# smolGura/fish-tts

Hardware: AMD Instinct MI355X
Metric: semantic tokens/sec (higher is better)
Workload: dtype bf16; 1 GPU; openaudio-s1-mini shapes (BASELINE configs[1]): batch=1 per GPU, 48-token prompt, 215 frames (10 s), top-p sampling, hipGraph-captured frame step, + DAC codec decode; prompt_len=48, parallelism=replica x1, frame_engine=3

## Files before the change

fish-tts_amd/csrc/engine.hip:

```cpp
#include "engine.h"
#include "ar_kernels.h"
#include "frame_engine.h"
#include "wide_kernels.h"
#include "codec_kernels.h"

#include <math.h>

#include <algorithm>
#include <mutex>
#include <stdio.h>
#include <stdlib.h>
#include <string.h>

using namespace ft;

static std::string g_create_err;
static void eng_release(ft_ctx* ctx);

ft_status ft_fail(ft_ctx* ctx, ft_status code, const std::string& msg) {
    if (ctx) ctx->err = msg; else g_create_err = msg;
    return code;
}

template <typename S, typename D>
// ... 131 lines not shown
    FT_TRY(dmalloc(ctx, &ctx->part_ml, M * c.n_head * ctx->nsplit_max * 2));
    ctx->cache_m_stride = (size_t)c.n_local_heads * ctx->n_slots * c.head_dim;
    ctx->fcache_m_stride = (size_t)c.fast_n_local_heads * c.num_codebooks * c.fast_head_dim;
    ctx->layers.resize(c.n_layer);
    ctx->flayers.resize(c.n_fast_layer);
    for (auto& l : ctx->layers) {
        FT_TRY(dmalloc(ctx, (char**)&l.kc, M * ctx->cache_m_stride * ctx->esz));
        FT_TRY(dmalloc(ctx, (char**)&l.vc, M * ctx->cache_m_stride * ctx->esz));
    }
    for (auto& l : ctx->flayers) {
        FT_TRY(dmalloc(ctx, (char**)&l.kc, M * ctx->fcache_m_stride * ctx->esz));
        FT_TRY(dmalloc(ctx, (char**)&l.vc, M * ctx->fcache_m_stride * ctx->esz));
    }
    const size_t R = c.num_codebooks + 1;
    FT_TRY(dmalloc(ctx, &ctx->d_pos, M));
    FT_TRY(dmalloc(ctx, &ctx->d_tok, M * R));
    FT_TRY(dmalloc(ctx, &ctx->d_tokn, M * R));
    FT_TRY(dmalloc(ctx, &ctx->d_seq, M * R * ctx->cap));
    FT_TRY(dmalloc(ctx, &ctx->d_nf, M));
    FT_TRY(dmalloc(ctx, &ctx->d_done, M));
    FT_TRY(dmalloc(ctx, &ctx->d_prompt, R * (size_t)c.max_seq_len));
    FT_TRY(dmalloc(ctx, &ctx->d_ctl, M));
    ctx->prefill_gemm_mode = getenv("FT_PREFILL_GEMM") ? atoi(getenv("FT_PREFILL_GEMM")) : 2;
    ctx->prefill_v0 = getenv("FT_PREFILL_V0") != nullptr || c.dtype != FT_BF16 || c.dim % 32 || (c.n_head * c.head_dim) % 32 ||
                      c.intermediate_size % 32;
    if (!ctx->prefill_v0) {
        const size_t S = c.max_seq_len;
        FT_TRY(dmalloc(ctx, &ctx->pf_x, S * c.dim));
        FT_TRY(dmalloc(ctx, &ctx->pf_qkv, S * qkvN));
        FT_TRY(dmalloc(ctx, &ctx->pf_y, S * c.n_head * c.head_dim));
        FT_TRY(dmalloc(ctx, &ctx->pf_xn, S * c.dim));
        FT_TRY(dmalloc(ctx, &ctx->pf_ybf, S * c.n_head * c.head_dim));
        FT_TRY(dmalloc(ctx, &ctx->pf_g, S * c.intermediate_size));
        FT_TRY(dmalloc(ctx, &ctx->pf_qbf, S * c.n_head * c.head_dim));
        FT_TRY(dmalloc(ctx, &ctx->pf_seqs, M));
        FT_TRY(dmalloc(ctx, &ctx->pf_rows, S));
    }
    if (c.dtype == FT_F16 || !ctx->prefill_v0) {
        const int HD = c.n_head * c.head_dim, HDf = c.fast_n_head * c.fast_head_dim;
        ctx->wide_ok = !getenv("FT_NO_WIDE") && !c.fast_attention_qkv_bias && !c.fast_attention_o_bias && c.fast_dim == c.dim &&
                       wide_k_ok(c.dim) && wide_k_ok(HD) && wide_k_ok(c.intermediate_size) && wide_k_ok(HDf) && wide_k_ok(c.fast_intermediate_size) &&
                       qkvN % 32 == 0 && fqkvN % 32 == 0 && c.intermediate_size % 16 == 0 && c.fast_intermediate_size % 16 == 0 &&
                       c.dim % 16 == 0 && c.vocab_size % 32 == 0 && ctx->fastV % 16 == 0;
        if (ctx->wide_ok) {
            ctx->xo_pair = (int)((M + 15) / 16 * 16);
            ctx->no_pair = getenv("FT_NO_PAIR") != nullptr;
            ctx->no_attn_wide = getenv("FT_NO_ATTN_WIDE") != nullptr;
            ctx->no_head_stream = getenv("FT_NO_HEAD_STREAM") != nullptr;
            ctx->xo_ldm = 2 * ctx->xo_pair;
            const size_t P = ctx->xo_ldm;
            FT_TRY(dmalloc(ctx, &ctx->xo_x, P * c.dim));
            FT_TRY(dmalloc(ctx, &ctx->xo_xf, P * c.fast_dim));
            FT_TRY(dmalloc(ctx, &ctx->xo_femb, P * c.fast_dim));
            FT_TRY(dmalloc(ctx, &ctx->xo_y, P * (size_t)std::max(HD, HDf)));
            FT_TRY(dmalloc(ctx, &ctx->xo_g, P * (size_t)std::max(c.intermediate_size, c.fast_intermediate_size)));
        }
    }
    const size_t nchunk = ((size_t)c.vocab_size + 1023) / 1024;
    FT_TRY(dmalloc(ctx, &ctx->samp_cut, M));
    FT_TRY(dmalloc(ctx, &ctx->samp_chunk_cnt, M * nchunk));
    FT_TRY(dmalloc(ctx, &ctx->samp_part_score, M * nchunk));
    FT_TRY(dmalloc(ctx, &ctx->samp_part_idx, M * nchunk));
    FT_HIP(ctx, hipHostMalloc((void**)&ctx->h_pin, (3 * M + 8) * sizeof(int), hipHostMallocDefault));
    return FT_OK;
}

extern "C" ft_status ft_create(const ft_ar_config* ar, const ft_codec_config* codec, int32_t device, ft_ctx** out) {
    if (!out || (!ar && !codec)) return ft_fail(nullptr, FT_ERR_ARG, "ft_create: need a config and an out pointer");
    int ndev = 0;
    if (hipGetDeviceCount(&ndev) != hipSuccess || ndev == 0)
        return ft_fail(nullptr, FT_ERR_HIP, "ft_create: no HIP device visible (the MI355X path has no CPU fallback)");
    if (device < 0 || device >= ndev) return ft_fail(nullptr, FT_ERR_ARG, "ft_create: bad device index");
    ft_ctx* ctx = new ft_ctx();
    ctx->device = device;
    ft_status st = FT_OK;
    do {
        if (hipSetDevice(device) != hipSuccess) { st = ft_fail(ctx, FT_ERR_HIP, "hipSetDevice failed"); break; }
        if (hipStreamCreateWithFlags(&ctx->stream, hipStreamNonBlocking) != hipSuccess) {
            st = ft_fail(ctx, FT_ERR_HIP, "hipStreamCreate failed"); break;
        }
        if (ar) {
            ctx->c = *ar;
            ctx->has_ar = true;
            if ((st = ar_validate(ctx)) != FT_OK) break;
            if ((st = ar_alloc(ctx)) != FT_OK) break;
            ar_expected(ctx);
        }
        if (codec) {
            ctx->cc = *codec;
            ctx->has_codec = true;
            if ((st = codec_create(ctx)) != FT_OK) break;
            codec_expected(ctx);
        }
    } while (0);
    if (st != FT_OK) {
        g_create_err = ctx->err;
        ft_destroy(ctx);
        return st;
    }
    *out = ctx;
    return FT_OK;
}

extern "C" void ft_destroy(ft_ctx* ctx) {
    if (!ctx) return;
    hipSetDevice(ctx->device);
    if (ctx->stream) hipStreamSynchronize(ctx->stream);
    for (auto& kv : ctx->graphs) hipGraphExecDestroy(kv.second);
    for (auto& kv : ctx->expected) if (kv.second.p) hipFree(kv.second.p);
    for (auto& l : ctx->layers) { hipFree(l.kc); hipFree(l.vc); if (l.w13) hipFree(l.w13); }
    for (auto& l : ctx->flayers) { hipFree(l.kc); hipFree(l.vc); if (l.w13) hipFree(l.w13); }
    float* bufs[] = {ctx->x, ctx->qkv, ctx->y, ctx->g, ctx->logits, ctx->femb, ctx->xf, ctx->qkvf, ctx->gf,
                     ctx->flog, ctx->part_o, ctx->part_ml, ctx->noise};
    for (float* b : bufs) if (b) hipFree(b);
    if (ctx->hid && ctx->hid != ctx->x) hipFree(ctx->hid);
    int* ibufs[] = {ctx->d_pos, ctx->d_tok, ctx->d_tokn, ctx->d_seq, ctx->d_nf, ctx->d_done, ctx->d_prompt};
    for (int* b : ibufs) if (b) hipFree(b);
    if (ctx->d_ctl) hipFree(ctx->d_ctl);
    if (ctx->wide_qkv0_tab) hipFree(ctx->wide_qkv0_tab);
    { void* pf[] = {ctx->pf_x, ctx->pf_qkv, ctx->pf_y, ctx->pf_xn, ctx->pf_ybf, ctx->pf_g, ctx->xo_x, ctx->xo_xf, ctx->xo_femb, ctx->xo_y, ctx->xo_g, ctx->pf_qbf}; for (void* q : pf) if (q) hipFree(q); }
    for (auto& l : ctx->layers) { if (l.bqkv_f32) hipFree(l.bqkv_f32); if (l.bo_f32) hipFree(l.bo_f32); }
    if (ctx->samp_cut) hipFree(ctx->samp_cut);
    if (ctx->samp_chunk_cnt) hipFree(ctx->samp_chunk_cnt);
    if (ctx->samp_part_score) hipFree(ctx->samp_part_score);
    if (ctx->samp_part_idx) hipFree(ctx->samp_part_idx);
    eng_release(ctx);
    if (ctx->h_pin) hipHostFree(ctx->h_pin);
    for (auto e : ctx->prof_ev) hipEventDestroy(e);
    codec_destroy(ctx);
    if (ctx->stream) hipStreamDestroy(ctx->stream);
    delete ctx;
}

extern "C" const char* ft_last_error(const ft_ctx* ctx) { return ctx ? ctx->err.c_str() : g_create_err.c_str(); }

extern "C" ft_status ft_sync(ft_ctx* ctx) {
    if (!ctx) return FT_ERR_ARG;
    FT_HIP(ctx, hipSetDevice(ctx->device));
    FT_HIP(ctx, hipStreamSynchronize(ctx->stream));
    return FT_OK;
}

extern "C" ft_status ft_load_weight(ft_ctx* ctx, const char* name, const void* src, int32_t src_dtype,
                                    const int64_t* shape, int32_t ndim) {
    if (!ctx || !name || !src || !shape) return ft_fail(ctx, FT_ERR_ARG, "ft_load_weight: null argument");
    if (ctx->finalized) return ft_fail(ctx, FT_ERR_STATE, "ft_load_weight: weights already finalized");
    auto it = ctx->expected.find(name);
    if (it == ctx->expected.end()) return ft_fail(ctx, FT_ERR_ARG, std::string("unknown weight name: ") + name);
    FtTensor& t = it->second;
    if ((int)t.shape.size() != ndim) return ft_fail(ctx, FT_ERR_ARG, std::string("rank mismatch for ") + name);
    for (int i = 0; i < ndim; ++i)
        if (t.shape[i] != shape[i]) {
            char buf[256];
            snprintf(buf, sizeof buf, "shape mismatch for %s: dim %d is %lld, expected %lld", name, i,
                     (long long)shape[i], (long long)t.shape[i]);
            return ft_fail(ctx, FT_ERR_ARG, buf);
        }
    if (src_dtype != FT_F32 && src_dtype != FT_BF16 && src_dtype != FT_F16)
        return ft_fail(ctx, FT_ERR_ARG, "src_dtype must be FT_F32, FT_BF16 or FT_F16");
    FT_HIP(ctx, hipSetDevice(ctx->device));
    const int64_t n = t.numel();
    const size_t ssz = src_dtype == FT_F32 ? 4 : 2, dsz = t.dtype == FT_F32 ? 4 : 2;
    if (!t.p) FT_HIP(ctx, hipMalloc(&t.p, (size_t)n * dsz + 64));
    if (src_dtype == t.dtype) {
        FT_HIP(ctx, hipMemcpy(t.p, src, (size_t)n * dsz, hipMemcpyDefault));
        return FT_OK;
    }
    void* stage = nullptr;
    FT_HIP(ctx, hipMalloc(&stage, (size_t)n * ssz));
    hipError_t e = hipMemcpy(stage, src, (size_t)n * ssz, hipMemcpyDefault);
    if (e == hipSuccess) {
        const int blocks = (int)((n + 255) / 256 < 4096 ? (n + 255) / 256 : 4096);
        auto to = [&](auto* sp) {
            if (t.dtype == FT_F32) convert_kernel<<<blocks, 256, 0, ctx->stream>>>(sp, (float*)t.p, n);
            else if (t.dtype == FT_BF16) convert_kernel<<<blocks, 256, 0, ctx->stream>>>(sp, (bf16_t*)t.p, n);
            else convert_kernel<<<blocks, 256, 0, ctx->stream>>>(sp, (f16_t*)t.p, n);
        };
        if (src_dtype == FT_F32) to((const float*)stage);
        else if (src_dtype == FT_BF16) to((const bf16_t*)stage);
        else to((const f16_t*)stage);
        e = hipStreamSynchronize(ctx->stream);
    }
    hipFree(stage);
    if (e != hipSuccess) return ft_fail(ctx, FT_ERR_HIP, std::string("ft_load_weight copy: ") + hipGetErrorString(e));
    return FT_OK;
}

static void* wp(ft_ctx* ctx, const std::string& n) {
    auto it = ctx->expected.find(n);
    return it == ctx->expected.end() ? nullptr : it->second.p;
}

static ft_status eng_setup(ft_ctx* ctx);
static ft_status wide_qkv0_build(ft_ctx* ctx);

static ft_status ar_finalize(ft_ctx* ctx) {
    const ft_ar_config& c = ctx->c;
    ctx->emb = wp(ctx, "embeddings.weight");
    ctx->cb_emb = wp(ctx, "codebook_embeddings.weight");
    ctx->norm = wp(ctx, "norm.weight");
    ctx->head = c.tie_word_embeddings ? ctx->emb : wp(ctx, "output.weight");
    ctx->fproj_w = wp(ctx, "fast_project_in.weight");
    ctx->fproj_b = wp(ctx, "fast_project_in.bias");
    ctx->fast_emb = wp(ctx, "fast_embeddings.weight");
    ctx->fast_norm = wp(ctx, "fast_norm.weight");
    ctx->fast_out = wp(ctx, "fast_output.weight");
    ctx->rope = (float*)wp(ctx, "rope.slow");
    ctx->frope = (float*)wp(ctx, "rope.fast");
    auto fill = [&](std::vector<FtLayer>& ls, const char* pre, int ffn, int dim) -> ft_status {
        for (size_t i = 0; i < ls.size(); ++i) {
            const std::string p = std::string(pre) + std::to_string(i);
            FtLayer& l = ls[i];
            l.attn_norm = wp(ctx, p + ".attention_norm.weight");
            l.wqkv = wp(ctx, p + ".attention.wqkv.weight");
            l.bqkv = wp(ctx, p + ".attention.wqkv.bias");
            l.qn = wp(ctx, p + ".attention.q_norm.weight");
            l.kn = wp(ctx, p + ".attention.k_norm.weight");
            l.wo = wp(ctx, p + ".attention.wo.weight");
            l.bo = wp(ctx, p + ".attention.wo.bias");
            l.ffn_norm = wp(ctx, p + ".ffn_norm.weight");
            l.w2 = wp(ctx, p + ".feed_forward.w2.weight");
            FtTensor& w1 = ctx->expected[p + ".feed_forward.w1.weight"];
            FtTensor& w3 = ctx->expected[p + ".feed_forward.w3.weight"];
            FT_HIP(ctx, hipMalloc(&l.w13, (size_t)2 * ffn * dim * ctx->esz));
            const int64_t n = (int64_t)ffn * dim;
            const int blocks = (int)((n + 255) / 256 < 4096 ? (n + 255) / 256 : 4096);
            if (ctx->esz == 2)
                interleave_rows_kernel<bf16_t><<<blocks, 256, 0, ctx->stream>>>((bf16_t*)w1.p, (bf16_t*)w3.p, (bf16_t*)l.w13, ffn, dim);
            else
                interleave_rows_kernel<float><<<blocks, 256, 0, ctx->stream>>>((float*)w1.p, (float*)w3.p, (float*)l.w13, ffn, dim);
            FT_HIP(ctx, hipStreamSynchronize(ctx->stream));
            hipFree(w1.p); w1.p = nullptr;
            hipFree(w3.p); w3.p = nullptr;
        }
        return FT_OK;
    };
    FT_TRY(fill(ctx->layers, "layers.", c.intermediate_size, c.dim));
    if (!ctx->prefill_v0 || ctx->wide_ok) {
        const int qkvN = (c.n_head + 2 * c.n_local_heads) * c.head_dim;
        auto to_f32 = [&](const void* b, float* o, int n) {
            if (c.dtype == FT_F16) convert_kernel<f16_t, float><<<(n + 255) / 256, 256, 0, ctx->stream>>>((const f16_t*)b, o, n);
            else convert_kernel<bf16_t, float><<<(n + 255) / 256, 256, 0, ctx->stream>>>((const bf16_t*)b, o, n);
        };
        for (auto& l : ctx->layers) {
            if (l.bqkv) {
                FT_HIP(ctx, hipMalloc((void**)&l.bqkv_f32, qkvN * sizeof(float)));
                to_f32(l.bqkv, l.bqkv_f32, qkvN);
            }
            if (l.bo) {
                FT_HIP(ctx, hipMalloc((void**)&l.bo_f32, c.dim * sizeof(float)));
                to_f32(l.bo, l.bo_f32, c.dim);
            }
        }
        FT_HIP(ctx, hipStreamSynchronize(ctx->stream));
    }
    FT_TRY(fill(ctx->flayers, "fast_layers.", c.fast_intermediate_size, c.fast_dim));
    FT_TRY(eng_setup(ctx));
    FT_TRY(wide_qkv0_build(ctx));
    return FT_OK;
}

constexpr int ENG_MAX_STRIKES = 2;
static std::mutex g_eng_mu;
static std::map<int, ft_ctx*> g_eng_owner;

static void eng_release(ft_ctx* ctx) {
    void* eb[] = {ctx->eng_layers, ctx->eng_flayers, ctx->eng_gx ,
                  ctx->eng_gpart, ctx->eng_fast_g, ctx->eng_ctl, ctx->eng_qkv0_tab};
    for (void* q : eb) if (q) hipFree(q);
    ctx->eng_layers = ctx->eng_flayers = nullptr;
    ctx->eng_gx = ctx->eng_gqkv = ctx->eng_gy = ctx->eng_gxb = ctx->eng_gg = ctx->eng_fast_g = ctx->eng_ctl = nullptr;
    ctx->eng_gpart = nullptr;
    ctx->eng_qkv0_tab = nullptr;
    ctx->eng_on = ctx->eng_fast_on = false;
    if (ctx->eng_owner) {
        std::lock_guard<std::mutex> lk(g_eng_mu);
        auto it = g_eng_owner.find(ctx->device);
        if (it != g_eng_owner.end() && it->second == ctx) g_eng_owner.erase(it);
        ctx->eng_owner = false;
    }
}

static bool eng_fits_cu(const void* fn, size_t lds, size_t lds_cap, const char* name, std::string& why) {
    hipFuncAttributes fa{};
    const hipError_t fe = hipFuncGetAttributes(&fa, fn);
    if (fe != hipSuccess) { (void)hipGetLastError(); why = std::string("hipFuncGetAttributes: ") + hipGetErrorString(fe); return false; }
    const int regs = std::max(fa.numRegs, 1), per_simd = 512 / (((regs + 7) / 8) * 8);
    const bool fits = per_simd * 4 >= ENG_THREADS / 64 && lds + fa.sharedSizeBytes <= lds_cap && fa.maxThreadsPerBlock >= ENG_THREADS;
    if (getenv("FT_LOG")) {
        int occ = -1;
        const hipError_t oe = hipOccupancyMaxActiveBlocksPerMultiprocessor(&occ, fn, ENG_THREADS, lds);
        if (oe != hipSuccess) (void)hipGetLastError();
        fprintf(stderr, "fish_tts_amd: %s engine kernel: %d registers (%d waves per SIMD), %zu B of LDS of %zu: %s (the occupancy query says %d)\n",
                name, fa.numRegs, per_simd, lds + fa.sharedSizeBytes, lds_cap, fits ? "fits a CU" : "does not fit a CU", occ);
    }
    if (!fits) why = std::string("a ") + name + " workgroup does not fit one CU (registers / LDS)";
    return fits;
}

typedef void (*eng_slow_fn_t)(SlowEngP);
typedef void (*eng_fast_fn_t)(FastEngP);
typedef void (*eng_qkv0_fn_t)(const bf16_t*, const bf16_t*, const bf16_t*, const bf16_t*, bf16_t*, int, int, int, float);
struct EngSlowEntry { int D, H, HKV, HDIM, F, SQ, SF, SO; eng_slow_fn_t xl, plain; };
struct EngFastEntry { int D, H, HKV, HDIM, F, V, SQ, SF, SO; eng_fast_fn_t loop; eng_qkv0_fn_t qkv0; };
template <typename S, bool WITH_XL>
static EngSlowEntry eng_slow_entry() {
    eng_slow_fn_t xl = nullptr;
    if constexpr (WITH_XL) xl = slow_engine_kernel<S, true>;
    return EngSlowEntry{S::D, S::H, S::HKV, S::HDIM, S::F, S::SQ, S::SF, S::SO, xl, slow_engine_kernel<S, false>};
}
template <typename S>
static EngFastEntry eng_fast_entry() {
    return EngFastEntry{S::D, S::H, S::HKV, S::HDIM, S::F, S::V, S::SQ, S::SF, S::SO, fast_engine_kernel<S, 10>, eng_qkv0_table_kernel<S>};
}
static const EngSlowEntry* eng_slow_shapes(int* n) {
    static const EngSlowEntry tab[] = {eng_slow_entry<EngSlowS1, true>(), eng_slow_entry<EngSlowShape<1024, 16, 8, 128, 4096>, true>(),
                                       eng_slow_entry<EngSlowShape<1024, 16, 4, 128, 3072>, false>()};
    *n = (int)(sizeof tab / sizeof tab[0]);
    return tab;
}
static const EngFastEntry* eng_fast_shapes(int* n) {
    static const EngFastEntry tab[] = {eng_fast_entry<EngFastS1>(), eng_fast_entry<EngFastShape<1024, 16, 8, 64, 4096, 1024>>()};
    *n = (int)(sizeof tab / sizeof tab[0]);
    return tab;
}

static bool eng_setup_try(ft_ctx* ctx, std::string& why) {
    const ft_ar_config& c = ctx->c;
    auto hip_ok = [&](hipError_t e, const char* what) {
        if (e == hipSuccess) return true;
        why = std::string(what) + ": " + hipGetErrorString(e);
        (void)hipGetLastError();
        return false;
    };
    if (getenv("FT_NO_ENGINE")) { why = "FT_NO_ENGINE is set"; return false; }
    if (c.dtype != FT_BF16) { why = "precision is not bf16"; return false; }
    hipDeviceProp_t prop;
    if (!hip_ok(hipGetDeviceProperties(&prop, ctx->device), "hipGetDeviceProperties")) return false;
    const int nb = prop.multiProcessorCount;
    const int HD = c.n_head * c.head_dim;
    const int qkvN = (c.n_head + 2 * c.n_local_heads) * c.head_dim;
    auto per = [&](int units) { return (units + nb - 1) / nb; };
    const EngSlowEntry* se = nullptr;
    {
        int n = 0;
        const EngSlowEntry* tab = eng_slow_shapes(&n);
        for (int i = 0; i < n && !se; ++i)
            if (c.dim == tab[i].D && c.n_head == tab[i].H && c.n_local_heads == tab[i].HKV && c.head_dim == tab[i].HDIM && c.intermediate_size == tab[i].F)
                se = &tab[i];
    }
    const bool shape_ok = se && c.fast_dim == c.dim && c.n_layer >= 1 && c.n_layer < ENG_EPOCH_STEP &&
                          per(qkvN) <= se->SQ * ENG_CW && per(c.dim) <= se->SO * ENG_CW && per(c.intermediate_size) <= se->SF * ENG_CW &&
                          qkvN % (4 * nb) == 0 && c.dim % (4 * nb) == 0 && c.intermediate_size % (4 * nb) == 0 && per(qkvN) <= ENG_LINE &&
                          per(c.intermediate_size) <= ENG_LINE && c.n_local_heads * ctx->nsplit_max <= nb && c.head_dim % (4 * ctx->nsplit_max) == 0 && nb == ENG_NB;
    if (!shape_ok) {
        char buf[320];
        snprintf(buf, sizeof buf, "widths outside the engine's instantiations (dim %d, heads %d / %d x %d, ffn %d, fast_dim %d on %d CUs; "
                 "built for dim 1024, 16 heads x 128 with 8 kv heads and ffn 3072 or 4096, or 4 kv heads and ffn 3072, on 256 CUs)", c.dim, c.n_head,
                 c.n_local_heads, c.head_dim, c.intermediate_size, c.fast_dim, nb);
        why = buf;
        return false;
    }
    {
        std::lock_guard<std::mutex> lk(g_eng_mu);
        auto it = g_eng_owner.find(ctx->device);
        if (it != g_eng_owner.end() && it->second != ctx) {
            why = "another context of this process already runs the frame engine on this device (its workgroups need every CU)";
            return false;
        }
        g_eng_owner[ctx->device] = ctx;
        ctx->eng_owner = true;
    }
    ctx->eng_nb = nb;
    std::vector<EngLayer> h(c.n_layer);
    for (int i = 0; i < c.n_layer; ++i) {
        const FtLayer& l = ctx->layers[i];
        h[i] = EngLayer{(const bf16_t*)l.wqkv, (const bf16_t*)l.bqkv, (const bf16_t*)l.attn_norm, (const bf16_t*)l.qn,
                        (const bf16_t*)l.kn, (const bf16_t*)l.wo, (const bf16_t*)l.bo, (const bf16_t*)l.ffn_norm,
                        (const bf16_t*)l.w13, (const bf16_t*)l.w2, (bf16_t*)l.kc, (bf16_t*)l.vc};
    }
    if (!hip_ok(hipMalloc((void**)&ctx->eng_layers, h.size() * sizeof(EngLayer)), "hipMalloc(engine layer table)")) return false;
    if (!hip_ok(hipMemcpy(ctx->eng_layers, h.data(), h.size() * sizeof(EngLayer), hipMemcpyHostToDevice), "hipMemcpy(engine layer table)")) return false;
    auto zalloc = [&](void** q, size_t bytes, const char* what) {
        return hip_ok(hipMalloc(q, bytes), what) && hip_ok(hipMemset(*q, 0, bytes), what);
    };
    const size_t L = c.n_layer;
    const size_t VB = (size_t)nb * ENG_LINE * 4;
    const size_t pool_words = ((L + 1) * VB + 3 * L * VB + L * HD * 4) / 4;
    ctx->eng_relay = getenv("FT_NO_RELAY") == nullptr;
    ctx->eng_pool_bytes = pool_words * 4 * (ctx->eng_relay ? 9 : 1);
    if (!zalloc((void**)&ctx->eng_gx, ctx->eng_pool_bytes, "hipMalloc(engine hand-off pool)")) return false;
    ctx->eng_pool_words = pool_words;
    ctx->eng_gxb = ctx->eng_gx + (L + 1) * (VB / 4);
    ctx->eng_gg = ctx->eng_gxb + L * (VB / 4);
    ctx->eng_gy = ctx->eng_gg + L * (VB / 4);
    ctx->eng_gqkv = ctx->eng_gy + L * HD;
    ctx->eng_gpart_bytes = L * c.n_head * ctx->nsplit_max * (size_t)(c.head_dim + 2) * 8;
    if (!zalloc((void**)&ctx->eng_gpart, ctx->eng_gpart_bytes, "hipMalloc(engine split partials)")) return false;
    if (!zalloc((void**)&ctx->eng_ctl, ENG_CTL_WORDS * 4, "hipMalloc(engine control words)")) return false;
    const int G = c.n_head / c.n_local_heads, hd = c.head_dim, NSLOT = 4 * (64 / (hd >> 3));
    size_t fl = (size_t)c.dim * 2 + HD + c.intermediate_size + (size_t)(G + 2) * hd + (size_t)G * hd + 2 * hd +
                (size_t)NSLOT * G * 2 + (size_t)NSLOT * G * hd + 64 * 6 + ENG_MAX_OUT + 8;
    ctx->eng_lds_slow = std::max(fl * sizeof(float), (size_t)82 * 1024);
    const size_t lds_cap = prop.maxSharedMemoryPerMultiProcessor;
    if (ctx->eng_lds_slow > lds_cap) { why = "the slow stack's LDS need exceeds the CU's"; return false; }
    ctx->eng_xl = ctx->xl_shape && nb == 256 && ctx->nsplit_max == 32 && c.n_local_heads * 32 == nb;
    ctx->eng_xl = ctx->eng_xl && se->xl != nullptr;
    ctx->eng_slow_fn = (const void*)(ctx->eng_xl ? se->xl : se->plain);
    const void* slow_fn = ctx->eng_slow_fn;
    if (!hip_ok(hipFuncSetAttribute(slow_fn, hipFuncAttributeMaxDynamicSharedMemorySize, (int)ctx->eng_lds_slow),
                "hipFuncSetAttribute(slow_engine_kernel)")) return false;
    if (!eng_fits_cu(slow_fn, ctx->eng_lds_slow, lds_cap, "slow-stack", why)) return false;
    ctx->eng_on = true;
    why = ctx->eng_xl ? "slow stack on the frame engine (one kv head per XCD)" : "slow stack on the frame engine";

    const int HDf = c.fast_n_head * c.fast_head_dim;
    const int fqkvN = (c.fast_n_head + 2 * c.fast_n_local_heads) * c.fast_head_dim;
    const EngFastEntry* fe = nullptr;
    {
        int n = 0;
        const EngFastEntry* tab = eng_fast_shapes(&n);
        for (int i = 0; i < n && !fe; ++i)
            if (c.fast_dim == tab[i].D && c.fast_n_head == tab[i].H && c.fast_n_local_heads == tab[i].HKV && c.fast_head_dim == tab[i].HDIM &&
                c.fast_intermediate_size == tab[i].F && ctx->fastV == tab[i].V)
                fe = &tab[i];
    }
    const bool fast_ok = !getenv("FT_NO_FAST_ENGINE") && fe && HDf == c.fast_dim && c.n_fast_layer >= 1 &&
                         c.num_codebooks >= 2 && c.num_codebooks <= 10 && fqkvN % (4 * nb) == 0 && ctx->fastV % (4 * nb) == 0 &&
                         per(fqkvN) <= fe->SQ * ENG_CW && per(c.fast_dim) <= fe->SO * ENG_CW && per(c.fast_intermediate_size) <= fe->SF * ENG_CW &&
                         per(ctx->fastV) <= fe->SO * ENG_CW && per(fqkvN) <= ENG_LINE && per(c.fast_intermediate_size) <= ENG_LINE && ctx->fastV <= 1024 &&
                         c.codebook_size <= 65536;
    if (!fast_ok) { why += "; fast loop on launches (FT_NO_FAST_ENGINE, or fast widths outside the instantiations: 1024 / 16 + 8 heads x 64 / ffn 3072 or 4096 / 1024 codes used, <= 10 codebooks)"; return true; }
    ctx->eng_fast_fn = (const void*)fe->loop;
    auto fast_off = [&](const std::string& w2) { why += "; fast loop on launches (" + w2 + ")"; return true; };
    std::vector<EngLayer> hf(c.n_fast_layer);
    for (int i = 0; i < c.n_fast_layer; ++i) {
        const FtLayer& l = ctx->flayers[i];
        hf[i] = EngLayer{(const bf16_t*)l.wqkv, (const bf16_t*)l.bqkv, (const bf16_t*)l.attn_norm, (const bf16_t*)l.qn,
                         (const bf16_t*)l.kn, (const bf16_t*)l.wo, (const bf16_t*)l.bo, (const bf16_t*)l.ffn_norm,
                         (const bf16_t*)l.w13, (const bf16_t*)l.w2, nullptr, nullptr};
    }
    std::string w2;
    auto hip_ok2 = [&](hipError_t e, const char* what) {
        if (e == hipSuccess) return true;
        w2 = std::string(what) + ": " + hipGetErrorString(e);
        (void)hipGetLastError();
        return false;
    };
    if (!hip_ok2(hipMalloc((void**)&ctx->eng_flayers, hf.size() * sizeof(EngLayer)), "hipMalloc(fast layer table)")) return fast_off(w2);
    if (!hip_ok2(hipMemcpy(ctx->eng_flayers, hf.data(), hf.size() * sizeof(EngLayer), hipMemcpyHostToDevice), "hipMemcpy(fast layer table)")) return fast_off(w2);
    const size_t nLf = c.n_fast_layer;
    ctx->eng_fast_words = (2 * ((nLf + 1) + 3 * nLf + 1)) * (VB / 4) + (size_t)c.num_codebooks * ENG_LINE;
    ctx->eng_fast_bytes = ctx->eng_fast_words * 4 * (ctx->eng_relay ? 9 : 1);
    if (!hip_ok2(hipMalloc((void**)&ctx->eng_fast_g, ctx->eng_fast_bytes), "hipMalloc(fast hand-off pool)") ||
        !hip_ok2(hipMemset(ctx->eng_fast_g, 0, ctx->eng_fast_bytes), "hipMemset(fast hand-off pool)")) return fast_off(w2);
    const int kvw = c.fast_n_local_heads * c.fast_head_dim;
    ctx->eng_pair = getenv("FT_NO_PAIR") == nullptr &&
                    eng_fast_lds_bytes(c.fast_dim, fqkvN, HDf, c.fast_intermediate_size, ctx->fastV, (int)nLf, c.num_codebooks, kvw, true) <= lds_cap;
    ctx->eng_lds_fast = eng_fast_lds_bytes(c.fast_dim, fqkvN, HDf, c.fast_intermediate_size, ctx->fastV, (int)nLf, c.num_codebooks, kvw, ctx->eng_pair);
    if (ctx->eng_lds_fast > lds_cap) return fast_off("the codebook loop's LDS need exceeds the CU's");
    ctx->eng_lds_fast = std::max(ctx->eng_lds_fast, (size_t)82 * 1024);
    if (!hip_ok2(hipFuncSetAttribute(ctx->eng_fast_fn, hipFuncAttributeMaxDynamicSharedMemorySize,
                                     (int)ctx->eng_lds_fast), "hipFuncSetAttribute(fast_engine_kernel)")) return fast_off(w2);
    if (!eng_fits_cu(ctx->eng_fast_fn, ctx->eng_lds_fast, lds_cap, "codebook-loop", w2)) return fast_off(w2);
    if (getenv("FT_NO_QKV0") == nullptr && c.num_codebooks > 2) {
        const size_t tb = (size_t)ctx->fastV * fqkvN * sizeof(bf16_t);
        if (!hip_ok2(hipMalloc((void**)&ctx->eng_qkv0_tab, tb), "hipMalloc(layer-0 q k v table)")) return fast_off(w2);
        const FtLayer& l0 = ctx->flayers[0];
        const size_t lds = ((size_t)c.fast_dim + ENG_MAX_OUT) * sizeof(float);
        fe->qkv0<<<dim3(fqkvN / (fe->SQ * ENG_CW), 16), ENG_CW * 64, lds, ctx->stream>>>(
            (const bf16_t*)l0.wqkv, (const bf16_t*)l0.bqkv, (const bf16_t*)l0.attn_norm, (const bf16_t*)ctx->fast_emb,
            (bf16_t*)ctx->eng_qkv0_tab, c.fast_dim, fqkvN, ctx->fastV, c.norm_eps);
        if (!hip_ok2(hipGetLastError(), "eng_qkv0_table_kernel") || !hip_ok2(hipStreamSynchronize(ctx->stream), "eng_qkv0_table_kernel")) {
            hipFree(ctx->eng_qkv0_tab); ctx->eng_qkv0_tab = nullptr;
            return fast_off(w2);
        }
    }
    ctx->eng_fast_on = true;
    why = ctx->eng_xl ? "slow stack (one kv head per XCD) and codebook loop on the frame engine" : "slow stack and codebook loop on the frame engine";
    return true;
}

static ft_status eng_setup(ft_ctx* ctx) {
    ctx->eng_on = ctx->eng_fast_on = false;
    std::string why;
    if (!eng_setup_try(ctx, why)) {
        eng_release(ctx);
        ctx->eng_why = "launch path: " + why;
    } else {
        char buf[64];
        snprintf(buf, sizeof buf, " (%d workgroups)", ctx->eng_nb);
        ctx->eng_why = why + buf;
    }
    if (getenv("FT_LOG")) fprintf(stderr, "fish_tts_amd: batch-1 decode frames: %s\n", ctx->eng_why.c_str());
    return FT_OK;
}

extern "C" ft_status ft_finalize_weights(ft_ctx* ctx) {
    if (!ctx) return FT_ERR_ARG;
    if (ctx->finalized) return FT_OK;
    FT_HIP(ctx, hipSetDevice(ctx->device));
    for (auto& kv : ctx->expected)
        if (!kv.second.p) return ft_fail(ctx, FT_ERR_MISSING_WEIGHT, "missing weight: " + kv.first);
    if (ctx->has_ar) FT_TRY(ar_finalize(ctx));
    if (ctx->has_codec) FT_TRY(codec_finalize(ctx));
    ctx->finalized = true;
    return FT_OK;
}

struct Launch {
    ft_ctx* ctx;
    hipStream_t s;
    int m0, M;
    int pos_off;
    hipError_t err = hipSuccess;
    bool gemv_only = false;
    bool tail_only = false;
    void chk() { hipError_t e = hipGetLastError(); if (e != hipSuccess && err == hipSuccess) err = e; }
};

struct PfX {
    const void* gain = nullptr;
    const float* ss_in = nullptr;
    int nblk = 0;
    float* ss_out = nullptr;
};
enum { PF_ID_NONE = -1, PF_ID_SKINNY1 = 0, PF_ID_SKINNY2 = 1, PF_ID_SKINNY4 = 2, PF_ID_LIN128 = 3, PF_ID_LIN64 = 4, PF_ID_TAP64_128 = 5,
       PF_ID_TAP64_64 = 6, PF_ID_TAP_128 = 7, PF_ID_TAP_64 = 8 };
static int pf_gemm(Launch& L, const bf16_t* X, long ldx, int S, const void* W, const float* bias, int N, int K,
                   int act, const float* resid, float* out_f32, bf16_t* out_bf, long ldo, int round_out,
                   const PfX& fx = PfX());
static bool wide_batch(const Launch& L) {
    return L.ctx->wide_ok && L.M >= L.ctx->wide_min && L.M <= 64 && !L.gemv_only && !L.ctx->prof;
}

static bool wide_pair(const Launch& L) {
    const ft_ctx* ctx = L.ctx;
    return wide_batch(L) && !ctx->no_pair && ctx->c.num_codebooks >= 2 && ctx->c.n_fast_layer > 0 && ctx->xo_pair + L.M <= 64;
}

enum { WIDE_ID_S11 = 0, WIDE_ID_S12 = 1, WIDE_ID_S22 = 2, WIDE_ID_G12 = 3, WIDE_ID_G22 = 4, WIDE_ID_R11 = 5, WIDE_ID_HEAD = 6 };
template <typename WT>
static int wide_gemm(Launch& L, const bf16_t* X, const void* W, const float* bias, int N, int K, const void* gain, int epi,
                      float* out_f32, long ldo, bf16_t* out_xo, const bf16_t* resid_xo, int rows = 0, bool vocab_head = false) {
    const int M = rows > 0 ? rows : L.M;
    WidePT<WT> p{};
    p.X = (const WT*)X; p.ldm = L.ctx->xo_ldm; p.W = (const WT*)W; p.ldw = K; p.gain = (const WT*)gain; p.eps = L.ctx->c.norm_eps;
    p.bias = bias; p.M = M; p.N = N; p.K = K; p.out_f32 = out_f32; p.ldo = ldo; p.out_xo = (WT*)out_xo; p.ldm_o = L.ctx->xo_ldm;
    p.resid_xo = (const WT*)resid_xo;
    bool ok;
    int id;
    if (epi == WEPI_RESID) { id = WIDE_ID_R11; ok = wide_gemm_launch<1, 1, false, WEPI_RESID>(p, L.s); }
    else if (epi == WEPI_SWIGLU) {
        id = M > 16 ? WIDE_ID_G22 : WIDE_ID_G12;
        ok = M > 16 ? wide_gemm_launch<2, 2, true, WEPI_SWIGLU>(p, L.s) : wide_gemm_launch<1, 2, true, WEPI_SWIGLU>(p, L.s);
    }
    else if (vocab_head && M <= 32 && K == 1024 && N % 16 == 0 && N >= 4096 && !L.ctx->no_head_stream) {
        static DevOnce once;
        once.run([] { hipFuncSetAttribute((const void*)wide_head_kernel<1024, WT>, hipFuncAttributeMaxDynamicSharedMemorySize, (int)wide_head_lds<1024>()); });
        wide_head_kernel<1024, WT><<<256, 512, wide_head_lds<1024>(), L.s>>>(p);
        id = WIDE_ID_HEAD;
        ok = true;
    }
    else if (N >= 32768) {
        id = M > 16 ? WIDE_ID_S22 : WIDE_ID_S12;
        ok = M > 16 ? wide_gemm_launch<2, 2, true, WEPI_STORE>(p, L.s) : wide_gemm_launch<1, 2, true, WEPI_STORE>(p, L.s);
    }
    else if (N >= 4096 && M > 16) { id = WIDE_ID_S12; ok = wide_gemm_launch<1, 2, true, WEPI_STORE>(p, L.s); }
    else { id = WIDE_ID_S11; ok = wide_gemm_launch<1, 1, true, WEPI_STORE>(p, L.s); }
    if (!ok && L.err == hipSuccess) L.err = hipErrorInvalidValue;
    L.chk();
    return id;
}

template <typename WT>
static __global__ __launch_bounds__(256) void xo_from_rows_kernel(const float* x, int ldx, int D, bf16_t* xo, int ldm) {
    const int m = blockIdx.y;
    for (int d = blockIdx.x * 256 + threadIdx.x; d < D; d += gridDim.x * 256) xo[xo_index(m, d, ldm)] = h16_bits<WT>(x[(size_t)m * ldx + d]);
}

static __global__ __launch_bounds__(256) void xo_from_h16_rows_kernel(const bf16_t* x, int D, bf16_t* xo, int ldm, int rows) {
    const int m = blockIdx.y;
    if (m >= rows) return;
    for (int d = blockIdx.x * 256 + threadIdx.x; d < D; d += gridDim.x * 256) xo[xo_index(m, d, ldm)] = x[(size_t)m * D + d];
}
template <typename WT>
static __global__ void f32_to_h16_kernel(const float* x, bf16_t* o, long n) {
    for (long i = (long)blockIdx.x * blockDim.x + threadIdx.x; i < n; i += (long)gridDim.x * blockDim.x) o[i] = h16_bits<WT>(x[i]);
}

template <typename WT>
static ft_status wide_qkv0_build_t(ft_ctx* ctx) {
    const ft_ar_config& c = ctx->c;
    if (!ctx->wide_ok || getenv("FT_NO_QKV0") || c.num_codebooks <= 2 || c.n_fast_layer < 1) return FT_OK;
    const int Df = c.fast_dim, qkvN = (c.fast_n_head + 2 * c.fast_n_local_heads) * c.fast_head_dim, V = ctx->fastV;
    const FtLayer& l0 = ctx->flayers[0];
    if (l0.bqkv) return FT_OK;
    constexpr int CH = 64;
    bf16_t* xo = nullptr; float* out = nullptr;
    if (hipMalloc((void**)&xo, (size_t)Df * CH * sizeof(bf16_t)) != hipSuccess || hipMalloc((void**)&out, (size_t)CH * qkvN * sizeof(float)) != hipSuccess ||
        hipMalloc((void**)&ctx->wide_qkv0_tab, (size_t)V * qkvN * sizeof(bf16_t)) != hipSuccess) {
        (void)hipGetLastError();
        if (xo) hipFree(xo);
        if (out) hipFree(out);
        if (ctx->wide_qkv0_tab) { hipFree(ctx->wide_qkv0_tab); ctx->wide_qkv0_tab = nullptr; }
        return FT_OK;
    }
    bool ok = true;
    for (int c0 = 0; c0 < V && ok; c0 += CH) {
        const int rows = std::min(CH, V - c0);
        xo_from_h16_rows_kernel<<<dim3((Df + 255) / 256, rows), 256, 0, ctx->stream>>>((const bf16_t*)ctx->fast_emb + (size_t)c0 * Df, Df, xo, CH, rows);
        WidePT<WT> p{};
        p.X = (const WT*)xo; p.ldm = CH; p.W = (const WT*)l0.wqkv; p.ldw = Df; p.gain = (const WT*)l0.attn_norm; p.eps = c.norm_eps;
        p.M = rows; p.N = qkvN; p.K = Df; p.out_f32 = out; p.ldo = qkvN;
        ok = wide_gemm_launch<1, 1, true, WEPI_STORE>(p, ctx->stream);
        f32_to_h16_kernel<WT><<<256, 256, 0, ctx->stream>>>(out, ctx->wide_qkv0_tab + (size_t)c0 * qkvN, (long)rows * qkvN);
    }
    ok = ok && hipStreamSynchronize(ctx->stream) == hipSuccess && hipGetLastError() == hipSuccess;
    hipFree(xo); hipFree(out);
    if (!ok) { hipFree(ctx->wide_qkv0_tab); ctx->wide_qkv0_tab = nullptr; (void)hipGetLastError(); }
    return FT_OK;
}
static ft_status wide_qkv0_build(ft_ctx* ctx) {
    if (ctx->c.dtype == FT_BF16) return wide_qkv0_build_t<bf16_t>(ctx);
    if (ctx->c.dtype == FT_F16) return wide_qkv0_build_t<f16_t>(ctx);
    return FT_OK;
}

static bool eng_slow_ok(const Launch& L) {
    const ft_ctx* ctx = L.ctx;
    return ctx->eng_on && !ctx->eng_suspended && L.M == 1 && !L.gemv_only && !ctx->prof && ctx->c.n_local_heads * ctx->nsplit <= ctx->eng_nb &&
           ctx->c.head_dim % (4 * ctx->nsplit) == 0;
}

static bool eng_fast_ok(const Launch& L) {
    const ft_ctx* ctx = L.ctx;
    return ctx->eng_fast_on && !ctx->eng_suspended && L.M == 1 && !L.gemv_only && !ctx->prof;
}

static void enqueue_fast_engine(Launch& L) {
    ft_ctx* ctx = L.ctx;
    const ft_ar_config& c = ctx->c;
    const int m0 = L.m0, R = c.num_codebooks + 1, nb = ctx->eng_nb;
    const size_t nLf = c.n_fast_layer, VW = (size_t)nb * ENG_LINE;
    FastEngP p{};
    p.layers = ctx->eng_flayers; p.n_layer = c.n_fast_layer; p.ncb = c.num_codebooks;
    p.D = c.fast_dim; p.H = c.fast_n_head; p.Hkv = c.fast_n_local_heads; p.hd = c.fast_head_dim; p.F = c.fast_intermediate_size;
    p.qkvN = (c.fast_n_head + 2 * c.fast_n_local_heads) * c.fast_head_dim; p.V = ctx->fastV;
    p.eps = c.norm_eps; p.scale = (float)(1.0 / sqrt((double)c.fast_head_dim));
    p.rope = ctx->frope; p.fast_norm = (const bf16_t*)ctx->fast_norm; p.fast_out = (const bf16_t*)ctx->fast_out;
    p.fast_emb = (const bf16_t*)ctx->fast_emb;
    p.qkv0_tab = (const bf16_t*)ctx->eng_qkv0_tab;
    p.hid = ctx->hid + (size_t)m0 * c.fast_dim; p.femb = ctx->femb + (size_t)m0 * c.fast_dim;
    unsigned* g = ctx->eng_fast_g;
    p.gx = g; g += 2 * (nLf + 1) * VW;
    p.gqkv = g; g += 2 * nLf * VW;
    p.gxb = g; g += 2 * nLf * VW;
    p.gg = g; g += 2 * nLf * VW;
    p.glog = g; g += 2 * VW;
    p.gcode = g;
    p.ctl = ctx->eng_ctl;
    p.rep_delta0 = ctx->eng_relay ? (long)ctx->eng_fast_words : 0; p.rep_stride = ctx->eng_relay ? (long)ctx->eng_fast_words : 0;
    SampP s{};
    s.logits = nullptr; s.ldl = ctx->fastV; s.V = ctx->fastV;
    s.ctl = ctx->d_ctl + m0; s.tokn = ctx->d_tokn + (size_t)m0 * R; s.seq = ctx->d_seq + (size_t)m0 * R * ctx->cap;
    s.cap = ctx->cap; s.nf = ctx->d_nf + m0; s.cb = 1; s.ncb = c.num_codebooks; s.sem_begin = c.semantic_begin_id;
    s.im_end = c.im_end_id; s.cbsize = c.codebook_size; s.fast_emb = ctx->fast_emb;
    s.femb = ctx->femb + (size_t)m0 * c.fast_dim; s.Df = c.fast_dim; s.noise = ctx->noise;
    s.noise_row_len = ctx->noise_row_len; s.noise_rows = ctx->noise_rows; s.noise_off = 0; s.last = 0;
    s.tok = ctx->d_tok + (size_t)m0 * R; s.pos = ctx->d_pos + m0; s.done = ctx->d_done + m0;
    p.samp = s;
    p.noise_cb_stride = ctx->fastV; p.noise_off1 = c.vocab_size;
    p.pair = ctx->eng_pair ? 1 : 0;
    ((eng_fast_fn_t)ctx->eng_fast_fn)<<<nb, ENG_THREADS, ctx->eng_lds_fast, L.s>>>(p);
    L.chk();
}

static void enqueue_slow_engine(Launch& L, const int* toks, long tok_row_stride, long tok_m_stride, int col) {
    ft_ctx* ctx = L.ctx;
    const ft_ar_config& c = ctx->c;
    const int m0 = L.m0;
    SlowEngP p{};
    p.layers = ctx->eng_layers; p.n_layer = c.n_layer;
    p.D = c.dim; p.H = c.n_head; p.Hkv = c.n_local_heads; p.hd = c.head_dim; p.F = c.intermediate_size;
    p.qkvN = (c.n_head + 2 * c.n_local_heads) * c.head_dim;
    p.eps = c.norm_eps; p.scale = 1.0f / sqrtf((float)c.head_dim);
    p.emb = (const bf16_t*)ctx->emb; p.cb_emb = (const bf16_t*)ctx->cb_emb;
    p.toks = toks + (size_t)m0 * tok_m_stride + col; p.tok_row_stride = tok_row_stride;
    p.ncb = c.num_codebooks; p.cbsize = c.codebook_size; p.vocab = c.vocab_size; p.sem_begin = c.semantic_begin_id;
    p.sem_end = c.semantic_end_id; p.scale_cb = c.scale_codebook_embeddings; p.inv_div = (float)sqrt((double)(c.num_codebooks + 1));
    p.rope = ctx->rope; p.pos = ctx->d_pos + m0; p.pos_off = L.pos_off; p.n_slots = ctx->n_slots; p.nsplit = ctx->nsplit;
    p.cache_off = (size_t)m0 * ctx->cache_m_stride;
    p.gx = ctx->eng_gx; p.gqkv = ctx->eng_gqkv; p.gpart = ctx->eng_gpart; p.gy = ctx->eng_gy; p.gxb = ctx->eng_gxb; p.gg = ctx->eng_gg;
    p.ctl = ctx->eng_ctl; p.x_out = ctx->x + (size_t)m0 * c.dim; p.nt = 1;
    p.rep_delta0 = ctx->eng_relay ? (long)ctx->eng_pool_words : 0; p.rep_stride = ctx->eng_relay ? (long)ctx->eng_pool_words : 0;
    ((eng_slow_fn_t)ctx->eng_slow_fn)<<<ctx->eng_nb, ENG_THREADS, ctx->eng_lds_slow, L.s>>>(p);
    L.chk();
}


template <typename WT, int ROUND, int R>
static void gemv_nt(Launch& L, const GemvP& p, int nt) {
    const dim3 grid((p.N + 4 * R - 1) / (4 * R), L.M), block(256);
#define FT_NT(n) case n: gemv_kernel<WT, n, R, ROUND><<<grid, block, 0, L.s>>>(p); break;
    switch (nt) { FT_NT(1) FT_NT(2) FT_NT(3) FT_NT(4) FT_NT(6) FT_NT(8) FT_NT(12) default: L.err = hipErrorInvalidValue; }
#undef FT_NT
}

static int pick_nt(int K, int vec) {
    const int need = (K + 64 * vec - 1) / (64 * vec);
    const int opts[] = {1, 2, 3, 4, 6, 8, 12};
    for (int o : opts) if (o >= need) return o;
    return -1;
}

template <typename WT, int ROUND, int R, int MB>
static void gemv_mb_nt(Launch& L, const GemvP& p, int nt) {
    const dim3 grid((p.N + 4 * R - 1) / (4 * R), (L.M + MB - 1) / MB), block(256);
#define FT_NT(n) case n: gemv_mb_kernel<WT, n, R, MB, ROUND><<<grid, block, 0, L.s>>>(p, L.M); break;
    switch (nt) { FT_NT(1) FT_NT(2) FT_NT(4) FT_NT(6) default: L.err = hipErrorInvalidValue; }
#undef FT_NT
}

struct GemvId { int MB, R, NT; };
template <typename WT, int ROUND>
static GemvId gemv(Launch& L, GemvP p, int R) {
    const int nt = pick_nt(p.K, Vec<WT>::N);
    if (nt < 0) { L.err = hipErrorInvalidValue; return GemvId{-1, -1, -1}; }
    GemvId id{0, 0, nt};
    ft_ctx* ctx = L.ctx;
    hipEvent_t e0 = nullptr, e1 = nullptr;
    if (ctx->prof && !ctx->prof_count_only) {
        hipEventCreate(&e0); hipEventCreate(&e1);
        hipEventRecord(e0, L.s);
    }
    if (p.epi == EPI_SWIGLU && R < 2) R = 2;
    const bool mb_ok = sizeof(WT) == 2 && L.M >= 2 && (nt == 1 || nt == 2 || nt == 4 || nt == 6);
    if (mb_ok) {
        if constexpr (sizeof(WT) == 2) {
            const bool four = L.M >= 3 && nt <= 2 && R <= 2;
            if (R >= 4) { id.R = 4; if (nt <= 2) { id.MB = 2; gemv_mb_nt<WT, ROUND, 4, 2>(L, p, nt); } else gemv_nt<WT, ROUND, 4>(L, p, nt); }
            else if (R == 2) { id.R = 2; id.MB = four ? 4 : 2; if (four) gemv_mb_nt<WT, ROUND, 2, 4>(L, p, nt); else gemv_mb_nt<WT, ROUND, 2, 2>(L, p, nt); }
            else { id.R = 1; id.MB = four ? 4 : 2; if (four) gemv_mb_nt<WT, ROUND, 1, 4>(L, p, nt); else gemv_mb_nt<WT, ROUND, 1, 2>(L, p, nt); }
        }
    } else if (R == 1) { id.R = 1; gemv_nt<WT, ROUND, 1>(L, p, nt); }
    else if (R == 2) { id.R = 2; gemv_nt<WT, ROUND, 2>(L, p, nt); }
    else if (R >= 8 && nt <= 2 && p.epi != EPI_SWIGLU) { id.R = 8; gemv_nt<WT, ROUND, 8>(L, p, nt); }
    else { id.R = 4; gemv_nt<WT, ROUND, 4>(L, p, nt); }
    if (ctx->prof) {
        if (!ctx->prof_count_only) {
            hipEventRecord(e1, L.s);
            ctx->prof_ev.push_back(e0); ctx->prof_ev.push_back(e1);
        }
        ctx->prof_bytes += (int64_t)p.N * p.K * sizeof(WT);
        ctx->prof_launches += 1;
    }
    L.chk();
    return id;
}

static int rows_per_wave(int N, int M) {
    const long waves1 = (long)N * M;
    if (waves1 >= 65536) return 4;
    if (waves1 >= 2048) return 2;
    return 1;
}

template <typename WT, int ROUND>
static void attn_decode(Launch& L, const AttnP& p) {
    ft_ctx* ctx = L.ctx;
    const int G = p.H / p.Hkv;
    const int nslot = 2048 / p.hd;
    const size_t lds = ((size_t)G * p.hd + 2 * p.hd + (size_t)nslot * G * 2 + (size_t)nslot * G * p.hd) * sizeof(float);
    const dim3 grid(p.Hkv, p.nsplit, L.M), block(256);
    switch (G) {
        case 1: attn_decode_kernel<WT, 1, ROUND><<<grid, block, lds, L.s>>>(p); break;
        case 2: attn_decode_kernel<WT, 2, ROUND><<<grid, block, lds, L.s>>>(p); break;
        case 4: attn_decode_kernel<WT, 4, ROUND><<<grid, block, lds, L.s>>>(p); break;
        case 8: {
            static DevOnce once;
            once.run([&] { hipFuncSetAttribute((const void*)attn_decode_kernel<WT, 8, ROUND>,
                                               hipFuncAttributeMaxDynamicSharedMemorySize, (int)lds); });
// ... 1987 lines not shown
```

fish-tts_amd/csrc/frame_engine.h:

```cpp
#pragma once
#include "ar_kernels.h"

namespace ft {

constexpr int ENG_NB = 256;
constexpr int ENG_WAVES = 8;
constexpr int ENG_THREADS = ENG_WAVES * 64;
constexpr int ENG_CW = 4;
constexpr int ENG_GW = 4;

template <int D_, int H_, int HKV_, int HDIM_, int F_>
struct EngSlowShape {
    static constexpr int D = D_, H = H_, HKV = HKV_, HDIM = HDIM_, F = F_;
    static constexpr int HD = H * HDIM, QKVN = (H + 2 * HKV) * HDIM, G = H / HKV;
    static constexpr int NTD = D / 512, NTA = HD / 512, NTF = F / 512;
    static constexpr int SQ = (QKVN / ENG_NB + ENG_CW - 1) / ENG_CW, SF = (F / ENG_NB + ENG_CW - 1) / ENG_CW, SO = (D / ENG_NB + ENG_CW - 1) / ENG_CW;
    static constexpr bool PK3 = F % 384 == 0 && (F / ENG_NB) % 3 == 0;
    static_assert(D % 512 == 0 && HD % 512 == 0 && F % 512 == 0, "weight rows are read as whole 16-byte pieces by 64 lanes");
    static_assert(QKVN % (4 * ENG_NB) == 0 && D % (4 * ENG_NB) == 0 && F % (4 * ENG_NB) == 0, "whole 16-byte granule groups per workgroup");
    static_assert(H % HKV == 0 && HDIM % 8 == 0 && HDIM <= 128, "grouped-query attention, 16-byte K/V pieces");
};
template <int D_, int H_, int HKV_, int HDIM_, int F_, int V_>
struct EngFastShape {
    static constexpr int D = D_, H = H_, HKV = HKV_, HDIM = HDIM_, F = F_, V = V_;
    static constexpr int HD = H * HDIM, QKVN = (H + 2 * HKV) * HDIM, KVW = HKV * HDIM;
    static constexpr int NTD = D / 512, NTA = HD / 512, NTF = F / 512;
    static constexpr int SQ = (QKVN / ENG_NB + ENG_CW - 1) / ENG_CW, SF = (F / ENG_NB + ENG_CW - 1) / ENG_CW, SO = (D / ENG_NB + ENG_CW - 1) / ENG_CW;
    static constexpr bool PK3 = F % 384 == 0 && (F / ENG_NB) % 3 == 0;
    static_assert(D % 512 == 0 && HD % 512 == 0 && F % 512 == 0 && V == 1024 && HD == D, "fast widths");
    static_assert(QKVN % (4 * ENG_NB) == 0 && D % (4 * ENG_NB) == 0 && F % (4 * ENG_NB) == 0 && V % (4 * ENG_NB) == 0, "whole granule groups per workgroup");
};
typedef EngSlowShape<1024, 16, 8, 128, 3072> EngSlowS1;
typedef EngFastShape<1024, 16, 8, 64, 3072, 1024> EngFastS1;
constexpr int ENG_EPOCH_STEP = 64;
constexpr unsigned long long ENG_TIMEOUT_TICKS = 20000000ull;

typedef __attribute__((address_space(1))) unsigned eng_gu32;
typedef __attribute__((address_space(1))) unsigned long long eng_gu64;
#define ENG_RLX __ATOMIC_RELAXED, __HIP_MEMORY_SCOPE_AGENT

enum { ENG_CTL_EPOCH = 0, ENG_CTL_ABORT = 1, ENG_CTL_EXIT = 2, ENG_CTL_WHERE = 3, ENG_CTL_ARRIVED = 4, ENG_CTL_FAULT = 5, ENG_CTL_FAULT_SKIP = 6,
       ENG_CTL_XCD = 16, ENG_CTL_WORDS = 32 };
constexpr unsigned ENG_FAULT_FAST = 0x10000u;
__device__ __forceinline__ bool eng_fault_here(unsigned* ctl, unsigned base, int b) {
    const unsigned f = __hip_atomic_load((__attribute__((address_space(1))) unsigned*)(ctl + ENG_CTL_FAULT), __ATOMIC_RELAXED, __HIP_MEMORY_SCOPE_AGENT);
    if (f != base + 1u + (unsigned)b) return false;
    const unsigned skip = __hip_atomic_load((__attribute__((address_space(1))) unsigned*)(ctl + ENG_CTL_FAULT_SKIP), __ATOMIC_RELAXED, __HIP_MEMORY_SCOPE_AGENT);
    if (skip > 0u) {
        __hip_atomic_store((__attribute__((address_space(1))) unsigned*)(ctl + ENG_CTL_FAULT_SKIP), skip - 1u, __ATOMIC_RELAXED, __HIP_MEMORY_SCOPE_AGENT);
        return false;
    }
    __hip_atomic_store((__attribute__((address_space(1))) unsigned*)(ctl + ENG_CTL_FAULT), 0u, __ATOMIC_RELAXED, __HIP_MEMORY_SCOPE_AGENT);
    return true;
}

struct EngLayer {
    const bf16_t *wqkv, *bqkv, *attn_norm, *qn, *kn, *wo, *bo, *ffn_norm, *w13, *w2;
    bf16_t *kc, *vc;
};

__device__ __forceinline__ void eng_barrier() {
    __builtin_amdgcn_fence(__ATOMIC_RELEASE, "workgroup", "local");
    __builtin_amdgcn_s_barrier();
    __builtin_amdgcn_fence(__ATOMIC_ACQUIRE, "workgroup", "local");
}

typedef const __attribute__((address_space(1))) U4* eng_gU4;
template <bool NT> __device__ __forceinline__ U4 eng_ldg16(const void* p) {
    if constexpr (NT) return __builtin_nontemporal_load((eng_gU4)p);
    else return *(eng_gU4)p;
}
__device__ __forceinline__ float eng_ldg_bf16(const bf16_t* p, size_t i) {
    return bf16_bits_to_f32(((const __attribute__((address_space(1))) bf16_t*)p)[i]);
}
typedef const __attribute__((address_space(4))) unsigned long long* eng_c64;
__device__ __forceinline__ EngLayer eng_layer(const EngLayer* table, int i) {
    static_assert(sizeof(EngLayer) == 12 * sizeof(unsigned long long), "EngLayer is twelve pointers");
    eng_c64 q = (eng_c64)(unsigned long long)(table + i);
    EngLayer l;
    l.wqkv = (const bf16_t*)q[0]; l.bqkv = (const bf16_t*)q[1]; l.attn_norm = (const bf16_t*)q[2]; l.qn = (const bf16_t*)q[3];
    l.kn = (const bf16_t*)q[4]; l.wo = (const bf16_t*)q[5]; l.bo = (const bf16_t*)q[6]; l.ffn_norm = (const bf16_t*)q[7];
    l.w13 = (const bf16_t*)q[8]; l.w2 = (const bf16_t*)q[9]; l.kc = (bf16_t*)q[10]; l.vc = (bf16_t*)q[11];
    return l;
}

__device__ __forceinline__ unsigned eng_tag16(unsigned e) { return (e & 0x7fffu) | 0x8000u; }
__device__ __forceinline__ unsigned eng_tag32(unsigned e) { return e | 0x80000000u; }
__device__ __forceinline__ unsigned long long eng_rt() { return __builtin_amdgcn_s_memrealtime(); }

__device__ __forceinline__ void eng_put(unsigned* g, int i, float v, unsigned tag16) {
    __hip_atomic_store((eng_gu32*)(g + i), (tag16 << 16) | (__float_as_uint(v) >> 16), ENG_RLX);
}
__device__ __forceinline__ void eng_put_raw(unsigned* g, int i, unsigned v16, unsigned tag16) {
    __hip_atomic_store((eng_gu32*)(g + i), (tag16 << 16) | (v16 & 0xffffu), ENG_RLX);
}
__device__ __forceinline__ void eng_put4(unsigned* g, float v0, float v1, float v2, float v3, unsigned tag16) {
    U4 w;
    w.x = (tag16 << 16) | (__float_as_uint(v0) >> 16); w.y = (tag16 << 16) | (__float_as_uint(v1) >> 16);
    w.z = (tag16 << 16) | (__float_as_uint(v2) >> 16); w.w = (tag16 << 16) | (__float_as_uint(v3) >> 16);
    asm volatile("global_store_dwordx4 %0, %1, off sc1" :: "v"(g), "v"(w) : "memory");
}
__device__ __forceinline__ void eng_put64(unsigned long long* g, size_t i, float v, unsigned tag32) {
    __hip_atomic_store((eng_gu64*)(g + i), ((unsigned long long)tag32 << 32) | __float_as_uint(v), ENG_RLX);
}

template <int FL = 0>
__device__ __forceinline__ void eng_ld3_sc1(const void* p0, const void* p1, const void* p2, U4& a, U4& b, U4& c) {
    asm volatile("global_load_dwordx4 %0, %3, off sc1\n\tglobal_load_dwordx4 %1, %4, off sc1\n\t"
                 "global_load_dwordx4 %2, %5, off sc1\n\ts_waitcnt vmcnt(0)"
                 : "=&v"(a), "=&v"(b), "=&v"(c) : "v"(p0), "v"(p1), "v"(p2) : "memory");
}
template <int FL = 0>
__device__ __forceinline__ void eng_ld1_sc1(const void* p0, U4& a) {
    asm volatile("global_load_dwordx4 %0, %1, off sc1\n\ts_waitcnt vmcnt(0)" : "=&v"(a) : "v"(p0) : "memory");
}

__device__ __forceinline__ bool eng_tags_ok(const U4& v, unsigned tag) {
    return (v.x >> 16) == tag && (v.y >> 16) == tag && (v.z >> 16) == tag && (v.w >> 16) == tag;
}
__device__ __forceinline__ void eng_unpack_to_lds(float* dst, const U4& v) {
    float4 f;
    f.x = __uint_as_float(v.x << 16); f.y = __uint_as_float(v.y << 16);
    f.z = __uint_as_float(v.z << 16); f.w = __uint_as_float(v.w << 16);
    *reinterpret_cast<float4*>(dst) = f;
}

struct EngSpin {
    unsigned* ctl;
    int* dead;
    unsigned spins = 0;
    unsigned long long t0 = 0;
    int where;
    __device__ __forceinline__ bool give_up(int lane) {
        if ((++spins & 255u) != 0u) return false;
        const unsigned long long t = eng_rt();
        if (t0 == 0) t0 = t;
        if (t - t0 > ENG_TIMEOUT_TICKS || __hip_atomic_load((eng_gu32*)(ctl + ENG_CTL_ABORT), ENG_RLX)) {
            if (lane == 0) {
                if (!__hip_atomic_load((eng_gu32*)(ctl + ENG_CTL_ABORT), ENG_RLX))
                    __hip_atomic_store((eng_gu32*)(ctl + ENG_CTL_WHERE), (unsigned)where, ENG_RLX);
                __hip_atomic_store((eng_gu32*)(ctl + ENG_CTL_ABORT), 1u, ENG_RLX);
                *dead = 1;
            }
            return true;
        }
        return false;
    }
};

constexpr int ENG_LINE = 32;
__device__ __forceinline__ size_t eng_pub(int b, int u_lo) { (void)b; return (size_t)u_lo; }
struct EngLayout {
    int per;
    __device__ __forceinline__ int off(int u) const { return u; }
};
struct EngIdent { __device__ __forceinline__ int operator()(int i) const { return i; } };

template <typename DMap = EngIdent, int FL = 0>
__device__ __forceinline__ void eng_gather(const unsigned* g, EngLayout lay, int u0, int n, unsigned tag, float* dst, int gw, int ngw,
                                           int lane, unsigned* ctl, int* dead, int where, DMap dmap = DMap(),
                                           unsigned long long* dbg = nullptr) {
    const int npiece = (n + 255) >> 8;
    EngSpin sp{ctl, dead, 0, 0, where};
    unsigned long long n_full = 0, t_first = 0;
    for (int p0 = gw; p0 < npiece; p0 += 3 * ngw) {
        const int c0 = p0;
        const int c1 = p0 + ngw < npiece ? p0 + ngw : c0;
        const int c2 = p0 + 2 * ngw < npiece ? p0 + 2 * ngw : c0;
        const int i0 = c0 * 256 + lane * 4 < n ? c0 * 256 + lane * 4 : c0 * 256;
        const int i1 = c1 * 256 + lane * 4 < n ? c1 * 256 + lane * 4 : c1 * 256;
        const int i2 = c2 * 256 + lane * 4 < n ? c2 * 256 + lane * 4 : c2 * 256;
        const int o0 = lay.off(u0 + i0), o1 = lay.off(u0 + i1), o2 = lay.off(u0 + i2);
        U4 a, b, c;
        for (;;) {
            if (c1 == c0) { eng_ld1_sc1<FL>(g + o0, a); b = a; c = a; }
            else eng_ld3_sc1<FL>(g + o0, g + o1, g + o2, a, b, c);
            const bool oa = eng_tags_ok(a, tag), ob = eng_tags_ok(b, tag), oc = eng_tags_ok(c, tag);
            if (dbg && n_full == 0) t_first = eng_rt();
            ++n_full;
            if (__all(oa && ob && oc)) break;
            if (sp.give_up(lane)) return;
        }
        if (c0 * 256 + lane * 4 < n) eng_unpack_to_lds(dst + dmap(i0), a);
        if (c1 != c0 && c1 * 256 + lane * 4 < n) eng_unpack_to_lds(dst + dmap(i1), b);
        if (c2 != c0 && c2 * 256 + lane * 4 < n) eng_unpack_to_lds(dst + dmap(i2), c);
    }
    if (dbg && lane == 0) { dbg[0] = t_first; dbg[1] = n_full; dbg[2] = 0; }
}

struct EngRelay {
    int on;
    int rank, nr;
    long delta;
};

__device__ __forceinline__ void eng_register(unsigned* ctl, int nb, int* r, int* dead) {
    const int xcd = (int)(__builtin_amdgcn_s_getreg(20 | (0 << 6) | (3 << 11)) & 7u);
    const unsigned rank = atomicAdd(ctl + ENG_CTL_XCD + xcd, 1u);
    atomicAdd(ctl + ENG_CTL_ARRIVED, 1u);
    EngSpin sp{ctl, dead, 0, 0, 9999};
    bool ok = true;
    while (__hip_atomic_load((eng_gu32*)(ctl + ENG_CTL_ARRIVED), ENG_RLX) < (unsigned)nb) {
        if (sp.give_up(0)) { ok = false; break; }
        __builtin_amdgcn_s_sleep(2);
    }
    r[0] = xcd; r[1] = (int)rank;
    r[2] = ok ? (int)__hip_atomic_load((eng_gu32*)(ctl + ENG_CTL_XCD + xcd), ENG_RLX) : 1;
}

template <typename DMap = EngIdent>
__device__ __forceinline__ void eng_gather_x(const EngRelay& rl, const unsigned* g, EngLayout lay, int u0, int n, unsigned tag, float* dst,
                                             int gw, int ngw, int lane, unsigned* ctl, int* dead, int where, DMap dmap = DMap(),
                                             unsigned long long* dbg = nullptr) {
    if (!rl.on) { eng_gather(g, lay, u0, n, tag, dst, gw, ngw, lane, ctl, dead, where, dmap, dbg); return; }
    unsigned* rep = const_cast<unsigned*>(g) + rl.delta;
    const int npiece = (n + 255) >> 8;
    for (int p = rl.rank; p < npiece; p += rl.nr) {
        if (p % ngw != gw) continue;
        const int i = p * 256 + lane * 4 < n ? p * 256 + lane * 4 : p * 256;
        const int o = lay.off(u0 + i);
        EngSpin sp{ctl, dead, 0, 0, where};
        U4 a;
        for (;;) {
            eng_ld1_sc1(g + o, a);
            if (__all(eng_tags_ok(a, tag))) break;
            if (sp.give_up(lane)) return;
        }
        if (p * 256 + lane * 4 < n) *reinterpret_cast<U4*>(rep + o) = a;
    }
    eng_gather<DMap, 1>(rep, lay, u0, n, tag, dst, gw, ngw, lane, ctl, dead, where, dmap, dbg);
}

__device__ __forceinline__ bool eng_tags3_ok(const U4& v, unsigned tag) { return (v.y >> 16) == tag && (v.w >> 16) == tag; }
__device__ __forceinline__ void eng_unpack3_to_lds(float* dst, const U4& v) {
    float2 a, b, c;
    a.x = __uint_as_float(v.x << 16); a.y = __uint_as_float(v.x & 0xffff0000u);
    b.x = __uint_as_float(v.y << 16); b.y = __uint_as_float(v.z << 16);
    c.x = __uint_as_float(v.z & 0xffff0000u); c.y = __uint_as_float(v.w << 16);
    reinterpret_cast<float2*>(dst)[0] = a; reinterpret_cast<float2*>(dst)[1] = b; reinterpret_cast<float2*>(dst)[2] = c;
}
template <int FL = 0>
__device__ __forceinline__ void eng_gather3(const unsigned* g, int n, unsigned tag, float* dst, int gw, int ngw, int lane, unsigned* ctl,
                                            int* dead, int where) {
    const int npiece = n / 384;
    EngSpin sp{ctl, dead, 0, 0, where};
    for (int p0 = gw; p0 < npiece; p0 += 3 * ngw) {
        const int c0 = p0;
        const int c1 = p0 + ngw < npiece ? p0 + ngw : c0;
        const int c2 = p0 + 2 * ngw < npiece ? p0 + 2 * ngw : c0;
        const unsigned* a0 = g + c0 * 256 + lane * 4;
        const unsigned* a1 = g + c1 * 256 + lane * 4;
        const unsigned* a2 = g + c2 * 256 + lane * 4;
        U4 a, b, c;
        for (;;) {
            if (c1 == c0) { eng_ld1_sc1<FL>(a0, a); b = a; c = a; }
            else eng_ld3_sc1<FL>(a0, a1, a2, a, b, c);
            if (__all(eng_tags3_ok(a, tag) && eng_tags3_ok(b, tag) && eng_tags3_ok(c, tag))) break;
            if (sp.give_up(lane)) return;
        }
        eng_unpack3_to_lds(dst + c0 * 384 + lane * 6, a);
        if (c1 != c0) eng_unpack3_to_lds(dst + c1 * 384 + lane * 6, b);
        if (c2 != c0) eng_unpack3_to_lds(dst + c2 * 384 + lane * 6, c);
    }
}
__device__ __forceinline__ void eng_gather3_x(const EngRelay& rl, const unsigned* g, int n, unsigned tag, float* dst, int gw, int ngw,
                                              int lane, unsigned* ctl, int* dead, int where) {
    if (!rl.on) { eng_gather3(g, n, tag, dst, gw, ngw, lane, ctl, dead, where); return; }
    unsigned* rep = const_cast<unsigned*>(g) + rl.delta;
    const int npiece = n / 384;
    for (int p = rl.rank; p < npiece; p += rl.nr) {
        if (p % ngw != gw) continue;
        const int o = p * 256 + lane * 4;
        EngSpin sp{ctl, dead, 0, 0, where};
        U4 a;
        for (;;) {
            eng_ld1_sc1(g + o, a);
            if (__all(eng_tags3_ok(a, tag))) break;
            if (sp.give_up(lane)) return;
        }
        *reinterpret_cast<U4*>(rep + o) = a;
    }
    eng_gather3<1>(rep, n, tag, dst, gw, ngw, lane, ctl, dead, where);
}

struct EngSrc2 { const unsigned* g[2]; float* dst[2]; unsigned tag[2]; };
template <int FL = 0>
__device__ __forceinline__ void eng_gather2(const EngSrc2& S, long delta, int n, int gw, int ngw, int lane, unsigned* ctl, int* dead,
                                            int where) {
    const int npiece = n >> 8, NP = 2 * npiece;
    EngSpin sp{ctl, dead, 0, 0, where};
    for (int p0 = gw; p0 < NP; p0 += 3 * ngw) {
        const int c0 = p0;
        const int c1 = p0 + ngw < NP ? p0 + ngw : c0;
        const int c2 = p0 + 2 * ngw < NP ? p0 + 2 * ngw : c0;
        const int s0 = c0 >= npiece, s1 = c1 >= npiece, s2 = c2 >= npiece;
        const int i0 = (c0 - s0 * npiece) * 256 + lane * 4, i1 = (c1 - s1 * npiece) * 256 + lane * 4, i2 = (c2 - s2 * npiece) * 256 + lane * 4;
        const unsigned* a0 = S.g[s0] + delta + i0;
        const unsigned* a1 = S.g[s1] + delta + i1;
        const unsigned* a2 = S.g[s2] + delta + i2;
        const unsigned t0 = S.tag[s0], t1 = S.tag[s1], t2 = S.tag[s2];
        U4 a, b, c;
        for (;;) {
            if (c1 == c0) { eng_ld1_sc1<FL>(a0, a); b = a; c = a; }
            else eng_ld3_sc1<FL>(a0, a1, a2, a, b, c);
            const bool oa = eng_tags_ok(a, t0), ob = c1 == c0 || eng_tags_ok(b, t1), oc = c2 == c0 || eng_tags_ok(c, t2);
            if (__all(oa && ob && oc)) break;
            if (sp.give_up(lane)) return;
        }
        eng_unpack_to_lds(S.dst[s0] + i0, a);
        if (c1 != c0) eng_unpack_to_lds(S.dst[s1] + i1, b);
        if (c2 != c0) eng_unpack_to_lds(S.dst[s2] + i2, c);
    }
}
__device__ __forceinline__ void eng_gather_x2(const EngRelay& rl, const EngSrc2& S, int n, int gw, int ngw, int lane, unsigned* ctl,
                                              int* dead, int where) {
    if (!rl.on) { eng_gather2(S, 0, n, gw, ngw, lane, ctl, dead, where); return; }
    const int npiece = n >> 8, NP = 2 * npiece;
    for (int p = rl.rank; p < NP; p += rl.nr) {
        if (p % ngw != gw) continue;
        const int s = p >= npiece;
        const int i = (p - s * npiece) * 256 + lane * 4;
        const unsigned* src = S.g[s] + i;
        const unsigned tg = S.tag[s];
        EngSpin sp{ctl, dead, 0, 0, where};
        U4 a;
        for (;;) {
            eng_ld1_sc1(src, a);
            if (__all(eng_tags_ok(a, tg))) break;
            if (sp.give_up(lane)) return;
        }
        *reinterpret_cast<U4*>(const_cast<unsigned*>(src) + rl.delta) = a;
    }
    eng_gather2<1>(S, rl.delta, n, gw, ngw, lane, ctl, dead, where);
}

template <int NT, int RPU, int MAXS>
struct EngW {
    U4 w[MAXS][RPU][NT];
    U4 gain[NT];
};

struct EngRowIdent { __device__ __forceinline__ int operator()(int u) const { return u; } };
struct EngRowQkvX {
    int q0, k0, v0, nq, nk;
    __device__ __forceinline__ int operator()(int u) const { return u < nq ? q0 + u : (u < nq + nk ? k0 + (u - nq) : v0 + (u - nq - nk)); }
};

template <bool NTL = true, int NT, int RPU, int MAXS, typename RM = EngRowIdent>
__device__ __forceinline__ void eng_issue(EngW<NT, RPU, MAXS>& r, const bf16_t* W, const bf16_t* gain, int K, int u_lo, int u_hi,
                                          int cw, int lane, int nt, RM rm = RM()) {
#pragma unroll
    for (int s = 0; s < MAXS; ++s) {
        int u = u_lo + cw + s * ENG_CW;
        u = u < u_hi ? u : u_hi - 1;
#pragma unroll
        for (int rr = 0; rr < RPU; ++rr)
#pragma unroll
            for (int t = 0; t < NT; ++t) {
                r.w[s][rr][t] = (nt & 2) ? U4{0u, 0u, 0u, 0u} : eng_ldg16<NTL>(W + (size_t)(rm(u) * RPU + rr) * K + t * 512 + lane * 8);
            }
    }
    if (gain) {
#pragma unroll
        for (int t = 0; t < NT; ++t) r.gain[t] = eng_ldg16<false>(gain + t * 512 + lane * 8);
    }
}

struct EngOut {
    float* vals;
    int* count;
    int seq;
};
constexpr int ENG_MAX_OUT = 64;
typedef __attribute__((address_space(3))) int* eng_lds_int;

template <int NT, int RPU, int MAXS, int PRO, int EPI, typename RM = EngRowIdent>
__device__ __forceinline__ void eng_gemv_rows(const EngW<NT, RPU, MAXS>& r, const float* xs, int K, float eps, const bf16_t* bias,
                                              const float* resid, float* vals, int u_lo, int u_hi, int cw, int lane, RM rm = RM()) {
    static_assert(EPI == EPI_SWIGLU ? RPU == 2 : RPU == 1, "a unit is a (w1, w3) pair for SwiGLU, one row otherwise");
    if (u_lo + cw < u_hi) {
        float xv[NT][8];
#pragma unroll
        for (int t = 0; t < NT; ++t) {
            const float4 f0 = *reinterpret_cast<const float4*>(xs + t * 512 + lane * 8);
            const float4 f1 = *reinterpret_cast<const float4*>(xs + t * 512 + lane * 8 + 4);
            xv[t][0] = f0.x; xv[t][1] = f0.y; xv[t][2] = f0.z; xv[t][3] = f0.w;
            xv[t][4] = f1.x; xv[t][5] = f1.y; xv[t][6] = f1.z; xv[t][7] = f1.w;
        }
        if (PRO == PRO_RMSNORM) {
            float ss = 0.f;
#pragma unroll
            for (int t = 0; t < NT; ++t)
#pragma unroll
                for (int j = 0; j < 8; ++j) ss = fmaf(xv[t][j], xv[t][j], ss);
            ss = wave_sum(ss);
            const float inv = rsqrt_exact(ss / (float)K + eps);
#pragma unroll
            for (int t = 0; t < NT; ++t) {
                float gv[8];
                Vec<bf16_t>::unpack(r.gain[t], gv);
#pragma unroll
                for (int j = 0; j < 8; ++j) xv[t][j] = round_bf16(round_bf16(xv[t][j] * inv) * gv[j]);
            }
        }
#pragma unroll
        for (int s = 0; s < MAXS; ++s) {
            const int u = u_lo + cw + s * ENG_CW;
            if (u >= u_hi) break;
            float acc[RPU];
#pragma unroll
            for (int rr = 0; rr < RPU; ++rr) {
                float a = 0.f;
#pragma unroll
                for (int t = 0; t < NT; ++t) {
                    float wv[8];
                    Vec<bf16_t>::unpack(r.w[s][rr][t], wv);
#pragma unroll
                    for (int j = 0; j < 8; ++j) a = fmaf(wv[j], xv[t][j], a);
                }
                acc[rr] = wave_sum(a);
            }
            float o;
            if (EPI == EPI_SWIGLU) {
                const float a = round_bf16(acc[0]);
                const float b = round_bf16(acc[RPU - 1]);
                const float sg = round_bf16(a / (1.0f + expf(-a)));
                o = round_bf16(sg * b);
            } else {
                float v = acc[0];
                if (bias) v += eng_ldg_bf16(bias, rm(u));
                v = round_bf16(v);
                if (EPI == EPI_RESID) v = round_bf16(resid[rm(u)] + v);
                o = v;
            }
            if (lane == 0) vals[u - u_lo] = o;
        }
    }
}

__device__ __forceinline__ void eng_put_local(unsigned* g, int i, float v, unsigned tag16) {
    __hip_atomic_store((eng_gu32*)(g + i), (tag16 << 16) | (__float_as_uint(v) >> 16), __ATOMIC_RELAXED, __HIP_MEMORY_SCOPE_WORKGROUP);
}
__device__ __forceinline__ void eng_put64_local(unsigned long long* g, size_t i, float v, unsigned tag32) {
    __hip_atomic_store((eng_gu64*)(g + i), ((unsigned long long)tag32 << 32) | __float_as_uint(v), __ATOMIC_RELAXED, __HIP_MEMORY_SCOPE_WORKGROUP);
}

template <int NT, int MAXS, typename RM>
__device__ __forceinline__ void eng_gemv_qkv_local(const EngW<NT, 1, MAXS>& r, const float* xs, int K, float eps, const bf16_t* bias,
                                                   unsigned* gvec, unsigned tag, int n, int cw, int lane, EngOut& eo, RM rm) {
    eng_gemv_rows<NT, 1, MAXS, PRO_RMSNORM, EPI_STORE>(r, xs, K, eps, bias, nullptr, eo.vals, 0, n, cw, lane, rm);
    __builtin_amdgcn_fence(__ATOMIC_RELEASE, "workgroup", "local");
    int old = 0;
    if (lane == 0) old = __hip_atomic_fetch_add((eng_lds_int)eo.count, 1, __ATOMIC_RELAXED, __HIP_MEMORY_SCOPE_WORKGROUP);
    old = __builtin_amdgcn_readfirstlane(old);
    eo.seq += 1;
    if (old + 1 == eo.seq * ENG_CW) {
        __builtin_amdgcn_fence(__ATOMIC_ACQUIRE, "workgroup", "local");
        if (lane < n) eng_put_local(gvec, rm(lane), eo.vals[lane], tag);
    }
}

template <int NT, int RPU, int MAXS, int PRO, int EPI, bool PK3 = false>
__device__ __forceinline__ void eng_gemv(const EngW<NT, RPU, MAXS>& r, const float* xs, int K, float eps, const bf16_t* bias,
                                         const float* resid, unsigned* gout, unsigned tag, float* plain, int u_lo, int u_hi,
                                         int cw, int lane, EngOut& eo) {
    eng_gemv_rows<NT, RPU, MAXS, PRO, EPI>(r, xs, K, eps, bias, resid, eo.vals, u_lo, u_hi, cw, lane);
    __builtin_amdgcn_fence(__ATOMIC_RELEASE, "workgroup", "local");
    int old = 0;
    if (lane == 0) old = __hip_atomic_fetch_add((eng_lds_int)eo.count, 1, __ATOMIC_RELAXED, __HIP_MEMORY_SCOPE_WORKGROUP);
    old = __builtin_amdgcn_readfirstlane(old);
    eo.seq += 1;
    if (old + 1 == eo.seq * ENG_CW) {
        __builtin_amdgcn_fence(__ATOMIC_ACQUIRE, "workgroup", "local");
        const int n = u_hi - u_lo;
        if constexpr (PK3) {
            if (lane * 3 < n) {
                const unsigned w0 = (__float_as_uint(eo.vals[3 * lane]) >> 16) | (__float_as_uint(eo.vals[3 * lane + 1]) & 0xffff0000u);
                const unsigned w1 = (__float_as_uint(eo.vals[3 * lane + 2]) >> 16) | (tag << 16);
                __hip_atomic_store((eng_gu64*)(reinterpret_cast<unsigned long long*>(gout) + (u_lo / 3 + lane)),
                                   ((unsigned long long)w1 << 32) | w0, ENG_RLX);
            }
        } else if (lane < n) {
            const float o = eo.vals[lane];
            eng_put(gout, lane, o, tag);
            if (plain) plain[u_lo + lane] = o;
        }
    }
}

template <int NT, int RPU, int MAXS, int PRO, int EPI>
__device__ __forceinline__ void eng_gemv_rows2(const EngW<NT, RPU, MAXS>& r, const float* xs0, const float* xs1, int K, float eps,
                                               const bf16_t* bias, const float* resid0, const float* resid1, float* vals0, float* vals1,
                                               int u_lo, int u_hi, int cw, int lane) {
    static_assert(EPI == EPI_SWIGLU ? RPU == 2 : RPU == 1, "a unit is a (w1, w3) pair for SwiGLU, one row otherwise");
    if (u_lo + cw < u_hi) {
        float xv[2][NT][8];
#pragma unroll
        for (int q = 0; q < 2; ++q) {
            const float* xs = q ? xs1 : xs0;
#pragma unroll
            for (int t = 0; t < NT; ++t) {
                const float4 f0 = *reinterpret_cast<const float4*>(xs + t * 512 + lane * 8);
                const float4 f1 = *reinterpret_cast<const float4*>(xs + t * 512 + lane * 8 + 4);
                xv[q][t][0] = f0.x; xv[q][t][1] = f0.y; xv[q][t][2] = f0.z; xv[q][t][3] = f0.w;
                xv[q][t][4] = f1.x; xv[q][t][5] = f1.y; xv[q][t][6] = f1.z; xv[q][t][7] = f1.w;
            }
        }
        if (PRO == PRO_RMSNORM) {
#pragma unroll
            for (int q = 0; q < 2; ++q) {
                float ss = 0.f;
#pragma unroll
                for (int t = 0; t < NT; ++t)
#pragma unroll
                    for (int j = 0; j < 8; ++j) ss = fmaf(xv[q][t][j], xv[q][t][j], ss);
                ss = wave_sum(ss);
                const float inv = rsqrt_exact(ss / (float)K + eps);
#pragma unroll
                for (int t = 0; t < NT; ++t) {
                    float gv[8];
                    Vec<bf16_t>::unpack(r.gain[t], gv);
#pragma unroll
                    for (int j = 0; j < 8; ++j) xv[q][t][j] = round_bf16(round_bf16(xv[q][t][j] * inv) * gv[j]);
                }
            }
        }
#pragma unroll
        for (int s = 0; s < MAXS; ++s) {
            const int u = u_lo + cw + s * ENG_CW;
            if (u >= u_hi) break;
            float acc[2][RPU];
#pragma unroll
            for (int rr = 0; rr < RPU; ++rr) {
                float a0 = 0.f, a1 = 0.f;
#pragma unroll
                for (int t = 0; t < NT; ++t) {
                    float wv[8];
                    Vec<bf16_t>::unpack(r.w[s][rr][t], wv);
#pragma unroll
                    for (int j = 0; j < 8; ++j) { a0 = fmaf(wv[j], xv[0][t][j], a0); a1 = fmaf(wv[j], xv[1][t][j], a1); }
                }
                acc[0][rr] = wave_sum(a0);
                acc[1][rr] = wave_sum(a1);
            }
#pragma unroll
            for (int q = 0; q < 2; ++q) {
                float o;
                if (EPI == EPI_SWIGLU) {
                    const float a = round_bf16(acc[q][0]);
                    const float bb = round_bf16(acc[q][RPU - 1]);
                    const float sg = round_bf16(a / (1.0f + expf(-a)));
                    o = round_bf16(sg * bb);
                } else {
                    float v = acc[q][0];
                    if (bias) v += eng_ldg_bf16(bias, u);
                    v = round_bf16(v);
                    if (EPI == EPI_RESID) v = round_bf16((q ? resid1 : resid0)[u] + v);
                    o = v;
                }
                if (lane == 0) (q ? vals1 : vals0)[u - u_lo] = o;
            }
        }
    }
}

template <int NT, int RPU, int MAXS, int PRO, int EPI>
__device__ __forceinline__ void eng_gemv2(const EngW<NT, RPU, MAXS>& r, const float* xs0, const float* xs1, int K, float eps,
                                          const bf16_t* bias, const float* resid0, const float* resid1, unsigned* gout0, unsigned* gout1,
                                          unsigned tag0, unsigned tag1, int u_lo, int u_hi, int cw, int lane, EngOut& eo) {
    if (NT <= 2) {
        eng_gemv_rows2<NT, RPU, MAXS, PRO, EPI>(r, xs0, xs1, K, eps, bias, resid0, resid1, eo.vals, eo.vals + 32, u_lo, u_hi, cw, lane);
    } else {
        eng_gemv_rows<NT, RPU, MAXS, PRO, EPI>(r, xs0, K, eps, bias, resid0, eo.vals, u_lo, u_hi, cw, lane);
        __builtin_amdgcn_sched_barrier(0);
        eng_gemv_rows<NT, RPU, MAXS, PRO, EPI>(r, xs1, K, eps, bias, resid1, eo.vals + 32, u_lo, u_hi, cw, lane);
    }
    __builtin_amdgcn_fence(__ATOMIC_RELEASE, "workgroup", "local");
    int old = 0;
    if (lane == 0) old = __hip_atomic_fetch_add((eng_lds_int)eo.count, 1, __ATOMIC_RELAXED, __HIP_MEMORY_SCOPE_WORKGROUP);
    old = __builtin_amdgcn_readfirstlane(old);
    eo.seq += 1;
    if (old + 1 == eo.seq * ENG_CW) {
        __builtin_amdgcn_fence(__ATOMIC_ACQUIRE, "workgroup", "local");
        const int n = u_hi - u_lo;
        const int i = lane & 31;
        if (i < n) {
            const float o = eo.vals[lane];
            eng_put(lane < 32 ? gout0 : gout1, i, o, lane < 32 ? tag0 : tag1);
        }
    }
}

__device__ __forceinline__ void eng_units(int U, int b, int nb, int& lo, int& hi) {
    lo = (int)((long)U * b / nb);
    hi = (int)((long)U * (b + 1) / nb);
}

struct SlowEngP {
    const EngLayer* layers;
    int n_layer;
    int D, H, Hkv, hd, F, qkvN;
    float eps, scale;
    const bf16_t* emb; const bf16_t* cb_emb; const int* toks; long tok_row_stride;
    int ncb, cbsize, vocab, sem_begin, sem_end, scale_cb; float inv_div;
    const float* rope; const int* pos; int pos_off; int n_slots, nsplit;
    size_t cache_off;
    unsigned* gx;
    unsigned* gqkv;
    unsigned long long* gpart;
    unsigned* gy;
    unsigned* gxb;
    unsigned* gg;
    unsigned* ctl;
    long rep_delta0, rep_stride;
    float* x_out;
    int nt;
    unsigned long long* stamps;
};
#define ENG_STAMP(k) do { if (p.stamps && tid == 0) p.stamps[((size_t)b * p.n_layer + li) * 16 + (k)] = eng_rt(); } while (0)
#define ENG_ASTAMP(wv, k) do { if (p.stamps && gw == (wv) && lane == 0) \
    p.stamps[((size_t)nb * p.n_layer + (size_t)b * p.n_layer + li) * 16 + (k)] = eng_rt(); } while (0)

constexpr int ENG_KVST = 6;

__device__ __forceinline__ int eng_att_role(int b, int nb, int li, int natt) {
    int a = b - (int)(((unsigned)li * (unsigned)natt) % (unsigned)nb);
    if (a < 0) a += nb;
    return a < natt ? a : -1;
}

template <typename S, bool XL = false>
__global__ __launch_bounds__(ENG_THREADS) void slow_engine_kernel(SlowEngP p) {
    constexpr int NTD = S::NTD, NTA = S::NTA, NTF = S::NTF, G = S::G;
    constexpr int SQ = S::SQ, SF = S::SF, SO = S::SO;
    extern __shared__ __attribute__((aligned(16))) float smem[];
    const int tid = threadIdx.x, lane = tid & 63, wave = __builtin_amdgcn_readfirstlane(tid >> 6);
    const int b = blockIdx.x;
    constexpr int nb = ENG_NB;
    const int cw = wave;
    const int gw = wave - ENG_CW;
    const int atid = tid - ENG_CW * 64;
    constexpr int D = S::D, F = S::F, hd = S::HDIM, hp = hd >> 1, H = S::H, Hkv = S::HKV, HD = H * hd, QKVN = (H + 2 * Hkv) * hd;
    static_assert(!XL || (ENG_NB % Hkv == 0 && QKVN % ENG_NB == 0), "XCD-local attention: the workgroups of an XCD share one kv head's rows");
    float* xA = smem;
    float* yS = xA + D;
    float* xB = yS + HD;
    float* gS = xB + D;
    float* qS = gS + F;
    float* q_s = qS + (G + 2) * hd;
    float* k_new = q_s + G * hd;
    float* v_new = k_new + hd;
    constexpr int LPP = hd >> 3, PPW = 64 / LPP, NSLOT = 4 * PPW;
    float* ml_s = v_new + hd;
    float* acc_s = ml_s + NSLOT * G * 2;
    float* mscr = acc_s + NSLOT * G * hd;
    float* outS = mscr + 64 * 6;
    int* dead = reinterpret_cast<int*>(outS + ENG_MAX_OUT);
    int* out_count = dead + 1;
    int* reg_s = dead + 4;
    if (tid == 0) { *dead = eng_fault_here(p.ctl, 0u, b) ? 1 : 0; *out_count = 0; }
    if (tid == ENG_CW * 64) {
        reg_s[0] = 0; reg_s[1] = 0; reg_s[2] = 1;
        if (XL || p.rep_stride) eng_register(p.ctl, nb, reg_s, dead);
        if (XL && (reg_s[2] * Hkv != nb || reg_s[0] >= Hkv || reg_s[1] >= reg_s[2] || p.nsplit != reg_s[2])) {
            if (!__hip_atomic_load((eng_gu32*)(p.ctl + ENG_CTL_ABORT), ENG_RLX)) __hip_atomic_store((eng_gu32*)(p.ctl + ENG_CTL_WHERE), 9998u, ENG_RLX);
            __hip_atomic_store((eng_gu32*)(p.ctl + ENG_CTL_ABORT), 1u, ENG_RLX);
            reg_s[0] = 0; reg_s[1] = 0;
            *dead = 1;
        }
    }
    const unsigned epoch = __hip_atomic_load((eng_gu32*)(p.ctl + ENG_CTL_EPOCH), ENG_RLX);
    const int pos = p.pos[0] + p.pos_off;
    unsigned long long clk0 = 0, rt0 = 0;
    if (p.stamps) { clk0 = __builtin_amdgcn_s_memtime(); rt0 = eng_rt(); }
    const size_t VSTR = (size_t)nb * ENG_LINE;
    const EngLayout layD{D / nb}, layF{F / nb}, layQ{QKVN / nb}, layLin{0};
    const int nsplit = XL ? nb / Hkv : p.nsplit;
    const int natt = Hkv * nsplit;
    const int chunk = (pos + nsplit) / nsplit;
    const int grp = lane / LPP, gl = lane % LPP;

    {
        const int* tk = p.toks;
        int t0 = tk[0];
        const bool is_vq = t0 >= p.sem_begin && t0 <= p.sem_end;
        t0 = min(max(t0, 0), p.vocab - 1);
        for (int d = tid; d < D; d += ENG_THREADS) {
            float vq = 0.f;
            if (is_vq) {
                constexpr int MAXCB = 16;
                for (int i0 = 0; i0 < p.ncb; i0 += MAXCB) {
                    int c[MAXCB];
                    float e[MAXCB];
#pragma unroll
                    for (int i = 0; i < MAXCB; ++i) c[i] = i0 + i < p.ncb ? tk[(size_t)(i0 + i + 1) * p.tok_row_stride] : 0;
#pragma unroll
                    for (int i = 0; i < MAXCB; ++i) {
                        const int cc = min(max(c[i], 0), p.cbsize - 1);
                        e[i] = i0 + i < p.ncb ? ld_elem(p.cb_emb, (size_t)(cc + (i0 + i) * p.cbsize) * D + d) : 0.f;
                    }
#pragma unroll
                    for (int i = 0; i < MAXCB; ++i) if (i0 + i < p.ncb) vq += e[i];
                }
                vq = round_bf16(vq);
            }
            float x = round_bf16(ld_elem(p.emb, (size_t)t0 * D + d) + vq);
            if (p.scale_cb && is_vq) x = round_bf16(x / p.inv_div);
            xA[d] = x;
        }
    }

    if (wave < ENG_CW) {
        int q_lo, q_hi, o_lo, o_hi, f_lo, f_hi, d_lo, d_hi;
        eng_units(QKVN, b, nb, q_lo, q_hi);
        if (XL) { q_lo = 0; q_hi = QKVN / nb; }
        eng_units(D, b, nb, o_lo, o_hi);
        eng_units(F, b, nb, f_lo, f_hi);
        eng_units(D, b, nb, d_lo, d_hi);
        EngW<NTD, 1, SQ> wq;
        EngW<NTA, 1, SO> wo;
        EngW<NTD, 2, SF> wf;
        EngW<NTF, 1, SO> wd;
        EngOut eo{outS, out_count, 0};
        {
            const EngLayer l0 = eng_layer(p.layers, 0);
            if (!XL) eng_issue(wq, l0.wqkv, l0.attn_norm, D, q_lo, q_hi, cw, lane, p.nt);
            eng_issue(wo, l0.wo, (const bf16_t*)nullptr, HD, o_lo, o_hi, cw, lane, p.nt);
            eng_issue(wf, l0.w13, l0.ffn_norm, D, f_lo, f_hi, cw, lane, p.nt);
            eng_issue(wd, l0.w2, (const bf16_t*)nullptr, F, d_lo, d_hi, cw, lane, p.nt);
            __builtin_amdgcn_sched_barrier(0);
        }
        eng_barrier();
        const int xnq = G * hd * Hkv / nb, xnk = hd * Hkv / nb;
        const EngRowQkvX rmq{reg_s[0] * G * hd + reg_s[1] * xnq, (H + reg_s[0]) * hd + reg_s[1] * xnk,
                             (H + Hkv + reg_s[0]) * hd + reg_s[1] * xnk, xnq, xnk};
        if (XL) {
            const EngLayer l0 = eng_layer(p.layers, 0);
            eng_issue(wq, l0.wqkv, l0.attn_norm, D, q_lo, q_hi, cw, lane, p.nt, rmq);
            __builtin_amdgcn_sched_barrier(0);
        }
        eng_barrier();
        for (int li = 0; li < p.n_layer; ++li) {
            const int par = li & 1, parn = (li + 1) & 1;
            const unsigned tag = eng_tag16(epoch + (unsigned)li);
            const unsigned tagn = eng_tag16(epoch + (unsigned)li + 1u);
            const EngLayer l = eng_layer(p.layers, li);
            const bool more = li + 1 < p.n_layer;
            const EngLayer ln = eng_layer(p.layers, more ? li + 1 : li);
            if (li > 0) { eng_barrier(); if (*dead) break; }
            ENG_STAMP(0);
            if (XL)
                eng_gemv_qkv_local<NTD, SQ>(wq, xA, D, p.eps, l.bqkv, p.gqkv + (size_t)par * VSTR, tag, q_hi, cw, lane, eo, rmq);
            else
                eng_gemv<NTD, 1, SQ, PRO_RMSNORM, EPI_STORE>(wq, xA, D, p.eps, l.bqkv, nullptr, p.gqkv + (size_t)par * VSTR + eng_pub(b, q_lo), tag, nullptr,
                                                             q_lo, q_hi, cw, lane, eo);
            __builtin_amdgcn_sched_barrier(0);
            ENG_STAMP(1);
            if (more) {
                if (XL) eng_issue(wq, ln.wqkv, ln.attn_norm, D, q_lo, q_hi, cw, lane, p.nt, rmq);
                else eng_issue(wq, ln.wqkv, ln.attn_norm, D, q_lo, q_hi, cw, lane, p.nt);
            }
            __builtin_amdgcn_sched_barrier(0);
            if (XL || eng_att_role(b, nb, li, natt) >= 0) {
                eng_barrier(); if (*dead) break;
                eng_barrier();
                eng_barrier();
            }
            ENG_STAMP(2);
            eng_barrier(); if (*dead) break;
            ENG_STAMP(3);
            eng_gemv<NTA, 1, SO, PRO_NONE, EPI_RESID>(wo, yS, HD, p.eps, l.bo, xA, p.gxb + (size_t)par * VSTR + eng_pub(b, o_lo), tag, nullptr, o_lo, o_hi, cw, lane, eo);
            __builtin_amdgcn_sched_barrier(0);
            ENG_STAMP(4);
            if (p.stamps && (p.nt & 2)) { asm volatile("s_waitcnt vmcnt(0)" ::: "memory"); ENG_STAMP(9); }
            if (more) eng_issue(wo, ln.wo, (const bf16_t*)nullptr, HD, o_lo, o_hi, cw, lane, p.nt);
            __builtin_amdgcn_sched_barrier(0);
            eng_barrier(); if (*dead) break;
            ENG_STAMP(5);
            eng_gemv<NTD, 2, SF, PRO_RMSNORM, EPI_SWIGLU, S::PK3>(wf, xB, D, p.eps, nullptr, nullptr,
                                                                   p.gg + (size_t)par * VSTR + (S::PK3 ? 0 : eng_pub(b, f_lo)), tag, nullptr, f_lo, f_hi, cw, lane, eo);
            __builtin_amdgcn_sched_barrier(0);
            ENG_STAMP(6);
            if (more) eng_issue(wf, ln.w13, ln.ffn_norm, D, f_lo, f_hi, cw, lane, p.nt);
            __builtin_amdgcn_sched_barrier(0);
            eng_barrier(); if (*dead) break;
            ENG_STAMP(7);
            eng_gemv<NTF, 1, SO, PRO_NONE, EPI_RESID>(wd, gS, F, p.eps, nullptr, xB, p.gx + (size_t)parn * VSTR + eng_pub(b, d_lo), tagn,
                                                      li == p.n_layer - 1 ? p.x_out : nullptr, d_lo, d_hi, cw, lane, eo);
            __builtin_amdgcn_sched_barrier(0);
            ENG_STAMP(8);
            if (more) eng_issue(wd, ln.w2, (const bf16_t*)nullptr, F, d_lo, d_hi, cw, lane, p.nt);
            __builtin_amdgcn_sched_barrier(0);
            if (!(p.nt & 2)) ENG_STAMP(9);
        }
    } else {
        U4 kpf[ENG_KVST], vpf[ENG_KVST];
        float gq0 = 1.f, gq1 = 1.f, gk0 = 1.f, gk1 = 1.f;
        int att_next = -1;
        int plan_layer = -1;
        const bf16_t *plan_kc = nullptr, *plan_vc = nullptr, *plan_qn = nullptr, *plan_kn = nullptr;
        const int period = (natt > 0 && nb % natt == 0) ? nb / natt : 0;
        int x_role = 0;
        auto role = [&](int layer) { return XL ? x_role : eng_att_role(b, nb, layer, natt); };
        auto kv_plan = [&](int from_layer) {
            plan_layer = -1;
            if (from_layer >= p.n_layer) return;
            if (XL) {
                plan_layer = from_layer;
            } else if (period > 0) {
                const int phase = b / natt;
                int d = phase - from_layer % period;
                if (d < 0) d += period;
                if (from_layer + d < p.n_layer) plan_layer = from_layer + d;
            } else {
                for (int l2 = from_layer; l2 < p.n_layer; ++l2)
                    if (role(l2) >= 0) { plan_layer = l2; break; }
            }
            if (plan_layer < 0) return;
            const EngLayer l2 = eng_layer(p.layers, plan_layer);
            plan_kc = l2.kc; plan_vc = l2.vc; plan_qn = l2.qn; plan_kn = l2.kn;
        };
        auto kv_issue = [&]() {
            att_next = plan_layer;
#pragma unroll
            for (int st = 0; st < ENG_KVST; ++st) { kpf[st] = U4{0u, 0u, 0u, 0u}; vpf[st] = U4{0u, 0u, 0u, 0u}; }
            if (att_next < 0) return;
            const int a = role(att_next);
            const int kvh = a / nsplit, split = a % nsplit;
            const int lo = split * chunk, hi = min(lo + chunk, pos + 1);
            if (lane < hp) {
                if (plan_qn) { gq0 = eng_ldg_bf16(plan_qn, 2 * lane); gq1 = eng_ldg_bf16(plan_qn, 2 * lane + 1); }
                if (plan_kn) { gk0 = eng_ldg_bf16(plan_kn, 2 * lane); gk1 = eng_ldg_bf16(plan_kn, 2 * lane + 1); }
            }
            const bf16_t* kc = plan_kc + p.cache_off + (size_t)kvh * p.n_slots * hd;
            const bf16_t* vc = plan_vc + p.cache_off + (size_t)kvh * p.n_slots * hd;
#pragma unroll
            for (int st = 0; st < ENG_KVST; ++st) {
                const int j = lo + st * NSLOT + gw * PPW + grp;
                if (j < hi && j != pos) {
                    kpf[st] = eng_ldg16<false>(kc + (size_t)j * hd + gl * 8);
                    vpf[st] = eng_ldg16<false>(vc + (size_t)j * hd + gl * 8);
                }
            }
        };
        if (!XL) { kv_plan(0); kv_issue(); }
        eng_barrier();
        const EngRelay rl{p.rep_stride != 0, reg_s[1], reg_s[2], p.rep_delta0 + (long)reg_s[0] * p.rep_stride};
        if (XL) { x_role = reg_s[0] * nsplit + reg_s[1]; kv_plan(0); kv_issue(); }
        float rope_c = 1.f, rope_s = 0.f;
        if (lane < hp) { rope_c = p.rope[((size_t)pos * hp + lane) * 2]; rope_s = p.rope[((size_t)pos * hp + lane) * 2 + 1]; }
        eng_barrier();
        for (int li = 0; li < p.n_layer; ++li) {
            const int par = li & 1;
            const unsigned tag = eng_tag16(epoch + (unsigned)li), tag32 = eng_tag32(epoch + (unsigned)li);
            const EngLayer l = eng_layer(p.layers, li);
            if (li > 0) {
                eng_gather_x(rl, p.gx + (size_t)par * VSTR, layD, 0, D, tag, xA, gw, ENG_GW, lane, p.ctl, dead, li * 8 + 0);
                eng_barrier(); if (*dead) break;
            }
            const int a = role(li);
            if (a >= 0) {
                kv_plan(li + 1);
                const int kvh = a / nsplit, split = a % nsplit;
                const int lo = split * chunk;
                const int hi = min(lo + chunk, pos + 1);
                bf16_t* kc = l.kc + p.cache_off + (size_t)kvh * p.n_slots * hd;
                bf16_t* vc = l.vc + p.cache_off + (size_t)kvh * p.n_slots * hd;
                const int slot = gw * PPW + grp;
                const unsigned* gq = p.gqkv + (size_t)par * VSTR;
                ENG_ASTAMP(0, 0);
                constexpr int QFL = XL ? 2 : 0;
                if (gw == 0) eng_gather<EngIdent, QFL>(gq, layQ, kvh * G * hd, G * hd, tag, qS, 0, 1, lane, p.ctl, dead, li * 8 + 1);
                if (gw == 1) eng_gather<EngIdent, QFL>(gq, layQ, (H + kvh) * hd, hd, tag, qS + G * hd, 0, 1, lane, p.ctl, dead, li * 8 + 1);
                if (gw == 2) eng_gather<EngIdent, QFL>(gq, layQ, (H + Hkv + kvh) * hd, hd, tag, qS + (G + 1) * hd, 0, 1, lane, p.ctl, dead, li * 8 + 1);
                eng_barrier(); if (*dead) break;
                ENG_ASTAMP(0, 1);
                if (gw >= 0) {
                    for (int item = gw; item < G + 2; item += 4) {
                        const float* src = qS + item * hd;
                        const bf16_t* gain = item < G ? l.qn : (item == G ? l.kn : nullptr);
                        float* dst = item < G ? q_s + item * hd : (item == G ? k_new : v_new);
                        if (item == G + 1) {
                            for (int e = lane; e < hd; e += 64) dst[e] = src[e];
                        } else {
                            float x0 = 0.f, x1 = 0.f;
                            if (lane < hp) { x0 = src[2 * lane]; x1 = src[2 * lane + 1]; }
                            if (gain) {
                                const float ss = wave_sum(x0 * x0 + x1 * x1);
                                const float inv = rsqrt_exact(ss / (float)hd + p.eps);
                                if (lane < hp) {
                                    const bool have = att_next == li;
                                    const float g0 = have ? (item < G ? gq0 : gk0) : eng_ldg_bf16(gain, 2 * lane);
                                    const float g1 = have ? (item < G ? gq1 : gk1) : eng_ldg_bf16(gain, 2 * lane + 1);
// ... 30 lines not shown
                        for (int e = 0; e < 8; ++e) acc[g][e] = 0.f;
                    }
                    auto step = [&](const int j, const float (&kv)[8], const float (&vv)[8]) {
                        const bool valid = j < hi;
#pragma unroll
                        for (int g = 0; g < G; ++g) {
                            float d = 0.f;
#pragma unroll
                            for (int e = 0; e < 8; ++e) d = fmaf(qr[g][e], kv[e], d);
                            if (LPP > 1) d = group_sum_rt(d, LPP);
                            if (valid) {
                                const float s = d * p.scale;
                                const float mn = fmaxf(mrun[g], s);
                                const float corr = expf(mrun[g] - mn);
                                const float pj = expf(s - mn);
                                lrun[g] = lrun[g] * corr + pj;
#pragma unroll
                                for (int e = 0; e < 8; ++e) acc[g][e] = acc[g][e] * corr + pj * vv[e];
                                mrun[g] = mn;
                            }
                        }
                    };
                    const bool pre = att_next == li;
                    for (int blk = 0; lo + gw * PPW + blk * (ENG_KVST * NSLOT) < hi; ++blk) {
#pragma unroll
                        for (int st = 0; st < ENG_KVST; ++st) {
                            const int base = lo + gw * PPW + (blk * ENG_KVST + st) * NSLOT;
                            if (base < hi) {
                                const int j = base + grp;
                                float kv[8], vv[8];
                                if (j < hi && j == pos) {
#pragma unroll
                                    for (int e = 0; e < 8; ++e) { kv[e] = k_new[gl * 8 + e]; vv[e] = v_new[gl * 8 + e]; }
                                } else if (pre || blk > 0) {
                                    Vec<bf16_t>::unpack(kpf[st], kv); Vec<bf16_t>::unpack(vpf[st], vv);
                                } else if (j < hi) {
                                    Vec<bf16_t>::unpack(eng_ldg16<false>(kc + (size_t)j * hd + gl * 8), kv);
                                    Vec<bf16_t>::unpack(eng_ldg16<false>(vc + (size_t)j * hd + gl * 8), vv);
                                } else {
#pragma unroll
                                    for (int e = 0; e < 8; ++e) { kv[e] = 0.f; vv[e] = 0.f; }
                                }
                                const int jn = j + ENG_KVST * NSLOT;
                                if (jn < hi && jn != pos) {
                                    kpf[st] = eng_ldg16<false>(kc + (size_t)jn * hd + gl * 8);
                                    vpf[st] = eng_ldg16<false>(vc + (size_t)jn * hd + gl * 8);
                                } else {
                                    kpf[st] = U4{0u, 0u, 0u, 0u}; vpf[st] = U4{0u, 0u, 0u, 0u};
                                }
                                step(j, kv, vv);
                            }
                        }
                    }
                    ENG_ASTAMP(0, 7);
#pragma unroll
                    for (int g = 0; g < G; ++g) {
                        if (gl == 0) { ml_s[(slot * G + g) * 2] = mrun[g]; ml_s[(slot * G + g) * 2 + 1] = lrun[g]; }
#pragma unroll
                        for (int e = 0; e < 8; ++e) acc_s[(size_t)(slot * G + g) * hd + gl * 8 + e] = acc[g][e];
                    }
                    ENG_ASTAMP(0, 8);
                }
                eng_barrier();
                ENG_ASTAMP(0, 3);
                if (gw >= 0) {
                    const bool quick = NSLOT == 16 && (hd & 63) == 0;
                    for (int idx0 = gw * 64; idx0 < G * hd; idx0 += 256) {
                        const int idx = idx0 + lane;
                        const int g = quick ? idx0 / hd : idx / hd, e = idx % hd;
                        float M = -INFINITY, L = 0.f, O = 0.f;
                        if (quick) {
                            const int sl = lane & 15;
                            const float m_l = ml_s[(sl * G + g) * 2], l_l = ml_s[(sl * G + g) * 2 + 1];
                            M = m_l;
                            M = fmaxf(M, dpp_f<DPP_XOR1>(M));
                            M = fmaxf(M, dpp_f<DPP_XOR2>(M));
                            M = fmaxf(M, dpp_f<DPP_HALF_MIRROR>(M));
                            M = fmaxf(M, dpp_f<DPP_MIRROR>(M));
                            if (M > -INFINITY) {
                                const float w_l = expf(m_l - M);
#pragma unroll
                                for (int s2 = 0; s2 < 16; ++s2) {
                                    const float w = lane_f(w_l, s2);
                                    L += lane_f(l_l, s2) * w;
                                    O += acc_s[(size_t)(s2 * G + g) * hd + e] * w;
                                }
                            }
                        } else if (idx < G * hd) {
                            for (int s2 = 0; s2 < NSLOT; ++s2) M = fmaxf(M, ml_s[(s2 * G + g) * 2]);
                            if (M > -INFINITY) {
                                for (int s2 = 0; s2 < NSLOT; ++s2) {
                                    const float w = expf(ml_s[(s2 * G + g) * 2] - M);
                                    L += ml_s[(s2 * G + g) * 2 + 1] * w;
                                    O += acc_s[(size_t)(s2 * G + g) * hd + e] * w;
                                }
                            }
                        }
                        if (idx < G * hd) {
                            const int head = kvh * G + g;
                            if (nsplit == 1) {
                                eng_put(p.gy + (size_t)par * HD, head * hd + e, round_bf16(O / L), tag);
                            } else {
                                unsigned long long* gp = p.gpart + (((size_t)par * H + head) * nsplit + split) * (hd + 2);
                                if (XL) {
                                    eng_put64_local(gp, e, O, tag32);
                                    if (e == 0) { eng_put64_local(gp, hd, M, tag32); eng_put64_local(gp, hd + 1, L, tag32); }
                                } else {
                                    eng_put64(gp, e, O, tag32);
                                    if (e == 0) { eng_put64(gp, hd, M, tag32); eng_put64(gp, hd + 1, L, tag32); }
                                }
                            }
                        }
                    }
                }
                ENG_ASTAMP(0, 4);
                if (XL && gw == 3 && nsplit == 32 && hd == 128 && G == 2) {
                    const int item = lane >> 5, s = lane & 31, e = split * 4;
                    const int head = kvh * G + item;
                    const unsigned long long* gs = p.gpart + (((size_t)par * H + head) * nsplit + s) * (hd + 2);
                    EngSpin sp{p.ctl, dead, 0, 0, li * 8 + 2};
                    U4 A, B, C;
                    bool alive = true;
                    for (;;) {
                        eng_ld3_sc1<2>(gs + e, gs + e + 2, gs + hd, A, B, C);
                        const bool ok = A.y == tag32 && A.w == tag32 && B.y == tag32 && B.w == tag32 && C.y == tag32 && C.w == tag32;
                        if (__all(ok)) break;
                        if (sp.give_up(lane)) { alive = false; break; }
                    }
                    ENG_ASTAMP(3, 5);
                    if (alive) {
                        const float m_ = __uint_as_float(C.x), l_ = __uint_as_float(C.z);
                        float Mc = m_;
                        Mc = fmaxf(Mc, dpp_f<DPP_XOR1>(Mc));
                        Mc = fmaxf(Mc, dpp_f<DPP_XOR2>(Mc));
                        Mc = fmaxf(Mc, dpp_f<DPP_HALF_MIRROR>(Mc));
                        float* mx = mscr;
                        float* pr = mscr + 8;
                        if ((lane & 7) == 0) mx[lane >> 3] = Mc;
                        __builtin_amdgcn_wave_barrier();
                        __builtin_amdgcn_fence(__ATOMIC_ACQ_REL, "wavefront");
                        float Mrun = -INFINITY;
                        const int ch = s >> 3;
#pragma unroll
                        for (int c = 0; c < 4; ++c) if (c <= ch) Mrun = fmaxf(Mrun, mx[item * 4 + c]);
                        const float w = m_ > -INFINITY ? expf(m_ - Mrun) : 0.f;
                        float* q5 = pr + (size_t)(item * 32 + s) * 5;
                        q5[0] = l_ * w;
                        q5[1] = __uint_as_float(A.x) * w; q5[2] = __uint_as_float(A.z) * w;
                        q5[3] = __uint_as_float(B.x) * w; q5[4] = __uint_as_float(B.z) * w;
                        __builtin_amdgcn_wave_barrier();
                        __builtin_amdgcn_fence(__ATOMIC_ACQ_REL, "wavefront");
                        const int ci = (lane >> 3) & 1, cq = lane & 7;
                        float acc = 0.f;
                        {
                            const float* src = pr + (size_t)ci * 32 * 5 + (cq < 5 ? cq : 0);
                            float v[32];
#pragma unroll
                            for (int k = 0; k < 32; ++k) v[k] = src[k * 5];
                            float mc[4], rr[4];
#pragma unroll
                            for (int c = 0; c < 4; ++c) mc[c] = mx[ci * 4 + c];
                            float M = -INFINITY;
#pragma unroll
                            for (int c = 0; c < 4; ++c) {
                                const float Mn = fmaxf(M, mc[c]);
                                rr[c] = (c > 0 && M > -INFINITY && mc[c] > -INFINITY) ? expf(M - Mn) : 1.0f;
                                M = Mn;
                            }
#pragma unroll
                            for (int c = 0; c < 4; ++c) {
                                acc *= rr[c];
#pragma unroll
                                for (int k = 0; k < 8; ++k) acc += v[c * 8 + k];
                            }
                        }
                        const float a0 = dpp_f<0x101>(acc), a1 = dpp_f<0x102>(acc), a2 = dpp_f<0x103>(acc), a3 = dpp_f<0x104>(acc);
                        if (lane == 0 || lane == 8) {
                            unsigned* gy = p.gy + (size_t)par * HD + (size_t)a * (G * 4) + ci * 4;
                            eng_put4(gy, round_bf16(a0 / acc), round_bf16(a1 / acc), round_bf16(a2 / acc), round_bf16(a3 / acc), tag);
                        }
                    }
                    ENG_ASTAMP(3, 6);
                } else
                if (nsplit > 1 && gw == 3) {
                    const int epb = hd / nsplit;
                    const int e4n = epb >> 2;
                    const int nitem = G * e4n;
                    EngSpin sp{p.ctl, dead, 0, 0, li * 8 + 2};
                    bool alive = true;
                    for (int ib = 0; ib < nitem && alive; ib += 8) {
                        const int it = ib + (lane >> 3), s8 = lane & 7;
                        const bool item_on = it < nitem;
                        const int g = item_on ? it / e4n : 0;
                        const int e = split * epb + (item_on ? (it % e4n) * 4 : 0);
                        const int head = kvh * G + g;
                        const unsigned long long* gp = p.gpart + ((size_t)par * H + head) * nsplit * (hd + 2);
                        float M = -INFINITY, L = 0.f, a0 = 0.f, a1 = 0.f, a2 = 0.f, a3 = 0.f;
                        for (int c0 = 0; c0 < nsplit && alive; c0 += 8) {
                            const bool son = item_on && c0 + s8 < nsplit;
                            const unsigned long long* gs = gp + (size_t)(son ? c0 + s8 : 0) * (hd + 2);
                            U4 A, B, C;
                            for (;;) {
                                eng_ld3_sc1(gs + e, gs + e + 2, gs + hd, A, B, C);
                                const bool ok = !son || (A.y == tag32 && A.w == tag32 && B.y == tag32 && B.w == tag32 &&
                                                         C.y == tag32 && C.w == tag32);
                                if (__all(ok)) break;
                                if (sp.give_up(lane)) { alive = false; break; }
                            }
                            if (!alive) break;
                            if (ib + 8 >= nitem && c0 + 8 >= nsplit) ENG_ASTAMP(3, 5);
                            const float m_ = son ? __uint_as_float(C.x) : -INFINITY;
                            const float l_ = son ? __uint_as_float(C.z) : 0.f;
                            float Mc = m_;
                            Mc = fmaxf(Mc, dpp_f<DPP_XOR1>(Mc));
                            Mc = fmaxf(Mc, dpp_f<DPP_XOR2>(Mc));
                            Mc = fmaxf(Mc, dpp_f<DPP_HALF_MIRROR>(Mc));
                            if (Mc > -INFINITY) {
                                const float Mn = fmaxf(M, Mc);
                                if (c0 > 0 && M > -INFINITY) {
                                    const float rr = expf(M - Mn);
                                    L *= rr; a0 *= rr; a1 *= rr; a2 *= rr; a3 *= rr;
                                }
                                M = Mn;
                                const float w = m_ > -INFINITY ? expf(m_ - M) : 0.f;
                                const float pl = l_ * w;
                                const float p0 = __uint_as_float(A.x) * w, p1 = __uint_as_float(A.z) * w;
                                const float p2 = __uint_as_float(B.x) * w, p3 = __uint_as_float(B.z) * w;
                                L += pl; a0 += p0; a1 += p1; a2 += p2; a3 += p3;
#define ENG_MSTEP(n) L += dpp_f<0x100 + n>(pl); a0 += dpp_f<0x100 + n>(p0); a1 += dpp_f<0x100 + n>(p1); \
                     a2 += dpp_f<0x100 + n>(p2); a3 += dpp_f<0x100 + n>(p3);
                                ENG_MSTEP(1) ENG_MSTEP(2) ENG_MSTEP(3) ENG_MSTEP(4) ENG_MSTEP(5) ENG_MSTEP(6) ENG_MSTEP(7)
#undef ENG_MSTEP
                            }
                        }
                        if (alive && s8 == 0 && item_on) {
                            unsigned* gy = p.gy + (size_t)par * HD + (size_t)a * (G * epb) + g * epb + (e - split * epb);
                            eng_put4(gy, round_bf16(a0 / L), round_bf16(a1 / L), round_bf16(a2 / L), round_bf16(a3 / L), tag);
                        }
                    }
                    ENG_ASTAMP(3, 6);
                }
            }
            {
                const int epb = hd / nsplit, ns = nsplit;
                auto ymap = [=](int i) { const int a2 = i / (G * epb), r2 = i % (G * epb), g2 = r2 / epb, eo = r2 % epb;
                                         return ((a2 / ns) * G + g2) * hd + (a2 % ns) * epb + eo; };
                eng_gather_x(rl, p.gy + (size_t)par * HD, layLin, 0, HD, tag, yS, gw, ENG_GW, lane, p.ctl, dead, li * 8 + 3, ymap);
            }
            eng_barrier(); if (*dead) break;
            if (a >= 0) kv_issue();
            const unsigned long long t_poll0 = p.stamps ? eng_rt() : 0ull;
            eng_gather_x(rl, p.gxb + (size_t)par * VSTR, layD, 0, D, tag, xB, gw, ENG_GW, lane, p.ctl, dead, li * 8 + 4, EngIdent(),
                       (p.stamps && gw == 0) ? p.stamps + ((size_t)b * p.n_layer + li) * 16 + 13 : nullptr);
            const unsigned long long t_poll1 = p.stamps ? eng_rt() : 0ull;
            eng_barrier(); if (*dead) break;
            if (p.stamps && tid == ENG_CW * 64) {
                unsigned long long* q = p.stamps + ((size_t)b * p.n_layer + li) * 16;
                q[10] = t_poll0; q[11] = t_poll1; q[12] = eng_rt();
            }
            if constexpr (S::PK3) eng_gather3_x(rl, p.gg + (size_t)par * VSTR, F, tag, gS, gw, ENG_GW, lane, p.ctl, dead, li * 8 + 5);
            else eng_gather_x(rl, p.gg + (size_t)par * VSTR, layF, 0, F, tag, gS, gw, ENG_GW, lane, p.ctl, dead, li * 8 + 5);
            eng_barrier(); if (*dead) break;
        }
    }

    eng_barrier();
    if (p.stamps && tid == 0 && b == 0) {
        p.stamps[14] = __builtin_amdgcn_s_memtime() - clk0; p.stamps[15] = eng_rt() - rt0;
    }
    if (tid == 0) {
        const unsigned old = atomicAdd(p.ctl + ENG_CTL_EXIT, 1u);
        if (old + 1 == (unsigned)nb) {
            __hip_atomic_store((eng_gu32*)(p.ctl + ENG_CTL_EXIT), 0u, ENG_RLX);
            __hip_atomic_store((eng_gu32*)(p.ctl + ENG_CTL_ARRIVED), 0u, ENG_RLX);
            for (int x = 0; x < 8; ++x) __hip_atomic_store((eng_gu32*)(p.ctl + ENG_CTL_XCD + x), 0u, ENG_RLX);
            __hip_atomic_store((eng_gu32*)(p.ctl + ENG_CTL_EPOCH), epoch + ENG_EPOCH_STEP, ENG_RLX);
        }
    }
}

struct FastEngP {
    const EngLayer* layers;
    int n_layer, ncb;
    int D, H, Hkv, hd, F, qkvN, V;
    float eps, scale;
    const float* rope;
    const bf16_t* fast_norm; const bf16_t* fast_out; const bf16_t* fast_emb;
    const float* hid;
    const float* femb;
    unsigned* gx;
    unsigned* gqkv;
    unsigned* gxb;
    unsigned* gg;
    unsigned* glog;
    unsigned* gcode;
    unsigned* ctl;
    long rep_delta0, rep_stride;
    SampP samp;
    long noise_cb_stride;
    long noise_off1;
    int pair;
    const bf16_t* qkv0_tab;
    unsigned long long* stamps;
};
#define ENG_FSTAMP(k) do { if (p.stamps && tid == 0) p.stamps[(((size_t)b * p.ncb + cb) * nL + li) * 16 + (k)] = eng_rt(); } while (0)

#define ENG_GSTAMP(k) do { if (p.stamps && atid == 0) p.stamps[(((size_t)b * p.ncb + cb) * nL + nL - 1) * 16 + (k)] = eng_rt(); } while (0)
constexpr int ENG_FV = 1024;

struct EngSub {
    int* end_at;
    int n;
    __device__ __forceinline__ void sync(int) { ++n; eng_barrier(); }
};
__device__ __forceinline__ void eng_draw_follow(const int* end_at) {
    for (int c = 1;; ++c) {
        eng_barrier();
        if (*reinterpret_cast<const volatile int*>(end_at) == c) break;
    }
}

template <int MAXCB, int HD>
__device__ __forceinline__ void eng_fast_attn(const float* qkvS, bf16_t* kS, bf16_t* vS, float* yS, const bf16_t* qn, const bf16_t* kn,
                                              const float (&cs)[2], const float (&sn)[2], int c, int ncb, int H, int Hkv, float eps, float scale,
                                              int w, int nw, int lane) {
    constexpr int EPL = HD > 64 ? 2 : 1;
    const int G = H / Hkv;
    for (int h = w; h < H; h += nw) {
        const int kvh = h / G;
        bf16_t* kh = kS + (size_t)kvh * ncb * HD + lane;
        bf16_t* vh = vS + (size_t)kvh * ncb * HD + lane;
        const float* qp = qkvS + h * HD + lane;
        const float* kp = qkvS + (H + kvh) * HD + lane;
        const float* vp = qkvS + (H + Hkv + kvh) * HD + lane;
        float q[EPL], kx[EPL], vx[EPL];
#pragma unroll
        for (int e = 0; e < EPL; ++e) { q[e] = qp[64 * e]; kx[e] = kp[64 * e]; vx[e] = vp[64 * e]; }
        if (c == 0) {
            if (h % G == 0) {
                if (kn) {
                    float ss = kx[0] * kx[0];
                    if (EPL > 1) ss = kx[0] * kx[0] + kx[EPL - 1] * kx[EPL - 1];
                    ss = wave_sum(ss);
                    const float inv = rsqrt_exact(ss / (float)HD + eps);
#pragma unroll
                    for (int e = 0; e < EPL; ++e) kx[e] = round_bf16((kx[e] * inv) * eng_ldg_bf16(kn, lane + 64 * e));
                }
#pragma unroll
                for (int e = 0; e < EPL; ++e) {
                    const float ko = dpp_f<DPP_XOR1>(kx[e]);
                    kx[e] = round_bf16((lane & 1) == 0 ? kx[e] * cs[e] - ko * sn[e] : kx[e] * cs[e] + ko * sn[e]);
                    kh[64 * e] = f32_to_bf16_bits(kx[e]); vh[64 * e] = f32_to_bf16_bits(vx[e]);
                }
            }
#pragma unroll
            for (int e = 0; e < EPL; ++e) yS[h * HD + lane + 64 * e] = round_bf16(vx[e]);
            continue;
        }
        if (qn) {
            float ss = q[0] * q[0];
            if (EPL > 1) ss = q[0] * q[0] + q[EPL - 1] * q[EPL - 1];
            ss = wave_sum(HD < 64 ? (lane < HD ? ss : 0.f) : ss);
            const float inv = rsqrt_exact(ss / (float)HD + eps);
#pragma unroll
            for (int e = 0; e < EPL; ++e) q[e] = round_bf16((q[e] * inv) * eng_ldg_bf16(qn, lane + 64 * e));
        }
        if (kn) {
            float ss = kx[0] * kx[0];
            if (EPL > 1) ss = kx[0] * kx[0] + kx[EPL - 1] * kx[EPL - 1];
            ss = wave_sum(ss);
            const float inv = rsqrt_exact(ss / (float)HD + eps);
#pragma unroll
            for (int e = 0; e < EPL; ++e) kx[e] = round_bf16((kx[e] * inv) * eng_ldg_bf16(kn, lane + 64 * e));
        }
#pragma unroll
        for (int e = 0; e < EPL; ++e) {
            const float qo = dpp_f<DPP_XOR1>(q[e]), ko = dpp_f<DPP_XOR1>(kx[e]);
            const bool even = (lane & 1) == 0;
            q[e] = round_bf16(even ? q[e] * cs[e] - qo * sn[e] : q[e] * cs[e] + qo * sn[e]);
            kx[e] = round_bf16(even ? kx[e] * cs[e] - ko * sn[e] : kx[e] * cs[e] + ko * sn[e]);
        }
        if (h % G == 0) {
#pragma unroll
            for (int e = 0; e < EPL; ++e) { kh[c * HD + 64 * e] = f32_to_bf16_bits(kx[e]); vh[c * HD + 64 * e] = f32_to_bf16_bits(vx[e]); }
        }
        float sl = -INFINITY;
        float mx = -INFINITY;
#pragma unroll
        for (int j = 0; j < MAXCB; ++j) {
            if (j <= c) {
                float pr;
                if (EPL > 1) {
                    const float k0 = j == c ? kx[0] : bf16_bits_to_f32(kh[j * HD]), k1 = j == c ? kx[EPL - 1] : bf16_bits_to_f32(kh[j * HD + 64 * (EPL - 1)]);
                    pr = fmaf(q[EPL - 1], k1, q[0] * k0);
                } else {
                    const float k0 = j == c ? kx[0] : bf16_bits_to_f32(kh[j * HD]);
                    pr = fmaf(0.f, 0.f, q[0] * k0);
                }
                const float d = wave_sum(pr);
                const float sj = round_bf16(round_bf16(d) * scale);
                mx = fmaxf(mx, sj);
                if (lane == j) sl = sj;
            }
        }
        const float el = lane <= c ? expf(sl - mx) : 0.f;
        float sum = 0.f;
#pragma unroll
        for (int j = 0; j < MAXCB; ++j)
            if (j <= c) sum += lane_f(el, j);
        const float pl = lane <= c ? round_bf16(el / sum) : 0.f;
        float o[EPL];
#pragma unroll
        for (int e = 0; e < EPL; ++e) o[e] = 0.f;
#pragma unroll
        for (int j = 0; j < MAXCB; ++j) {
            if (j <= c) {
                const float pj = lane_f(pl, j);
#pragma unroll
                for (int e = 0; e < EPL; ++e) o[e] = fmaf(pj, j == c ? vx[e] : bf16_bits_to_f32(vh[j * HD + 64 * e]), o[e]);
            }
        }
#pragma unroll
        for (int e = 0; e < EPL; ++e) yS[h * HD + lane + 64 * e] = round_bf16(o[e]);
    }
}

constexpr int DPP_ROW_SHL4 = 0x104, DPP_ROW_SHL8 = 0x108, DPP_ROW_SHL12 = 0x10C;
template <int MAXCB, int GQ>
__device__ __forceinline__ void eng_fast_attn64(const float* qkvS, bf16_t* kS, bf16_t* vS, float* yS, const bf16_t* qn, const bf16_t* kn,
                                                float cs, float sn, int c, int ncb, int H, int Hkv, float eps, float scale,
                                                int w, int nw, int lane) {
    constexpr int HD = 64;
    const bool even = (lane & 1) == 0;
    const int r = lane >> 4, k4 = (lane & 15) * 4;
    for (int kvh = w; kvh < Hkv; kvh += nw) {
        bf16_t* kh = kS + (size_t)kvh * ncb * HD;
        bf16_t* vh = vS + (size_t)kvh * ncb * HD;
        float kx = qkvS[(H + kvh) * HD + lane];
        const float vx = qkvS[(H + Hkv + kvh) * HD + lane];
        float* slot = yS + (size_t)kvh * GQ * HD;
        float q[GQ];
#pragma unroll
        for (int g = 0; g < GQ; ++g) q[g] = qkvS[(kvh * GQ + g) * HD + lane];
        if (kn) {
            const float ss = wave_sum(kx * kx);
            const float inv = rsqrt_exact(ss / (float)HD + eps);
            kx = round_bf16((kx * inv) * eng_ldg_bf16(kn, lane));
        }
        {
            const float ko = dpp_f<DPP_XOR1>(kx);
            kx = round_bf16(even ? kx * cs - ko * sn : kx * cs + ko * sn);
        }
        kh[c * HD + lane] = f32_to_bf16_bits(kx);
        vh[c * HD + lane] = f32_to_bf16_bits(vx);
        if (c == 0) {
#pragma unroll
            for (int g = 0; g < GQ; ++g) slot[g * HD + lane] = round_bf16(vx);
            continue;
        }
#pragma unroll
        for (int g = 0; g < GQ; ++g) {
            if (qn) {
                const float ss = wave_sum(q[g] * q[g]);
                const float inv = rsqrt_exact(ss / (float)HD + eps);
                q[g] = round_bf16((q[g] * inv) * eng_ldg_bf16(qn, lane));
            }
            const float qo = dpp_f<DPP_XOR1>(q[g]);
            q[g] = round_bf16(even ? q[g] * cs - qo * sn : q[g] * cs + qo * sn);
            slot[g * HD + lane] = q[g];
        }
        __builtin_amdgcn_wave_barrier();
        float4 q4[GQ];
#pragma unroll
        for (int g = 0; g < GQ; ++g) q4[g] = *reinterpret_cast<const float4*>(slot + g * HD + k4);
        __builtin_amdgcn_wave_barrier();
#pragma unroll
        for (int ps = 0; ps < (MAXCB + 3) / 4; ++ps) {
            if (ps * 4 <= c) {
                const int j = ps * 4 + r;
                const int jj = j <= c ? j : c;
                const uint2 kb = *reinterpret_cast<const uint2*>(kh + jj * HD + k4);
                const float k0 = __uint_as_float(kb.x << 16), k1 = __uint_as_float(kb.x & 0xffff0000u);
                const float k2 = __uint_as_float(kb.y << 16), k3 = __uint_as_float(kb.y & 0xffff0000u);
#pragma unroll
                for (int g = 0; g < GQ; ++g) {
                    const float p0 = fmaf(0.f, 0.f, q4[g].x * k0), p1 = fmaf(0.f, 0.f, q4[g].y * k1);
                    const float p2 = fmaf(0.f, 0.f, q4[g].z * k2), p3 = fmaf(0.f, 0.f, q4[g].w * k3);
                    float sdot = (p0 + p1) + (p2 + p3);
                    sdot += dpp_f<DPP_XOR1>(sdot);
                    sdot += dpp_f<DPP_XOR2>(sdot);
                    float a = sdot + dpp_f<DPP_ROW_SHL4>(sdot);
                    a = a + dpp_f<DPP_ROW_SHL8>(sdot);
                    a = a + dpp_f<DPP_ROW_SHL12>(sdot);
                    const float sj = round_bf16(round_bf16(a) * scale);
                    if ((lane & 15) == 0 && j <= c) slot[g * HD + j] = sj;
                }
            }
        }
        __builtin_amdgcn_wave_barrier();
        float sl[GQ], el[GQ], sum[GQ], pl[GQ], o[GQ];
#pragma unroll
        for (int g = 0; g < GQ; ++g) sl[g] = lane <= c ? slot[g * HD + lane] : -INFINITY;
        __builtin_amdgcn_wave_barrier();
#pragma unroll
        for (int g = 0; g < GQ; ++g) {
            float mx = sl[g];
            mx = fmaxf(mx, dpp_f<DPP_XOR1>(mx));
            mx = fmaxf(mx, dpp_f<DPP_XOR2>(mx));
            mx = fmaxf(mx, dpp_f<DPP_HALF_MIRROR>(mx));
            mx = fmaxf(mx, dpp_f<DPP_MIRROR>(mx));
            mx = lane_f(mx, 0);
            el[g] = lane <= c ? expf(sl[g] - mx) : 0.f;
            sum[g] = 0.f; o[g] = 0.f;
        }
#pragma unroll
        for (int j = 0; j < MAXCB; ++j)
            if (j <= c) {
#pragma unroll
                for (int g = 0; g < GQ; ++g) sum[g] += lane_f(el[g], j);
            }
#pragma unroll
        for (int g = 0; g < GQ; ++g) pl[g] = lane <= c ? round_bf16(el[g] / sum[g]) : 0.f;
#pragma unroll
        for (int j = 0; j < MAXCB; ++j)
            if (j <= c) {
                const float vj = bf16_bits_to_f32(vh[j * HD + lane]);
#pragma unroll
                for (int g = 0; g < GQ; ++g) o[g] = fmaf(lane_f(pl[g], j), vj, o[g]);
            }
#pragma unroll
        for (int g = 0; g < GQ; ++g) slot[g * HD + lane] = round_bf16(o[g]);
    }
}
template <int MAXCB, int HD>
__device__ __forceinline__ void eng_fast_attn_any(const float* qkvS, bf16_t* kS, bf16_t* vS, float* yS, const bf16_t* qn, const bf16_t* kn,
                                                  const float (&cs)[2], const float (&sn)[2], int c, int ncb, int H, int Hkv, float eps,
                                                  float scale, int w, int nw, int lane) {
    if constexpr (HD == 64 && MAXCB <= 16) {
        const int G = H / Hkv;
        if (G == 2) { eng_fast_attn64<MAXCB, 2>(qkvS, kS, vS, yS, qn, kn, cs[0], sn[0], c, ncb, H, Hkv, eps, scale, w, nw, lane); return; }
        if (G == 1) { eng_fast_attn64<MAXCB, 1>(qkvS, kS, vS, yS, qn, kn, cs[0], sn[0], c, ncb, H, Hkv, eps, scale, w, nw, lane); return; }
    }
    eng_fast_attn<MAXCB, HD>(qkvS, kS, vS, yS, qn, kn, cs, sn, c, ncb, H, Hkv, eps, scale, w, nw, lane);
}

struct EngSampLds {
    float* redbuf;
    int* pen_id;
    float* pen_val;
    float* amv;
    int* ami;
    int* wcnt;
    float* prL;
    uint32_t* keyL;
    uint32_t* cut;
};
struct EngDrawPre {
    RowCtl ctl;
    int nfv;
    int pen;
    float q4[4];
};
__device__ __forceinline__ EngDrawPre eng_draw_pre(const SampP& p, int tid) {
    EngDrawPre d;
    d.ctl = p.ctl[0];
    d.nfv = p.nf[0];
    d.pen = -1;
    if (d.nfv > 0 && p.cb != 0 && tid < 16) {
        const int it = d.nfv - 1;
        const int ws = it < 16 ? 0 : it - 16;
        d.pen = p.seq[(size_t)(p.cb + 1) * p.cap + ws + 1 + tid];
    }
    const float* qrow = nullptr;
    if (p.noise && d.nfv < p.noise_rows) qrow = p.noise + (size_t)d.nfv * p.noise_row_len + p.noise_off;
    draw_noise4(p, d.ctl, qrow, 4 * tid, d.nfv, 0, ENG_FV, d.q4);
    return d;
}
__device__ __forceinline__ int eng_sample_small(const SampP& p, const EngDrawPre& pre, const float* L, const EngSampLds& S, EngSub& sub, int tid, int lane, int wave,
                                                unsigned long long* stp = nullptr) {
    constexpr int V = ENG_FV;
    const RowCtl ctl = pre.ctl;
    const int nfv = pre.nfv;
    const int R = p.ncb + 1;
    const int* seq = p.seq;
    int red_phase = 0;
    auto red_sum = [&](float v) {
        v = wave_sum(v);
        float* slot = S.redbuf + 4 * (red_phase & 1);
        ++red_phase;
        if (lane == 0) slot[wave] = v;
        sub.sync(lane);
        return ((slot[0] + slot[1]) + slot[2]) + slot[3];
    };
    const int i0 = 4 * tid;
    float l[4];
#pragma unroll
    for (int e = 0; e < 4; ++e) l[e] = (i0 + e) < V ? L[i0 + e] : -INFINITY;
    if (nfv > 0) {
        const int it = nfv - 1;
        const int ws = it < 16 ? 0 : it - 16;
        const int npen = p.cb == 0 ? R : 16;
        (void)ws;
        if (tid < npen) {
            const int id = p.cb == 0 ? seq[(size_t)tid * p.cap + ws + 1] : pre.pen;
            S.pen_id[tid] = -1;
            if (id >= 0 && id < V) {
                const float sv = L[id];
                S.pen_id[tid] = id;
                S.pen_val[tid] = sv < 0.f ? round_bf16(sv * ctl.rep) : round_bf16(sv / ctl.rep);
            }
        }
        sub.sync(lane);
        if (p.cb != 0) {
            int ids[16]; float nvs[16];
#pragma unroll
            for (int k = 0; k < 16; k += 4) {
                const int4 a = *reinterpret_cast<const int4*>(S.pen_id + k);
                const float4 v = *reinterpret_cast<const float4*>(S.pen_val + k);
                ids[k] = a.x; ids[k + 1] = a.y; ids[k + 2] = a.z; ids[k + 3] = a.w;
                nvs[k] = v.x; nvs[k + 1] = v.y; nvs[k + 2] = v.z; nvs[k + 3] = v.w;
            }
#pragma unroll
            for (int k = 0; k < 16; ++k) {
                const unsigned d = (unsigned)(ids[k] - i0);
#pragma unroll
                for (int e = 0; e < 4; ++e) if (d == (unsigned)e) l[e] = nvs[k];
            }
        } else {
            for (int k = 0; k < npen; ++k) {
                const int id = S.pen_id[k];
                if (id >= i0 && id < i0 + 4) {
                    const float nv = S.pen_val[k];
#pragma unroll
                    for (int e = 0; e < 4; ++e) if (i0 + e == id) l[e] = nv;
                }
            }
        }
    }
    if (p.cb == 0 && ctl.ban_eos && p.im_end < V) {
#pragma unroll
        for (int e = 0; e < 4; ++e) if (i0 + e == p.im_end) l[e] = -INFINITY;
    }
    int bb_phase = 0;
    auto block_best = [&](ArgMax a) {
        a = wave_argmax(a);
        float* av = S.amv + 4 * (bb_phase & 1);
        int* ai = S.ami + 4 * (bb_phase & 1);
        ++bb_phase;
        if (lane == 0) { av[wave] = a.v; ai[wave] = a.i; }
        sub.sync(lane);
        ArgMax t{av[0], ai[0]};
#pragma unroll
        for (int w = 1; w < 4; ++w) t = better(t, ArgMax{av[w], ai[w]});
        return t;
    };
    ArgMax am{-INFINITY, 0x7fffffff};
#pragma unroll
    for (int e = 0; e < 4; ++e) if (i0 + e < V) am = better(am, ArgMax{l[e], i0 + e});
    am = block_best(am);
    if (stp && tid == 0) stp[12] = eng_rt();
    const float Lmax = am.v;
    float ex[4], z = 0.f;
#pragma unroll
    for (int e = 0; e < 4; ++e) { ex[e] = (i0 + e) < V ? expf(l[e] - Lmax) : 0.f; z += ex[e]; }
    const float Z = red_sum(z);
    if (stp && tid == 0) stp[-16 + 10] = eng_rt();
    const float tp = round_bf16(ctl.top_p);
    auto removed = [&](float cum) { return round_bf16(cum) > tp; };
    constexpr uint32_t cmask = 0xffff0000u;
    uint32_t key[4];
#pragma unroll
    for (int e = 0; e < 4; ++e) {
        const bool v = (i0 + e) < V;
        key[e] = v ? (order_key(l[e]) & cmask) : 0u;
        S.prL[i0 + e] = v ? round_bf16(ex[e] / Z) : 0.f;
        S.keyL[i0 + e] = key[e];
    }
    const bool only_top = removed(round_bf16(1.0f / Z));
    int winner = am.i;
    if (!only_top) {
        sub.sync(lane);
        const float Tc = fmaxf(ctl.temperature, 1e-5f);
        const float Mt = round_bf16(Lmax / Tc);
        float etp[4];
        if (wave != 0) {
#pragma unroll
            for (int e = 0; e < 4; ++e) etp[e] = expf(round_bf16(l[e] / Tc) - Mt);
        }
        if (stp && tid == 0) stp[-16 + 11] = eng_rt();
        if (wave == 0) {
            float pr[16];
            uint32_t ky[16];
#pragma unroll
            for (int e = 0; e < 16; ++e) { pr[e] = S.prL[lane + 64 * e]; ky[e] = S.keyL[lane + 64 * e]; }
            float tot = 0.f;
#pragma unroll
            for (int e = 0; e < 16; ++e) tot += pr[e];
            tot = wave_sum(tot);
            if (stp && tid == 0) stp[-16 + 12] = eng_rt();
            uint32_t kstar = 0;
            int nk = 0, all_kept = 0;
            if (!removed(tot)) {
                all_kept = 1;
            } else {
                uint32_t kmx = 0u;
#pragma unroll
                for (int e = 0; e < 16; ++e) kmx = ky[e] > kmx ? ky[e] : kmx;
                {
                    int km = (int)(kmx >> 16);
                    km = max(km, dpp_i<DPP_XOR1>(km));
                    km = max(km, dpp_i<DPP_XOR2>(km));
                    km = max(km, dpp_i<DPP_HALF_MIRROR>(km));
                    km = max(km, dpp_i<DPP_MIRROR>(km));
                    km = max(max(__builtin_amdgcn_readlane(km, 0), __builtin_amdgcn_readlane(km, 16)),
                             max(__builtin_amdgcn_readlane(km, 32), __builtin_amdgcn_readlane(km, 48)));
                    kmx = (uint32_t)km << 16;
                }
                for (int bit = 31; bit >= 16; --bit) {
                    const uint32_t cand = kstar | (1u << bit);
                    if (cand > kmx) continue;
                    float ms = 0.f;
#pragma unroll
                    for (int e = 0; e < 16; ++e) ms += ky[e] >= cand ? pr[e] : 0.f;
                    if (removed(wave_sum(ms))) kstar = cand;
                }
                if (stp && tid == 0) stp[-16 + 13] = eng_rt();
                float above = 0.f, cnt = 0.f;
#pragma unroll
                for (int e = 0; e < 16; ++e) {
                    if (ky[e] > kstar) above += pr[e];
                    else if (ky[e] == kstar && (lane + 64 * e) < V) cnt += 1.f;
                }
                above = wave_sum(above);
                const int icnt = (int)wave_sum(cnt);
                const uint32_t ubits = (kstar & 0x80000000u) ? (kstar & 0x7fffffffu) : ~(kstar | ~cmask);
                const float pk = round_bf16(expf(__uint_as_float(ubits) - Lmax) / Z);
                int lo_n = 0, hi_n = icnt;
                while (lo_n < hi_n) {
                    const int mid = (lo_n + hi_n + 1) >> 1;
                    if (removed(fmaf((float)mid, pk, above))) hi_n = mid - 1; else lo_n = mid;
                }
                nk = lo_n;
            }
            if (stp && tid == 0) stp[-16 + 14] = eng_rt();
            if (lane == 0) { S.cut[0] = kstar; S.cut[1] = (uint32_t)nk; S.cut[2] = (uint32_t)all_kept; }
        }
        sub.sync(lane);
        if (stp && tid == 0) stp[13] = eng_rt();
        const uint32_t kstar = S.cut[0];
        const int nk = (int)S.cut[1];
        const bool all_kept = S.cut[2] != 0;
        if (wave == 0) {
#pragma unroll
            for (int e = 0; e < 4; ++e) etp[e] = expf(round_bf16(l[e] / Tc) - Mt);
        }
        bool mem[4];
        int mine = 0;
#pragma unroll
        for (int e = 0; e < 4; ++e) { mem[e] = (i0 + e) < V && !all_kept && key[e] == kstar; mine += mem[e] ? 1 : 0; }
        int below = 0, wtot = 0;
        const unsigned long long lower = (1ull << lane) - 1ull;
#pragma unroll
        for (int c = 1; c <= 4; ++c) {
            const unsigned long long bal = __ballot(mine >= c);
            below += __popcll(bal & lower);
            wtot += __popcll(bal);
        }
        if (lane == 0) S.wcnt[wave] = wtot;
        sub.sync(lane);
        int rank = below;
        for (int w = 0; w < wave; ++w) rank += S.wcnt[w];
        bool keep[4];
        float et[4], z2 = 0.f;
#pragma unroll
        for (int e = 0; e < 4; ++e) {
            keep[e] = (i0 + e) < V && (all_kept || key[e] > kstar || (mem[e] && rank < nk));
            rank += mem[e] ? 1 : 0;
            et[e] = keep[e] ? etp[e] : 0.f;
            z2 += et[e];
        }
        const float Z2 = red_sum(z2);
        ArgMax best{-1.f, 0x7fffffff};
#pragma unroll
        for (int e = 0; e < 4; ++e) {
            if (i0 + e < V) {
                const float prob = keep[e] ? round_bf16(et[e] / Z2) : 0.f;
                best = better(best, ArgMax{round_bf16(prob / round_bf16(pre.q4[e])), i0 + e});
            }
        }
        winner = block_best(best).i;
    }
    return winner;
}

template <typename S>
__global__ __launch_bounds__(ENG_CW * 64) void eng_qkv0_table_kernel(const bf16_t* wqkv, const bf16_t* bqkv, const bf16_t* attn_norm,
                                                                      const bf16_t* fast_emb, bf16_t* tab, int D, int qkvN, int ncodes,
                                                                      float eps) {
    extern __shared__ __attribute__((aligned(16))) float smem[];
    float* xs = smem;
    float* vals = xs + D;
    const int tid = threadIdx.x, lane = tid & 63, cw = tid >> 6;
    int q_lo, q_hi;
    eng_units(qkvN, blockIdx.x, gridDim.x, q_lo, q_hi);
    constexpr int NTD = S::NTD;
    EngW<NTD, 1, S::SQ> wq;
    eng_issue<false>(wq, wqkv, attn_norm, D, q_lo, q_hi, cw, lane, 0);
    const int per = (ncodes + gridDim.y - 1) / gridDim.y;
    const int c_lo = blockIdx.y * per, c_hi = min(c_lo + per, ncodes);
    for (int code = c_lo; code < c_hi; ++code) {
        for (int d = tid * 8; d < D; d += ENG_CW * 64 * 8) {
            float e8[8];
            Vec<bf16_t>::unpack(eng_ldg16<false>(fast_emb + (size_t)code * D + d), e8);
#pragma unroll
            for (int j = 0; j < 8; ++j) xs[d + j] = e8[j];
        }
        __syncthreads();
        eng_gemv_rows<NTD, 1, S::SQ, PRO_RMSNORM, EPI_STORE>(wq, xs, D, eps, bqkv, nullptr, vals, q_lo, q_hi, cw, lane);
        __syncthreads();
        if (tid < q_hi - q_lo) tab[(size_t)code * qkvN + q_lo + tid] = f32_to_bf16_bits(vals[tid]);
        __syncthreads();
    }
}

inline size_t eng_fast_lds_bytes(int D, int qkvN, int HD, int F, int V, int nL, int ncb, int KVW, bool pair) {
    size_t fl = (size_t)D * 2 + qkvN + HD + F + V + ENG_MAX_OUT + 8 + 32 + 32 + 20 + 2048 + 4 + 4 + 16;
    size_t by = fl * sizeof(float) + (size_t)nL * 2 * ncb * KVW * 2 + 64;
    if (pair) by += ((size_t)2 * D + (size_t)(F > qkvN + HD ? F : qkvN + HD)) * sizeof(float) + 16;
    return by;
}

template <typename FS, int MAXCB>
__global__ __launch_bounds__(ENG_THREADS) void fast_engine_kernel(FastEngP p) {
    constexpr int NTD = FS::NTD, NTA = FS::NTA, NTF = FS::NTF, HDIM = FS::HDIM;
    constexpr int SQ = FS::SQ, SF = FS::SF, SO = FS::SO;
    extern __shared__ __attribute__((aligned(16))) float smem[];
    const int tid = threadIdx.x, lane = tid & 63, wave = __builtin_amdgcn_readfirstlane(tid >> 6);
    const int b = blockIdx.x;
    constexpr int nb = ENG_NB;
    const int cw = wave, gw = wave - ENG_CW, atid = tid - ENG_CW * 64;
    constexpr int D = FS::D, F = FS::F, hd = HDIM, H = FS::H, Hkv = FS::HKV, HD = H * hd, KVW = Hkv * hd, QKVN = (H + 2 * Hkv) * hd, V = FS::V;
    float* xA = smem;
    float* qkvS = xA + D;
    float* yS = qkvS + QKVN;
    float* xB = yS + HD;
    float* gS = xB + D;
    float* logS = gS + F;
    float* outS = logS + V;
    float* redbuf = outS + ENG_MAX_OUT;
    int* pen_id = reinterpret_cast<int*>(redbuf + 8);
    float* pen_val = reinterpret_cast<float*>(pen_id + 32);
    float* amv = pen_val + 32;
    int* ami = reinterpret_cast<int*>(amv + 8);
    int* wcnt = ami + 8;
    float* prL = reinterpret_cast<float*>(wcnt + 4);
    uint32_t* keyL = reinterpret_cast<uint32_t*>(prL + 1024);
    uint32_t* cut = keyL + 1024;
    int* dead = reinterpret_cast<int*>(cut + 4);
    int* out_count = dead + 1;
    int* sub_count = dead + 2;
    int* codes_s = dead + 4;
    int* reg_s = codes_s + MAXCB;
    bf16_t* kvS = reinterpret_cast<bf16_t*>(reg_s + 4);
    float* xA1 = smem + ((((size_t)(reinterpret_cast<float*>(kvS + (size_t)p.n_layer * 2 * p.ncb * KVW) - smem)) + 3) & ~(size_t)3);
    float* xB1 = xA1 + D;
    float* gS1 = xB1 + D;
    float* qkvS1 = gS1;
    float* yS1 = gS1 + QKVN;
    if (tid == 0) { *dead = eng_fault_here(p.ctl, ENG_FAULT_FAST, b) ? 1 : 0; *out_count = 0; *sub_count = 0; }
    if (tid == ENG_CW * 64) {
        reg_s[0] = 0; reg_s[1] = 0; reg_s[2] = 1;
        if (p.rep_stride) eng_register(p.ctl, nb, reg_s, dead);
    }
    const unsigned epoch = __hip_atomic_load((eng_gu32*)(p.ctl + ENG_CTL_EPOCH), ENG_RLX);
    const size_t VSTR = (size_t)nb * ENG_LINE;
    const EngLayout layD{D / nb}, layF{F / nb}, layQ{QKVN / nb}, layV{V / nb};
    const int nL = p.n_layer;
    auto bx = [&](int par, int l) { return p.gx + ((size_t)par * (nL + 1) + l) * VSTR; };
    auto bq = [&](int par, int l) { return p.gqkv + ((size_t)par * nL + l) * VSTR; };
    auto bxb = [&](int par, int l) { return p.gxb + ((size_t)par * nL + l) * VSTR; };
    auto bg = [&](int par, int l) { return p.gg + ((size_t)par * nL + l) * VSTR; };
    auto blog = [&](int par) { return p.glog + (size_t)par * VSTR; };
    auto drawer = [&](int cb) { return (cb * 37) % nb; };
    bool alive = true;
    const bool pair = p.pair != 0 && p.ncb >= 2;

    if (wave < ENG_CW) {
        int q_lo, q_hi, o_lo, o_hi, f_lo, f_hi, h_lo, h_hi;
        eng_units(QKVN, b, nb, q_lo, q_hi);
        eng_units(D, b, nb, o_lo, o_hi);
        eng_units(F, b, nb, f_lo, f_hi);
        eng_units(V, b, nb, h_lo, h_hi);
        EngW<NTD, 1, SQ> wq;
        EngW<NTA, 1, SO> wo;
        EngW<NTD, 2, SF> wf;
        EngW<NTF, 1, SO> wd;
        EngW<NTD, 1, SO> wh;
        EngOut eo{outS, out_count, 0};
        {
            const EngLayer l0 = eng_layer(p.layers, 0);
            eng_issue<false>(wq, l0.wqkv, l0.attn_norm, D, q_lo, q_hi, cw, lane, 0);
            eng_issue<false>(wo, l0.wo, (const bf16_t*)nullptr, HD, o_lo, o_hi, cw, lane, 0);
            eng_issue<false>(wf, l0.w13, l0.ffn_norm, D, f_lo, f_hi, cw, lane, 0);
            eng_issue<false>(wd, l0.w2, (const bf16_t*)nullptr, F, o_lo, o_hi, cw, lane, 0);
            __builtin_amdgcn_sched_barrier(0);
        }
        eng_barrier();
        eng_barrier();
        if (pair) {
            const unsigned tag0 = eng_tag16(epoch), tag1 = eng_tag16(epoch + 1u);
            float r0c[2], r0s[2], r1c[2], r1s[2];
#pragma unroll
            for (int e = 0; e < 2; ++e) {
                const int d = lane + 64 * e;
                r0c[e] = d < hd ? p.rope[((size_t)(d >> 1)) * 2] : 1.f;
                r0s[e] = d < hd ? p.rope[((size_t)(d >> 1)) * 2 + 1] : 0.f;
                r1c[e] = d < hd ? p.rope[((size_t)(hd >> 1) + (d >> 1)) * 2] : 1.f;
                r1s[e] = d < hd ? p.rope[((size_t)(hd >> 1) + (d >> 1)) * 2 + 1] : 0.f;
            }
            for (int li = 0; li < nL; ++li) {
                const int cb = 1;
                unsigned *gxL = p.gx, *gqL = p.gqkv, *gxbL = p.gxb, *ggL = p.gg;
                asm volatile("" : "+s"(gxL), "+s"(gqL), "+s"(gxbL), "+s"(ggL));
                auto bx = [&](int par, int l_) { return gxL + ((size_t)par * (nL + 1) + l_) * VSTR; };
                auto bq = [&](int par, int l_) { return gqL + ((size_t)par * nL + l_) * VSTR; };
                auto bxb = [&](int par, int l_) { return gxbL + ((size_t)par * nL + l_) * VSTR; };
                auto bg = [&](int par, int l_) { return ggL + ((size_t)par * nL + l_) * VSTR; };
                const EngLayer l = eng_layer(p.layers, li);
                const bool more = !(p.ncb == 2 && li == nL - 1);
                const bool tail0 = li + 1 < nL;
                const EngLayer ln = eng_layer(p.layers, li + 1 < nL ? li + 1 : 0);
                bf16_t* kL = kvS + (size_t)(li * 2) * p.ncb * KVW;
                bf16_t* vL = kvS + (size_t)(li * 2 + 1) * p.ncb * KVW;
                eng_barrier(); if (*dead) { alive = false; break; }
                ENG_FSTAMP(0);
                eng_gemv2<NTD, 1, SQ, PRO_RMSNORM, EPI_STORE>(wq, xA, xA1, D, p.eps, l.bqkv, nullptr, nullptr, bq(0, li) + eng_pub(b, q_lo),
                                                              bq(1, li) + eng_pub(b, q_lo), tag0, tag1, q_lo, q_hi, cw, lane, eo);
                __builtin_amdgcn_sched_barrier(0);
                ENG_FSTAMP(1);
                if (more && !(li == nL - 1 && p.qkv0_tab != nullptr)) eng_issue<false>(wq, ln.wqkv, ln.attn_norm, D, q_lo, q_hi, cw, lane, 0);
                __builtin_amdgcn_sched_barrier(0);
                eng_barrier(); if (*dead) { alive = false; break; }
                ENG_FSTAMP(2);
                eng_fast_attn_any<MAXCB, HDIM>(qkvS, kL, vL, yS, l.qn, l.kn, r0c, r0s, 0, p.ncb, H, Hkv, p.eps, p.scale, wave, ENG_WAVES, lane);
                eng_barrier();
                eng_fast_attn_any<MAXCB, HDIM>(qkvS1, kL, vL, yS1, l.qn, l.kn, r1c, r1s, 1, p.ncb, H, Hkv, p.eps, p.scale, wave, ENG_WAVES, lane);
                ENG_FSTAMP(9);
                eng_barrier();
                ENG_FSTAMP(3);
                if (tail0)
                    eng_gemv2<NTA, 1, SO, PRO_NONE, EPI_RESID>(wo, yS, yS1, HD, p.eps, l.bo, xA, xA1, bxb(0, li) + eng_pub(b, o_lo),
                                                               bxb(1, li) + eng_pub(b, o_lo), tag0, tag1, o_lo, o_hi, cw, lane, eo);
                else
                    eng_gemv<NTA, 1, SO, PRO_NONE, EPI_RESID>(wo, yS1, HD, p.eps, l.bo, xA1, bxb(1, li) + eng_pub(b, o_lo), tag1, nullptr,
                                                              o_lo, o_hi, cw, lane, eo);
                __builtin_amdgcn_sched_barrier(0);
                ENG_FSTAMP(4);
                if (more) eng_issue<false>(wo, ln.wo, (const bf16_t*)nullptr, HD, o_lo, o_hi, cw, lane, 0);
                __builtin_amdgcn_sched_barrier(0);
                eng_barrier(); if (*dead) { alive = false; break; }
                ENG_FSTAMP(5);
                if (tail0)
                    eng_gemv2<NTD, 2, SF, PRO_RMSNORM, EPI_SWIGLU>(wf, xB, xB1, D, p.eps, nullptr, nullptr, nullptr, bg(0, li) + eng_pub(b, f_lo),
                                                                   bg(1, li) + eng_pub(b, f_lo), tag0, tag1, f_lo, f_hi, cw, lane, eo);
                else
                    eng_gemv<NTD, 2, SF, PRO_RMSNORM, EPI_SWIGLU, FS::PK3>(wf, xB1, D, p.eps, nullptr, nullptr, bg(1, li) + (FS::PK3 ? 0 : eng_pub(b, f_lo)), tag1, nullptr,
                                                                    f_lo, f_hi, cw, lane, eo);
                __builtin_amdgcn_sched_barrier(0);
                ENG_FSTAMP(6);
                if (more) eng_issue<false>(wf, ln.w13, ln.ffn_norm, D, f_lo, f_hi, cw, lane, 0);
                __builtin_amdgcn_sched_barrier(0);
                eng_barrier(); if (*dead) { alive = false; break; }
                ENG_FSTAMP(7);
                if (tail0)
                    eng_gemv2<NTF, 1, SO, PRO_NONE, EPI_RESID>(wd, gS, gS1, F, p.eps, nullptr, xB, xB1, bx(0, li + 1) + eng_pub(b, o_lo),
                                                               bx(1, li + 1) + eng_pub(b, o_lo), tag0, tag1, o_lo, o_hi, cw, lane, eo);
                else
                    eng_gemv<NTF, 1, SO, PRO_NONE, EPI_RESID>(wd, gS1, F, p.eps, nullptr, xB1, bx(1, li + 1) + eng_pub(b, o_lo), tag1, nullptr,
                                                              o_lo, o_hi, cw, lane, eo);
                __builtin_amdgcn_sched_barrier(0);
                ENG_FSTAMP(8);
                if (more) eng_issue<false>(wd, ln.w2, (const bf16_t*)nullptr, F, o_lo, o_hi, cw, lane, 0);
                if (li == nL - 1) eng_issue<false>(wh, p.fast_out, p.fast_norm, D, h_lo, h_hi, cw, lane, 0);
                __builtin_amdgcn_sched_barrier(0);
            }
            if (alive) {
                eng_barrier();
                if (*dead) alive = false;
                else {
                    eng_gemv<NTD, 1, SO, PRO_RMSNORM, EPI_STORE>(wh, xA, D, p.eps, nullptr, nullptr, blog(1) + eng_pub(b, h_lo), tag1, nullptr,
                                                                 h_lo, h_hi, cw, lane, eo);
                    __builtin_amdgcn_sched_barrier(0);
                    eng_draw_follow(sub_count);
                }
            }
        }
        for (int cb = pair ? 2 : 0; cb < p.ncb && alive; ++cb) {
            const int par = cb & 1;
            const unsigned tag = eng_tag16(epoch + (unsigned)cb);
            float rcs[2], rsn[2];
#pragma unroll
            for (int e = 0; e < 2; ++e) {
                const int d = lane + 64 * e;
                rcs[e] = d < hd ? p.rope[((size_t)cb * (hd >> 1) + (d >> 1)) * 2] : 1.f;
                rsn[e] = d < hd ? p.rope[((size_t)cb * (hd >> 1) + (d >> 1)) * 2 + 1] : 0.f;
            }
            const bool tab0 = p.qkv0_tab != nullptr && cb >= 2;
            for (int li = 0; li < nL; ++li) {
                const EngLayer l = eng_layer(p.layers, li);
                const bool more = !(cb == p.ncb - 1 && li == nL - 1);
                const EngLayer ln = eng_layer(p.layers, li + 1 < nL ? li + 1 : 0);
                eng_barrier(); if (*dead) { alive = false; break; }
                ENG_FSTAMP(0);
                if (!(li == 0 && tab0))
                    eng_gemv<NTD, 1, SQ, PRO_RMSNORM, EPI_STORE>(wq, xA, D, p.eps, l.bqkv, nullptr, bq(par, li) + eng_pub(b, q_lo), tag,
                                                                 nullptr, q_lo, q_hi, cw, lane, eo);
                __builtin_amdgcn_sched_barrier(0);
                ENG_FSTAMP(1);
                if (more && !(li == nL - 1 && p.qkv0_tab != nullptr && cb + 1 >= 2))
                    eng_issue<false>(wq, ln.wqkv, ln.attn_norm, D, q_lo, q_hi, cw, lane, 0);
                __builtin_amdgcn_sched_barrier(0);
                eng_barrier(); if (*dead) { alive = false; break; }
                ENG_FSTAMP(2);
                eng_fast_attn_any<MAXCB, HDIM>(qkvS, kvS + (size_t)(li * 2) * p.ncb * KVW, kvS + (size_t)(li * 2 + 1) * p.ncb * KVW, yS, l.qn, l.kn,
                                         rcs, rsn, cb, p.ncb, H, Hkv, p.eps, p.scale, wave, ENG_WAVES, lane);
                ENG_FSTAMP(9);
                eng_barrier();
                ENG_FSTAMP(3);
                eng_gemv<NTA, 1, SO, PRO_NONE, EPI_RESID>(wo, yS, HD, p.eps, l.bo, xA, bxb(par, li) + eng_pub(b, o_lo), tag, nullptr,
                                                          o_lo, o_hi, cw, lane, eo);
                __builtin_amdgcn_sched_barrier(0);
                ENG_FSTAMP(4);
                if (more) eng_issue<false>(wo, ln.wo, (const bf16_t*)nullptr, HD, o_lo, o_hi, cw, lane, 0);
                __builtin_amdgcn_sched_barrier(0);
                eng_barrier(); if (*dead) { alive = false; break; }
                ENG_FSTAMP(5);
                eng_gemv<NTD, 2, SF, PRO_RMSNORM, EPI_SWIGLU, FS::PK3>(wf, xB, D, p.eps, nullptr, nullptr, bg(par, li) + (FS::PK3 ? 0 : eng_pub(b, f_lo)), tag, nullptr,
                                                                f_lo, f_hi, cw, lane, eo);
                __builtin_amdgcn_sched_barrier(0);
                ENG_FSTAMP(6);
                if (more) eng_issue<false>(wf, ln.w13, ln.ffn_norm, D, f_lo, f_hi, cw, lane, 0);
                __builtin_amdgcn_sched_barrier(0);
                eng_barrier(); if (*dead) { alive = false; break; }
                ENG_FSTAMP(7);
                eng_gemv<NTF, 1, SO, PRO_NONE, EPI_RESID>(wd, gS, F, p.eps, nullptr, xB, bx(par, li + 1) + eng_pub(b, o_lo), tag, nullptr,
                                                          o_lo, o_hi, cw, lane, eo);
                __builtin_amdgcn_sched_barrier(0);
                ENG_FSTAMP(8);
                if (more) eng_issue<false>(wd, ln.w2, (const bf16_t*)nullptr, F, o_lo, o_hi, cw, lane, 0);
                if (li == nL - 1 && cb >= 1) eng_issue<false>(wh, p.fast_out, p.fast_norm, D, h_lo, h_hi, cw, lane, 0);
                __builtin_amdgcn_sched_barrier(0);
            }
            if (!alive) break;
            if (cb >= 1) {
                eng_barrier(); if (*dead) { alive = false; break; }
                eng_gemv<NTD, 1, SO, PRO_RMSNORM, EPI_STORE>(wh, xA, D, p.eps, nullptr, nullptr, blog(par) + eng_pub(b, h_lo), tag, nullptr,
                                                             h_lo, h_hi, cw, lane, eo);
                __builtin_amdgcn_sched_barrier(0);
                eng_draw_follow(sub_count);
            }
        }
    } else {
        EngSub sub{sub_count, 0};
        SampP sp = p.samp;
        int prev_code = 0;
        eng_barrier();
        const EngRelay rl{p.rep_stride != 0, reg_s[1], reg_s[2], p.rep_delta0 + (long)reg_s[0] * p.rep_stride};
        eng_barrier();
        if (pair) {
            const unsigned tag0 = eng_tag16(epoch), tag1 = eng_tag16(epoch + 1u);
            float r0c[2], r0s[2], r1c[2], r1s[2];
#pragma unroll
            for (int e = 0; e < 2; ++e) {
                const int d = lane + 64 * e;
                r0c[e] = d < hd ? p.rope[((size_t)(d >> 1)) * 2] : 1.f;
                r0s[e] = d < hd ? p.rope[((size_t)(d >> 1)) * 2 + 1] : 0.f;
                r1c[e] = d < hd ? p.rope[((size_t)(hd >> 1) + (d >> 1)) * 2] : 1.f;
                r1s[e] = d < hd ? p.rope[((size_t)(hd >> 1) + (d >> 1)) * 2 + 1] : 0.f;
            }
            for (int li = 0; li < nL; ++li) {
                const EngLayer l = eng_layer(p.layers, li);
                const bool tail0 = li + 1 < nL;
                const int wh = 1000 + 64 + li * 8;
                bf16_t* kL = kvS + (size_t)(li * 2) * p.ncb * KVW;
                bf16_t* vL = kvS + (size_t)(li * 2 + 1) * p.ncb * KVW;
                if (li > 0) {
                    eng_gather_x2(rl, EngSrc2{{bx(0, li), bx(1, li)}, {xA, xA1}, {tag0, tag1}}, D, gw, ENG_GW, lane, p.ctl, dead, wh + 0);
                } else {
                    for (int d = atid * 4; d < D; d += ENG_GW * 64 * 4) {
                        *reinterpret_cast<float4*>(xA + d) = *reinterpret_cast<const float4*>(p.hid + d);
                        *reinterpret_cast<float4*>(xA1 + d) = *reinterpret_cast<const float4*>(p.femb + d);
                    }
                }
                eng_barrier(); if (*dead) { alive = false; break; }
                eng_gather_x2(rl, EngSrc2{{bq(0, li), bq(1, li)}, {qkvS, qkvS1}, {tag0, tag1}}, QKVN, gw, ENG_GW, lane, p.ctl, dead, wh + 1);
                eng_barrier(); if (*dead) { alive = false; break; }
                eng_fast_attn_any<MAXCB, HDIM>(qkvS, kL, vL, yS, l.qn, l.kn, r0c, r0s, 0, p.ncb, H, Hkv, p.eps, p.scale, wave, ENG_WAVES, lane);
                eng_barrier();
                eng_fast_attn_any<MAXCB, HDIM>(qkvS1, kL, vL, yS1, l.qn, l.kn, r1c, r1s, 1, p.ncb, H, Hkv, p.eps, p.scale, wave, ENG_WAVES, lane);
                eng_barrier();
                if (tail0) eng_gather_x2(rl, EngSrc2{{bxb(0, li), bxb(1, li)}, {xB, xB1}, {tag0, tag1}}, D, gw, ENG_GW, lane, p.ctl, dead, wh + 2);
                else eng_gather_x(rl, bxb(1, li), layD, 0, D, tag1, xB1, gw, ENG_GW, lane, p.ctl, dead, wh + 2);
                eng_barrier(); if (*dead) { alive = false; break; }
                if (tail0) eng_gather_x2(rl, EngSrc2{{bg(0, li), bg(1, li)}, {gS, gS1}, {tag0, tag1}}, F, gw, ENG_GW, lane, p.ctl, dead, wh + 3);
                else if constexpr (FS::PK3) eng_gather3_x(rl, bg(1, li), F, tag1, gS1, gw, ENG_GW, lane, p.ctl, dead, wh + 3);
                else eng_gather_x(rl, bg(1, li), layF, 0, F, tag1, gS1, gw, ENG_GW, lane, p.ctl, dead, wh + 3);
                eng_barrier(); if (*dead) { alive = false; break; }
            }
        }
        for (int cb = pair ? 1 : 0; cb < p.ncb && alive; ++cb) {
            const int par = cb & 1;
            const unsigned tag = eng_tag16(epoch + (unsigned)cb);
            float rcs[2], rsn[2];
#pragma unroll
            for (int e = 0; e < 2; ++e) {
                const int d = lane + 64 * e;
                rcs[e] = d < hd ? p.rope[((size_t)cb * (hd >> 1) + (d >> 1)) * 2] : 1.f;
                rsn[e] = d < hd ? p.rope[((size_t)cb * (hd >> 1) + (d >> 1)) * 2 + 1] : 0.f;
            }
            EngDrawPre pre{};
            if (cb >= 1) {
                sp.cb = cb;
                sp.noise_off = p.noise_off1 + (long)(cb - 1) * p.noise_cb_stride;
                pre = eng_draw_pre(sp, atid);
            }
            for (int li = (pair && cb == 1) ? nL : 0; li < nL; ++li) {
                const EngLayer l = eng_layer(p.layers, li);
                if (li > 0) {
                    eng_gather_x(rl, bx(par, li), layD, 0, D, tag, xA, gw, ENG_GW, lane, p.ctl, dead, 1000 + cb * 64 + li * 8 + 0);
                } else if (cb <= 1) {
                    const float* src = cb == 0 ? p.hid : p.femb;
                    for (int d = atid * 4; d < D; d += ENG_GW * 64 * 4) *reinterpret_cast<float4*>(xA + d) = *reinterpret_cast<const float4*>(src + d);
                } else {
                    const int code = prev_code;
                    const int d0 = atid * 8;
                    if (p.qkv0_tab && D <= ENG_GW * 64 * 8 && QKVN <= ENG_GW * 64 * 8) {
                        const U4 ue = eng_ldg16<false>(p.fast_emb + (size_t)code * D + (d0 < D ? d0 : 0));
                        const U4 uq = eng_ldg16<false>(p.qkv0_tab + (size_t)code * QKVN + (d0 < QKVN ? d0 : 0));
                        float e8[8], q8[8];
                        Vec<bf16_t>::unpack(ue, e8);
                        Vec<bf16_t>::unpack(uq, q8);
                        if (d0 < D) {
#pragma unroll
                            for (int j = 0; j < 8; ++j) xA[d0 + j] = e8[j];
                        }
                        if (d0 < QKVN) {
#pragma unroll
                            for (int j = 0; j < 8; ++j) qkvS[d0 + j] = q8[j];
                        }
                    } else {
                        for (int d = d0; d < D; d += ENG_GW * 64 * 8) {
                            float e8[8];
                            Vec<bf16_t>::unpack(eng_ldg16<false>(p.fast_emb + (size_t)code * D + d), e8);
#pragma unroll
                            for (int j = 0; j < 8; ++j) xA[d + j] = e8[j];
                        }
                        if (p.qkv0_tab) {
                            for (int d = d0; d < QKVN; d += ENG_GW * 64 * 8) {
                                float e8[8];
                                Vec<bf16_t>::unpack(eng_ldg16<false>(p.qkv0_tab + (size_t)code * QKVN + d), e8);
#pragma unroll
                                for (int j = 0; j < 8; ++j) qkvS[d + j] = e8[j];
                            }
                        }
                    }
                }
                eng_barrier(); if (*dead) { alive = false; break; }
                if (!(li == 0 && cb >= 2 && p.qkv0_tab))
                    eng_gather_x(rl, bq(par, li), layQ, 0, QKVN, tag, qkvS, gw, ENG_GW, lane, p.ctl, dead, 1000 + cb * 64 + li * 8 + 1);
                eng_barrier(); if (*dead) { alive = false; break; }
                eng_fast_attn_any<MAXCB, HDIM>(qkvS, kvS + (size_t)(li * 2) * p.ncb * KVW, kvS + (size_t)(li * 2 + 1) * p.ncb * KVW, yS, l.qn, l.kn,
                                         rcs, rsn, cb, p.ncb, H, Hkv, p.eps, p.scale, wave, ENG_WAVES, lane);
                eng_barrier();
                eng_gather_x(rl, bxb(par, li), layD, 0, D, tag, xB, gw, ENG_GW, lane, p.ctl, dead, 1000 + cb * 64 + li * 8 + 2);
                eng_barrier(); if (*dead) { alive = false; break; }
                if constexpr (FS::PK3) eng_gather3_x(rl, bg(par, li), F, tag, gS, gw, ENG_GW, lane, p.ctl, dead, 1000 + cb * 64 + li * 8 + 3);
                else eng_gather_x(rl, bg(par, li), layF, 0, F, tag, gS, gw, ENG_GW, lane, p.ctl, dead, 1000 + cb * 64 + li * 8 + 3);
                eng_barrier(); if (*dead) { alive = false; break; }
            }
            if (!alive) break;
            if (cb >= 1) {
                eng_gather_x(rl, bx(par, nL), layD, 0, D, tag, xA, gw, ENG_GW, lane, p.ctl, dead, 1000 + cb * 64 + 56);
                eng_barrier(); if (*dead) { alive = false; break; }
                ENG_GSTAMP(10);
                {
                    eng_gather_x(rl, blog(par), layV, 0, V, tag, logS, gw, ENG_GW, lane, p.ctl, dead, 1000 + cb * 64 + 57);
                    sub.n = 0;
                    if (atid == 0) *sub_count = *dead ? 1 : 0;
                    sub.sync(lane);
                    ENG_GSTAMP(11);
                    if (*reinterpret_cast<volatile int*>(sub_count) == 0) {
                        const int last = cb == p.ncb - 1;
                        const int nfv = pre.nfv;
                        EngSampLds S{redbuf, pen_id, pen_val, amv, ami, wcnt, prL, keyL, cut};
                        const int code = eng_sample_small(sp, pre, logS, S, sub, atid, lane, gw,
                                                          p.stamps ? p.stamps + (((size_t)b * p.ncb + cb) * nL + nL - 1) * 16 : nullptr);
                        ENG_GSTAMP(14);
                        const int R = p.ncb + 1;
                        if (atid == 0) { codes_s[cb] = code; *sub_count = sub.n + 1; }
                        sub.sync(lane);
                        prev_code = code;
                        if (b == drawer(cb)) {
                            if (atid == 0) sp.tokn[cb + 1] = code;
                            if (last) {
                                const int frozen = sp.done[0];
                                if (atid < R) {
                                    const int v = atid < 2 ? sp.tokn[atid] : (atid - 1 == cb ? code : codes_s[atid - 1]);
                                    sp.tok[atid] = v;
                                    if (nfv < sp.cap && !frozen) sp.seq[(size_t)atid * sp.cap + nfv] = v;
                                }
                                if (atid == 0 && !frozen) {
                                    sp.pos[0] += 1;
                                    sp.nf[0] = nfv + 1;
                                    if (sp.tokn[0] == sp.im_end) sp.done[0] = 1;
                                }
                            }
                        }
                    }
                }
            }
        }
    }

    eng_barrier();
    if (tid == 0) {
        const unsigned old = atomicAdd(p.ctl + ENG_CTL_EXIT, 1u);
        if (old + 1 == (unsigned)nb) {
            __hip_atomic_store((eng_gu32*)(p.ctl + ENG_CTL_EXIT), 0u, ENG_RLX);
            __hip_atomic_store((eng_gu32*)(p.ctl + ENG_CTL_ARRIVED), 0u, ENG_RLX);
            for (int x = 0; x < 8; ++x) __hip_atomic_store((eng_gu32*)(p.ctl + ENG_CTL_XCD + x), 0u, ENG_RLX);
            __hip_atomic_store((eng_gu32*)(p.ctl + ENG_CTL_EPOCH), epoch + ENG_EPOCH_STEP, ENG_RLX);
        }
    }
}

}
```

Baseline: 777.9 tokens/s.

## Keep part of fast-layer W13 weights resident in gathering waves' registers

For the fast codebook loop, a resident variant of the kernel loads a slice of each layer's W13 rows once into the gathering waves' registers and computes those rows' SwiGLU outputs there. The compute waves then stream a smaller W13 range, and completion counting now expects arrivals from all waves. The aim is to cut per-codebook weight streaming and spread the FFN gemv onto otherwise idle waves. The cost is much higher register pressure in the gathering waves, a possible occupancy or spill penalty, and more complex synchronisation. A non-temporal load flag is also threaded through the weight issues.

```diff
diff --git a/fish-tts_amd/csrc/engine.hip b/fish-tts_amd/csrc/engine.hip
--- a/fish-tts_amd/csrc/engine.hip
+++ b/fish-tts_amd/csrc/engine.hip
@@ -457,7 +457,7 @@
 typedef void (*eng_fast_fn_t)(FastEngP);
 typedef void (*eng_qkv0_fn_t)(const bf16_t*, const bf16_t*, const bf16_t*, const bf16_t*, bf16_t*, int, int, int, float);
 struct EngSlowEntry { int D, H, HKV, HDIM, F, SQ, SF, SO; eng_slow_fn_t xl, plain; };
-struct EngFastEntry { int D, H, HKV, HDIM, F, V, SQ, SF, SO; eng_fast_fn_t loop; eng_qkv0_fn_t qkv0; };
+struct EngFastEntry { int D, H, HKV, HDIM, F, V, SQ, SF, SO; eng_fast_fn_t loop; eng_qkv0_fn_t qkv0; eng_fast_fn_t resident; int resf, resl; };
 template <typename S, bool WITH_XL>
 static EngSlowEntry eng_slow_entry() {
     eng_slow_fn_t xl = nullptr;
@@ -466,7 +466,10 @@
 }
 template <typename S>
 static EngFastEntry eng_fast_entry() {
-    return EngFastEntry{S::D, S::H, S::HKV, S::HDIM, S::F, S::V, S::SQ, S::SF, S::SO, fast_engine_kernel<S, 10>, eng_qkv0_table_kernel<S>};
+    eng_fast_fn_t res = nullptr;
+    if constexpr (S::RESF > 0) res = fast_engine_kernel<S, 10, true>;
+    return EngFastEntry{S::D, S::H, S::HKV, S::HDIM, S::F, S::V, S::SQ, S::SF, S::SO, fast_engine_kernel<S, 10, false>, eng_qkv0_table_kernel<S>,
+                        res, S::RESF, S::RESL};
 }
 static const EngSlowEntry* eng_slow_shapes(int* n) {
     static const EngSlowEntry tab[] = {eng_slow_entry<EngSlowS1, true>(), eng_slow_entry<EngSlowShape<1024, 16, 8, 128, 4096>, true>(),
@@ -586,7 +589,8 @@
                          per(ctx->fastV) <= fe->SO * ENG_CW && per(fqkvN) <= ENG_LINE && per(c.fast_intermediate_size) <= ENG_LINE && ctx->fastV <= 1024 &&
                          c.codebook_size <= 65536;
     if (!fast_ok) { why += "; fast loop on launches (FT_NO_FAST_ENGINE, or fast widths outside the instantiations: 1024 / 16 + 8 heads x 64 / ffn 3072 or 4096 / 1024 codes used, <= 10 codebooks)"; return true; }
-    ctx->eng_fast_fn = (const void*)fe->loop;
+    const bool fast_res = fe->resident != nullptr && c.n_fast_layer <= fe->resl && getenv("FT_NO_RESIDENT") == nullptr;
+    ctx->eng_fast_fn = (const void*)(fast_res ? fe->resident : fe->loop);
     auto fast_off = [&](const std::string& w2) { why += "; fast loop on launches (" + w2 + ")"; return true; };
     std::vector<EngLayer> hf(c.n_fast_layer);
     for (int i = 0; i < c.n_fast_layer; ++i) {
@@ -633,6 +637,16 @@
     }
     ctx->eng_fast_on = true;
     why = ctx->eng_xl ? "slow stack (one kv head per XCD) and codebook loop on the frame engine" : "slow stack and codebook loop on the frame engine";
+    {
+        char buf[160];
+        if (fast_res)
+            snprintf(buf, sizeof buf, "; codebook loop: %d of %d W13 pairs per CU of %d layers resident in the gathering waves' registers",
+                     fe->resf * ENG_GW, per(c.fast_intermediate_size), c.n_fast_layer);
+        else
+            snprintf(buf, sizeof buf, "; codebook loop: all weights streamed (%s)", fe->resident == nullptr ? "no resident set fits this shape class" :
+                     c.n_fast_layer > fe->resl ? "more layers than the resident set holds" : "FT_NO_RESIDENT is set");
+        why += buf;
+    }
     return true;
 }
 
diff --git a/fish-tts_amd/csrc/frame_engine.h b/fish-tts_amd/csrc/frame_engine.h
--- a/fish-tts_amd/csrc/frame_engine.h
+++ b/fish-tts_amd/csrc/frame_engine.h
@@ -27,6 +27,8 @@
     static constexpr int NTD = D / 512, NTA = HD / 512, NTF = F / 512;
     static constexpr int SQ = (QKVN / ENG_NB + ENG_CW - 1) / ENG_CW, SF = (F / ENG_NB + ENG_CW - 1) / ENG_CW, SO = (D / ENG_NB + ENG_CW - 1) / ENG_CW;
     static constexpr bool PK3 = F % 384 == 0 && (F / ENG_NB) % 3 == 0;
+    static constexpr int RESF = (NTD <= 2 && F / ENG_NB == 12) ? 2 : 0;
+    static constexpr int RESL = RESF ? 4 : 0;
     static_assert(D % 512 == 0 && HD % 512 == 0 && F % 512 == 0 && V == 1024 && HD == D, "fast widths");
     static_assert(QKVN % (4 * ENG_NB) == 0 && D % (4 * ENG_NB) == 0 && F % (4 * ENG_NB) == 0 && V % (4 * ENG_NB) == 0, "whole granule groups per workgroup");
 };
@@ -346,6 +348,19 @@
     __device__ __forceinline__ int operator()(int u) const { return u < nq ? q0 + u : (u < nq + nk ? k0 + (u - nq) : v0 + (u - nq - nk)); }
 };
 
+template <int NT, int RPU, int MAXS>
+__device__ __forceinline__ void eng_res_pin(EngW<NT, RPU, MAXS>& r) {
+#pragma unroll
+    for (int s = 0; s < MAXS; ++s)
+#pragma unroll
+        for (int rr = 0; rr < RPU; ++rr)
+#pragma unroll
+            for (int t = 0; t < NT; ++t) {
+                U4& w = r.w[s][rr][t];
+                asm volatile("" : "+v"(w.x), "+v"(w.y), "+v"(w.z), "+v"(w.w));
+            }
+}
+
 template <bool NTL = true, int NT, int RPU, int MAXS, typename RM = EngRowIdent>
 __device__ __forceinline__ void eng_issue(EngW<NT, RPU, MAXS>& r, const bf16_t* W, const bf16_t* gain, int K, int u_lo, int u_hi,
                                           int cw, int lane, int nt, RM rm = RM()) {
@@ -460,17 +475,17 @@
     }
 }
 
-template <int NT, int RPU, int MAXS, int PRO, int EPI, bool PK3 = false>
-__device__ __forceinline__ void eng_gemv(const EngW<NT, RPU, MAXS>& r, const float* xs, int K, float eps, const bf16_t* bias,
-                                         const float* resid, unsigned* gout, unsigned tag, float* plain, int u_lo, int u_hi,
-                                         int cw, int lane, EngOut& eo) {
-    eng_gemv_rows<NT, RPU, MAXS, PRO, EPI>(r, xs, K, eps, bias, resid, eo.vals, u_lo, u_hi, cw, lane);
+template <int NT, int RPU, int MAXS, int PRO, int EPI, bool PK3 = false, int ARR = ENG_CW>
+__device__ __forceinline__ void eng_gemv_part(const EngW<NT, RPU, MAXS>& r, const float* xs, int K, float eps, const bf16_t* bias,
+                                              const float* resid, unsigned* gout, unsigned tag, float* plain, int u_lo, int u_hi,
+                                              int r_lo, int r_hi, int cw, int lane, EngOut& eo) {
+    eng_gemv_rows<NT, RPU, MAXS, PRO, EPI>(r, xs, K, eps, bias, resid, eo.vals + (r_lo - u_lo), r_lo, r_hi, cw, lane);
     __builtin_amdgcn_fence(__ATOMIC_RELEASE, "workgroup", "local");
     int old = 0;
     if (lane == 0) old = __hip_atomic_fetch_add((eng_lds_int)eo.count, 1, __ATOMIC_RELAXED, __HIP_MEMORY_SCOPE_WORKGROUP);
     old = __builtin_amdgcn_readfirstlane(old);
     eo.seq += 1;
-    if (old + 1 == eo.seq * ENG_CW) {
+    if (old + 1 == eo.seq * ARR) {
         __builtin_amdgcn_fence(__ATOMIC_ACQUIRE, "workgroup", "local");
         const int n = u_hi - u_lo;
         if constexpr (PK3) {
@@ -486,6 +501,12 @@
             if (plain) plain[u_lo + lane] = o;
         }
     }
+}
+template <int NT, int RPU, int MAXS, int PRO, int EPI, bool PK3 = false>
+__device__ __forceinline__ void eng_gemv(const EngW<NT, RPU, MAXS>& r, const float* xs, int K, float eps, const bf16_t* bias,
+                                         const float* resid, unsigned* gout, unsigned tag, float* plain, int u_lo, int u_hi,
+                                         int cw, int lane, EngOut& eo) {
+    eng_gemv_part<NT, RPU, MAXS, PRO, EPI, PK3, ENG_CW>(r, xs, K, eps, bias, resid, gout, tag, plain, u_lo, u_hi, u_lo, u_hi, cw, lane, eo);
 }
 
 template <int NT, int RPU, int MAXS, int PRO, int EPI>
@@ -564,23 +585,24 @@
     }
 }
 
-template <int NT, int RPU, int MAXS, int PRO, int EPI>
-__device__ __forceinline__ void eng_gemv2(const EngW<NT, RPU, MAXS>& r, const float* xs0, const float* xs1, int K, float eps,
-                                          const bf16_t* bias, const float* resid0, const float* resid1, unsigned* gout0, unsigned* gout1,
-                                          unsigned tag0, unsigned tag1, int u_lo, int u_hi, int cw, int lane, EngOut& eo) {
+template <int NT, int RPU, int MAXS, int PRO, int EPI, int ARR = ENG_CW>
+__device__ __forceinline__ void eng_gemv2_part(const EngW<NT, RPU, MAXS>& r, const float* xs0, const float* xs1, int K, float eps,
+                                               const bf16_t* bias, const float* resid0, const float* resid1, unsigned* gout0, unsigned* gout1,
+                                               unsigned tag0, unsigned tag1, int u_lo, int u_hi, int r_lo, int r_hi, int cw, int lane, EngOut& eo) {
+    float* const v0 = eo.vals + (r_lo - u_lo);
     if (NT <= 2) {
-        eng_gemv_rows2<NT, RPU, MAXS, PRO, EPI>(r, xs0, xs1, K, eps, bias, resid0, resid1, eo.vals, eo.vals + 32, u_lo, u_hi, cw, lane);
+        eng_gemv_rows2<NT, RPU, MAXS, PRO, EPI>(r, xs0, xs1, K, eps, bias, resid0, resid1, v0, v0 + 32, r_lo, r_hi, cw, lane);
     } else {
-        eng_gemv_rows<NT, RPU, MAXS, PRO, EPI>(r, xs0, K, eps, bias, resid0, eo.vals, u_lo, u_hi, cw, lane);
+        eng_gemv_rows<NT, RPU, MAXS, PRO, EPI>(r, xs0, K, eps, bias, resid0, v0, r_lo, r_hi, cw, lane);
         __builtin_amdgcn_sched_barrier(0);
-        eng_gemv_rows<NT, RPU, MAXS, PRO, EPI>(r, xs1, K, eps, bias, resid1, eo.vals + 32, u_lo, u_hi, cw, lane);
+        eng_gemv_rows<NT, RPU, MAXS, PRO, EPI>(r, xs1, K, eps, bias, resid1, v0 + 32, r_lo, r_hi, cw, lane);
     }
     __builtin_amdgcn_fence(__ATOMIC_RELEASE, "workgroup", "local");
     int old = 0;
     if (lane == 0) old = __hip_atomic_fetch_add((eng_lds_int)eo.count, 1, __ATOMIC_RELAXED, __HIP_MEMORY_SCOPE_WORKGROUP);
     old = __builtin_amdgcn_readfirstlane(old);
     eo.seq += 1;
-    if (old + 1 == eo.seq * ENG_CW) {
+    if (old + 1 == eo.seq * ARR) {
         __builtin_amdgcn_fence(__ATOMIC_ACQUIRE, "workgroup", "local");
         const int n = u_hi - u_lo;
         const int i = lane & 31;
@@ -589,6 +611,13 @@
             eng_put(lane < 32 ? gout0 : gout1, i, o, lane < 32 ? tag0 : tag1);
         }
     }
+}
+template <int NT, int RPU, int MAXS, int PRO, int EPI>
+__device__ __forceinline__ void eng_gemv2(const EngW<NT, RPU, MAXS>& r, const float* xs0, const float* xs1, int K, float eps,
+                                          const bf16_t* bias, const float* resid0, const float* resid1, unsigned* gout0, unsigned* gout1,
+                                          unsigned tag0, unsigned tag1, int u_lo, int u_hi, int cw, int lane, EngOut& eo) {
+    eng_gemv2_part<NT, RPU, MAXS, PRO, EPI, ENG_CW>(r, xs0, xs1, K, eps, bias, resid0, resid1, gout0, gout1, tag0, tag1, u_lo, u_hi, u_lo, u_hi,
+                                                    cw, lane, eo);
 }
 
 __device__ __forceinline__ void eng_units(int U, int b, int nb, int& lo, int& hi) {
@@ -1225,6 +1254,7 @@
     int pair;
     const bf16_t* qkv0_tab;
     unsigned long long* stamps;
+    int nt;
 };
 #define ENG_FSTAMP(k) do { if (p.stamps && tid == 0) p.stamps[(((size_t)b * p.ncb + cb) * nL + li) * 16 + (k)] = eng_rt(); } while (0)
 
@@ -1753,10 +1783,15 @@
     return by;
 }
 
-template <typename FS, int MAXCB>
+template <typename FS, int MAXCB, bool RES>
 __global__ __launch_bounds__(ENG_THREADS) void fast_engine_kernel(FastEngP p) {
     constexpr int NTD = FS::NTD, NTA = FS::NTA, NTF = FS::NTF, HDIM = FS::HDIM;
     constexpr int SQ = FS::SQ, SF = FS::SF, SO = FS::SO;
+    static_assert(!RES || (FS::RESF > 0 && FS::RESL > 0), "this shape class has no resident set");
+    constexpr int RF = RES ? FS::RESF : 0, RL = RES ? FS::RESL : 0, FRES = RF * ENG_GW;
+    constexpr int SFC = RES ? (FS::F / ENG_NB - FRES + ENG_CW - 1) / ENG_CW : SF;
+    constexpr int ARRF = RES ? ENG_WAVES : ENG_CW;
+    static_assert(FS::F / ENG_NB > FRES, "the compute waves keep at least one pair");
     extern __shared__ __attribute__((aligned(16))) float smem[];
     const int tid = threadIdx.x, lane = tid & 63, wave = __builtin_amdgcn_readfirstlane(tid >> 6);
     const int b = blockIdx.x;
@@ -1790,7 +1825,12 @@
     float* gS1 = xB1 + D;
     float* qkvS1 = gS1;
     float* yS1 = gS1 + QKVN;
-    if (tid == 0) { *dead = eng_fault_here(p.ctl, ENG_FAULT_FAST, b) ? 1 : 0; *out_count = 0; *sub_count = 0; }
+    int f_lo, f_hi;
+    eng_units(F, b, nb, f_lo, f_hi);
+    const int f_c_hi = f_hi - FRES;
+    EngW<NTD, 2, (RF ? RF : 1)> res[RL ? RL : 1];
+    if (p.stamps && tid == 0) p.stamps[(size_t)b * p.ncb * p.n_layer * 16 + 15] = eng_rt();
+    if (tid == 0) { *dead = eng_fault_here(p.ctl, ENG_FAULT_FAST, b) ? 1 : 0; *out_count = 0; *sub_count = 0; dead[3] = 0; }
     if (tid == ENG_CW * 64) {
         reg_s[0] = 0; reg_s[1] = 0; reg_s[2] = 1;
         if (p.rep_stride) eng_register(p.ctl, nb, reg_s, dead);
@@ -1809,27 +1849,29 @@
     const bool pair = p.pair != 0 && p.ncb >= 2;
 
     if (wave < ENG_CW) {
-        int q_lo, q_hi, o_lo, o_hi, f_lo, f_hi, h_lo, h_hi;
+        int q_lo, q_hi, o_lo, o_hi, h_lo, h_hi;
         eng_units(QKVN, b, nb, q_lo, q_hi);
         eng_units(D, b, nb, o_lo, o_hi);
-        eng_units(F, b, nb, f_lo, f_hi);
         eng_units(V, b, nb, h_lo, h_hi);
         EngW<NTD, 1, SQ> wq;
         EngW<NTA, 1, SO> wo;
-        EngW<NTD, 2, SF> wf;
+        EngW<NTD, 2, SFC> wf;
         EngW<NTF, 1, SO> wd;
         EngW<NTD, 1, SO> wh;
         EngOut eo{outS, out_count, 0};
+        EngOut eo13{outS, dead + 3, 0};
+        EngOut& eoF = RES ? eo13 : eo;
         {
             const EngLayer l0 = eng_layer(p.layers, 0);
-            eng_issue<false>(wq, l0.wqkv, l0.attn_norm, D, q_lo, q_hi, cw, lane, 0);
-            eng_issue<false>(wo, l0.wo, (const bf16_t*)nullptr, HD, o_lo, o_hi, cw, lane, 0);
-            eng_issue<false>(wf, l0.w13, l0.ffn_norm, D, f_lo, f_hi, cw, lane, 0);
-            eng_issue<false>(wd, l0.w2, (const bf16_t*)nullptr, F, o_lo, o_hi, cw, lane, 0);
+            eng_issue<false>(wq, l0.wqkv, l0.attn_norm, D, q_lo, q_hi, cw, lane, p.nt);
+            eng_issue<false>(wo, l0.wo, (const bf16_t*)nullptr, HD, o_lo, o_hi, cw, lane, p.nt);
+            eng_issue<false>(wf, l0.w13, l0.ffn_norm, D, f_lo, f_c_hi, cw, lane, p.nt);
+            eng_issue<false>(wd, l0.w2, (const bf16_t*)nullptr, F, o_lo, o_hi, cw, lane, p.nt);
             __builtin_amdgcn_sched_barrier(0);
         }
         eng_barrier();
         eng_barrier();
+        if (p.stamps && tid == 0) p.stamps[(size_t)b * p.ncb * p.n_layer * 16 + 14] = eng_rt();
         if (pair) {
             const unsigned tag0 = eng_tag16(epoch), tag1 = eng_tag16(epoch + 1u);
             float r0c[2], r0s[2], r1c[2], r1s[2];
@@ -1861,7 +1903,7 @@
                                                               bq(1, li) + eng_pub(b, q_lo), tag0, tag1, q_lo, q_hi, cw, lane, eo);
                 __builtin_amdgcn_sched_barrier(0);
                 ENG_FSTAMP(1);
-                if (more && !(li == nL - 1 && p.qkv0_tab != nullptr)) eng_issue<false>(wq, ln.wqkv, ln.attn_norm, D, q_lo, q_hi, cw, lane, 0);
+                if (more && !(li == nL - 1 && p.qkv0_tab != nullptr)) eng_issue<false>(wq, ln.wqkv, ln.attn_norm, D, q_lo, q_hi, cw, lane, p.nt);
                 __builtin_amdgcn_sched_barrier(0);
                 eng_barrier(); if (*dead) { alive = false; break; }
                 ENG_FSTAMP(2);
@@ -1879,19 +1921,19 @@
                                                               o_lo, o_hi, cw, lane, eo);
                 __builtin_amdgcn_sched_barrier(0);
                 ENG_FSTAMP(4);
-                if (more) eng_issue<false>(wo, ln.wo, (const bf16_t*)nullptr, HD, o_lo, o_hi, cw, lane, 0);
+                if (more) eng_issue<false>(wo, ln.wo, (const bf16_t*)nullptr, HD, o_lo, o_hi, cw, lane, p.nt);
                 __builtin_amdgcn_sched_barrier(0);
                 eng_barrier(); if (*dead) { alive = false; break; }
                 ENG_FSTAMP(5);
                 if (tail0)
-                    eng_gemv2<NTD, 2, SF, PRO_RMSNORM, EPI_SWIGLU>(wf, xB, xB1, D, p.eps, nullptr, nullptr, nullptr, bg(0, li) + eng_pub(b, f_lo),
-                                                                   bg(1, li) + eng_pub(b, f_lo), tag0, tag1, f_lo, f_hi, cw, lane, eo);
+                    eng_gemv2_part<NTD, 2, SFC, PRO_RMSNORM, EPI_SWIGLU, ARRF>(wf, xB, xB1, D, p.eps, nullptr, nullptr, nullptr, bg(0, li) + eng_pub(b, f_lo),
+                                                                               bg(1, li) + eng_pub(b, f_lo), tag0, tag1, f_lo, f_hi, f_lo, f_c_hi, cw, lane, eoF);
                 else
-                    eng_gemv<NTD, 2, SF, PRO_RMSNORM, EPI_SWIGLU, FS::PK3>(wf, xB1, D, p.eps, nullptr, nullptr, bg(1, li) + (FS::PK3 ? 0 : eng_pub(b, f_lo)), tag1, nullptr,
-                                                                    f_lo, f_hi, cw, lane, eo);
+                    eng_gemv_part<NTD, 2, SFC, PRO_RMSNORM, EPI_SWIGLU, FS::PK3, ARRF>(wf, xB1, D, p.eps, nullptr, nullptr, bg(1, li) + (FS::PK3 ? 0 : eng_pub(b, f_lo)), tag1, nullptr,
+                                                                                f_lo, f_hi, f_lo, f_c_hi, cw, lane, eoF);
                 __builtin_amdgcn_sched_barrier(0);
                 ENG_FSTAMP(6);
-                if (more) eng_issue<false>(wf, ln.w13, ln.ffn_norm, D, f_lo, f_hi, cw, lane, 0);
+                if (more) eng_issue<false>(wf, ln.w13, ln.ffn_norm, D, f_lo, f_c_hi, cw, lane, p.nt);
                 __builtin_amdgcn_sched_barrier(0);
                 eng_barrier(); if (*dead) { alive = false; break; }
                 ENG_FSTAMP(7);
@@ -1903,8 +1945,8 @@
                                                               o_lo, o_hi, cw, lane, eo);
                 __builtin_amdgcn_sched_barrier(0);
                 ENG_FSTAMP(8);
-                if (more) eng_issue<false>(wd, ln.w2, (const bf16_t*)nullptr, F, o_lo, o_hi, cw, lane, 0);
-                if (li == nL - 1) eng_issue<false>(wh, p.fast_out, p.fast_norm, D, h_lo, h_hi, cw, lane, 0);
+                if (more) eng_issue<false>(wd, ln.w2, (const bf16_t*)nullptr, F, o_lo, o_hi, cw, lane, p.nt);
+                if (li == nL - 1) eng_issue<false>(wh, p.fast_out, p.fast_norm, D, h_lo, h_hi, cw, lane, p.nt);
                 __builtin_amdgcn_sched_barrier(0);
             }
             if (alive) {
@@ -1941,7 +1983,7 @@
                 __builtin_amdgcn_sched_barrier(0);
                 ENG_FSTAMP(1);
                 if (more && !(li == nL - 1 && p.qkv0_tab != nullptr && cb + 1 >= 2))
-                    eng_issue<false>(wq, ln.wqkv, ln.attn_norm, D, q_lo, q_hi, cw, lane, 0);
+                    eng_issue<false>(wq, ln.wqkv, ln.attn_norm, D, q_lo, q_hi, cw, lane, p.nt);
                 __builtin_amdgcn_sched_barrier(0);
                 eng_barrier(); if (*dead) { alive = false; break; }
                 ENG_FSTAMP(2);
@@ -1954,15 +1996,15 @@
                                                           o_lo, o_hi, cw, lane, eo);
                 __builtin_amdgcn_sched_barrier(0);
                 ENG_FSTAMP(4);
-                if (more) eng_issue<false>(wo, ln.wo, (const bf16_t*)nullptr, HD, o_lo, o_hi, cw, lane, 0);
+                if (more) eng_issue<false>(wo, ln.wo, (const bf16_t*)nullptr, HD, o_lo, o_hi, cw, lane, p.nt);
                 __builtin_amdgcn_sched_barrier(0);
                 eng_barrier(); if (*dead) { alive = false; break; }
                 ENG_FSTAMP(5);
-                eng_gemv<NTD, 2, SF, PRO_RMSNORM, EPI_SWIGLU, FS::PK3>(wf, xB, D, p.eps, nullptr, nullptr, bg(par, li) + (FS::PK3 ? 0 : eng_pub(b, f_lo)), tag, nullptr,
-                                                                f_lo, f_hi, cw, lane, eo);
+                eng_gemv_part<NTD, 2, SFC, PRO_RMSNORM, EPI_SWIGLU, FS::PK3, ARRF>(wf, xB, D, p.eps, nullptr, nullptr, bg(par, li) + (FS::PK3 ? 0 : eng_pub(b, f_lo)), tag, nullptr,
+                                                                            f_lo, f_hi, f_lo, f_c_hi, cw, lane, eoF);
                 __builtin_amdgcn_sched_barrier(0);
                 ENG_FSTAMP(6);
-                if (more) eng_issue<false>(wf, ln.w13, ln.ffn_norm, D, f_lo, f_hi, cw, lane, 0);
+                if (more) eng_issue<false>(wf, ln.w13, ln.ffn_norm, D, f_lo, f_c_hi, cw, lane, p.nt);
                 __builtin_amdgcn_sched_barrier(0);
                 eng_barrier(); if (*dead) { alive = false; break; }
                 ENG_FSTAMP(7);
@@ -1970,8 +2012,8 @@
                                                           o_lo, o_hi, cw, lane, eo);
                 __builtin_amdgcn_sched_barrier(0);
                 ENG_FSTAMP(8);
-                if (more) eng_issue<false>(wd, ln.w2, (const bf16_t*)nullptr, F, o_lo, o_hi, cw, lane, 0);
-                if (li == nL - 1 && cb >= 1) eng_issue<false>(wh, p.fast_out, p.fast_norm, D, h_lo, h_hi, cw, lane, 0);
+                if (more) eng_issue<false>(wd, ln.w2, (const bf16_t*)nullptr, F, o_lo, o_hi, cw, lane, p.nt);
+                if (li == nL - 1 && cb >= 1) eng_issue<false>(wh, p.fast_out, p.fast_norm, D, h_lo, h_hi, cw, lane, p.nt);
                 __builtin_amdgcn_sched_barrier(0);
             }
             if (!alive) break;
@@ -1987,6 +2029,8 @@
         EngSub sub{sub_count, 0};
         SampP sp = p.samp;
         int prev_code = 0;
+        EngOut eo13{outS, dead + 3, 0};
+        U4 fgain[NTD];
         eng_barrier();
         const EngRelay rl{p.rep_stride != 0, reg_s[1], reg_s[2], p.rep_delta0 + (long)reg_s[0] * p.rep_stride};
         eng_barrier();
@@ -2004,11 +2048,13 @@
             for (int li = 0; li < nL; ++li) {
                 const EngLayer l = eng_layer(p.layers, li);
                 const bool tail0 = li + 1 < nL;
+                int gl = lane;
+                if constexpr (RES) asm volatile("" : "+v"(gl));
                 const int wh = 1000 + 64 + li * 8;
                 bf16_t* kL = kvS + (size_t)(li * 2) * p.ncb * KVW;
                 bf16_t* vL = kvS + (size_t)(li * 2 + 1) * p.ncb * KVW;
                 if (li > 0) {
-                    eng_gather_x2(rl, EngSrc2{{bx(0, li), bx(1, li)}, {xA, xA1}, {tag0, tag1}}, D, gw, ENG_GW, lane, p.ctl, dead, wh + 0);
+                    eng_gather_x2(rl, EngSrc2{{bx(0, li), bx(1, li)}, {xA, xA1}, {tag0, tag1}}, D, gw, ENG_GW, gl, p.ctl, dead, wh + 0);
                 } else {
                     for (int d = atid * 4; d < D; d += ENG_GW * 64 * 4) {
                         *reinterpret_cast<float4*>(xA + d) = *reinterpret_cast<const float4*>(p.hid + d);
@@ -2016,18 +2062,42 @@
                     }
                 }
                 eng_barrier(); if (*dead) { alive = false; break; }
-                eng_gather_x2(rl, EngSrc2{{bq(0, li), bq(1, li)}, {qkvS, qkvS1}, {tag0, tag1}}, QKVN, gw, ENG_GW, lane, p.ctl, dead, wh + 1);
+                eng_gather_x2(rl, EngSrc2{{bq(0, li), bq(1, li)}, {qkvS, qkvS1}, {tag0, tag1}}, QKVN, gw, ENG_GW, gl, p.ctl, dead, wh + 1);
                 eng_barrier(); if (*dead) { alive = false; break; }
+                if constexpr (RES) {
+#pragma unroll
+                    for (int r = 0; r < RL; ++r)
+                        if (li == r) eng_issue<false>(res[r], l.w13, (const bf16_t*)nullptr, D, f_c_hi, f_hi, gw, lane, p.nt);
+#pragma unroll
+                    for (int t = 0; t < NTD; ++t) fgain[t] = eng_ldg16<false>(l.ffn_norm + t * 512 + lane * 8);
+                    __builtin_amdgcn_sched_barrier(0);
+                }
                 eng_fast_attn_any<MAXCB, HDIM>(qkvS, kL, vL, yS, l.qn, l.kn, r0c, r0s, 0, p.ncb, H, Hkv, p.eps, p.scale, wave, ENG_WAVES, lane);
                 eng_barrier();
                 eng_fast_attn_any<MAXCB, HDIM>(qkvS1, kL, vL, yS1, l.qn, l.kn, r1c, r1s, 1, p.ncb, H, Hkv, p.eps, p.scale, wave, ENG_WAVES, lane);
                 eng_barrier();
-                if (tail0) eng_gather_x2(rl, EngSrc2{{bxb(0, li), bxb(1, li)}, {xB, xB1}, {tag0, tag1}}, D, gw, ENG_GW, lane, p.ctl, dead, wh + 2);
-                else eng_gather_x(rl, bxb(1, li), layD, 0, D, tag1, xB1, gw, ENG_GW, lane, p.ctl, dead, wh + 2);
+                if (tail0) eng_gather_x2(rl, EngSrc2{{bxb(0, li), bxb(1, li)}, {xB, xB1}, {tag0, tag1}}, D, gw, ENG_GW, gl, p.ctl, dead, wh + 2);
+                else eng_gather_x(rl, bxb(1, li), layD, 0, D, tag1, xB1, gw, ENG_GW, gl, p.ctl, dead, wh + 2);
                 eng_barrier(); if (*dead) { alive = false; break; }
-                if (tail0) eng_gather_x2(rl, EngSrc2{{bg(0, li), bg(1, li)}, {gS, gS1}, {tag0, tag1}}, F, gw, ENG_GW, lane, p.ctl, dead, wh + 3);
-                else if constexpr (FS::PK3) eng_gather3_x(rl, bg(1, li), F, tag1, gS1, gw, ENG_GW, lane, p.ctl, dead, wh + 3);
-                else eng_gather_x(rl, bg(1, li), layF, 0, F, tag1, gS1, gw, ENG_GW, lane, p.ctl, dead, wh + 3);
+                if constexpr (RES) {
+#pragma unroll
+                    for (int r = 0; r < RL; ++r)
+                        if (li == r) {
+                            eng_res_pin(res[r]);
+#pragma unroll
+                            for (int t = 0; t < NTD; ++t) res[r].gain[t] = fgain[t];
+                            if (tail0)
+                                eng_gemv2_part<NTD, 2, RF, PRO_RMSNORM, EPI_SWIGLU, ARRF>(res[r], xB, xB1, D, p.eps, nullptr, nullptr, nullptr, bg(0, li) + eng_pub(b, f_lo),
+                                                                                          bg(1, li) + eng_pub(b, f_lo), tag0, tag1, f_lo, f_hi, f_c_hi, f_hi, gw, lane, eo13);
+                            else
+                                eng_gemv_part<NTD, 2, RF, PRO_RMSNORM, EPI_SWIGLU, FS::PK3, ARRF>(res[r], xB1, D, p.eps, nullptr, nullptr, bg(1, li) + (FS::PK3 ? 0 : eng_pub(b, f_lo)),
+                                                                                           tag1, nullptr, f_lo, f_hi, f_c_hi, f_hi, gw, lane, eo13);
+                        }
+                    __builtin_amdgcn_sched_barrier(0);
+                }
+                if (tail0) eng_gather_x2(rl, EngSrc2{{bg(0, li), bg(1, li)}, {gS, gS1}, {tag0, tag1}}, F, gw, ENG_GW, gl, p.ctl, dead, wh + 3);
+                else if constexpr (FS::PK3) eng_gather3_x(rl, bg(1, li), F, tag1, gS1, gw, ENG_GW, gl, p.ctl, dead, wh + 3);
+                else eng_gather_x(rl, bg(1, li), layF, 0, F, tag1, gS1, gw, ENG_GW, gl, p.ctl, dead, wh + 3);
                 eng_barrier(); if (*dead) { alive = false; break; }
             }
         }
@@ -2041,16 +2111,20 @@
                 rcs[e] = d < hd ? p.rope[((size_t)cb * (hd >> 1) + (d >> 1)) * 2] : 1.f;
                 rsn[e] = d < hd ? p.rope[((size_t)cb * (hd >> 1) + (d >> 1)) * 2 + 1] : 0.f;
             }
+            int at = atid, dl = lane;
+            if constexpr (RES) asm volatile("" : "+v"(at), "+v"(dl));
             EngDrawPre pre{};
             if (cb >= 1) {
                 sp.cb = cb;
                 sp.noise_off = p.noise_off1 + (long)(cb - 1) * p.noise_cb_stride;
-                pre = eng_draw_pre(sp, atid);
+                pre = eng_draw_pre(sp, at);
             }
             for (int li = (pair && cb == 1) ? nL : 0; li < nL; ++li) {
                 const EngLayer l = eng_layer(p.layers, li);
+                int gl = lane;
+                if constexpr (RES) asm volatile("" : "+v"(gl));
                 if (li > 0) {
-                    eng_gather_x(rl, bx(par, li), layD, 0, D, tag, xA, gw, ENG_GW, lane, p.ctl, dead, 1000 + cb * 64 + li * 8 + 0);
+                    eng_gather_x(rl, bx(par, li), layD, 0, D, tag, xA, gw, ENG_GW, gl, p.ctl, dead, 1000 + cb * 64 + li * 8 + 0);
                 } else if (cb <= 1) {
                     const float* src = cb == 0 ? p.hid : p.femb;
                     for (int d = atid * 4; d < D; d += ENG_GW * 64 * 4) *reinterpret_cast<float4*>(xA + d) = *reinterpret_cast<const float4*>(src + d);
@@ -2090,33 +2164,55 @@
                 }
                 eng_barrier(); if (*dead) { alive = false; break; }
                 if (!(li == 0 && cb >= 2 && p.qkv0_tab))
-                    eng_gather_x(rl, bq(par, li), layQ, 0, QKVN, tag, qkvS, gw, ENG_GW, lane, p.ctl, dead, 1000 + cb * 64 + li * 8 + 1);
+                    eng_gather_x(rl, bq(par, li), layQ, 0, QKVN, tag, qkvS, gw, ENG_GW, gl, p.ctl, dead, 1000 + cb * 64 + li * 8 + 1);
                 eng_barrier(); if (*dead) { alive = false; break; }
+                if constexpr (RES) {
+                    if (!pair && cb == 0) {
+#pragma unroll
+                        for (int r = 0; r < RL; ++r)
+                            if (li == r) eng_issue<false>(res[r], l.w13, (const bf16_t*)nullptr, D, f_c_hi, f_hi, gw, lane, p.nt);
+                    }
+#pragma unroll
+                    for (int t = 0; t < NTD; ++t) fgain[t] = eng_ldg16<false>(l.ffn_norm + t * 512 + lane * 8);
+                    __builtin_amdgcn_sched_barrier(0);
+                }
                 eng_fast_attn_any<MAXCB, HDIM>(qkvS, kvS + (size_t)(li * 2) * p.ncb * KVW, kvS + (size_t)(li * 2 + 1) * p.ncb * KVW, yS, l.qn, l.kn,
                                          rcs, rsn, cb, p.ncb, H, Hkv, p.eps, p.scale, wave, ENG_WAVES, lane);
                 eng_barrier();
-                eng_gather_x(rl, bxb(par, li), layD, 0, D, tag, xB, gw, ENG_GW, lane, p.ctl, dead, 1000 + cb * 64 + li * 8 + 2);
+                eng_gather_x(rl, bxb(par, li), layD, 0, D, tag, xB, gw, ENG_GW, gl, p.ctl, dead, 1000 + cb * 64 + li * 8 + 2);
                 eng_barrier(); if (*dead) { alive = false; break; }
-                if constexpr (FS::PK3) eng_gather3_x(rl, bg(par, li), F, tag, gS, gw, ENG_GW, lane, p.ctl, dead, 1000 + cb * 64 + li * 8 + 3);
-                else eng_gather_x(rl, bg(par, li), layF, 0, F, tag, gS, gw, ENG_GW, lane, p.ctl, dead, 1000 + cb * 64 + li * 8 + 3);
+                if constexpr (RES) {
+#pragma unroll
+                    for (int r = 0; r < RL; ++r)
+                        if (li == r) {
+                            eng_res_pin(res[r]);
+#pragma unroll
+                            for (int t = 0; t < NTD; ++t) res[r].gain[t] = fgain[t];
+                            eng_gemv_part<NTD, 2, RF, PRO_RMSNORM, EPI_SWIGLU, FS::PK3, ARRF>(res[r], xB, D, p.eps, nullptr, nullptr, bg(par, li) + (FS::PK3 ? 0 : eng_pub(b, f_lo)),
+                                                                                       tag, nullptr, f_lo, f_hi, f_c_hi, f_hi, gw, lane, eo13);
+                        }
+                    __builtin_amdgcn_sched_barrier(0);
+                }
+                if constexpr (FS::PK3) eng_gather3_x(rl, bg(par, li), F, tag, gS, gw, ENG_GW, gl, p.ctl, dead, 1000 + cb * 64 + li * 8 + 3);
+                else eng_gather_x(rl, bg(par, li), layF, 0, F, tag, gS, gw, ENG_GW, gl, p.ctl, dead, 1000 + cb * 64 + li * 8 + 3);
                 eng_barrier(); if (*dead) { alive = false; break; }
             }
             if (!alive) break;
             if (cb >= 1) {
-                eng_gather_x(rl, bx(par, nL), layD, 0, D, tag, xA, gw, ENG_GW, lane, p.ctl, dead, 1000 + cb * 64 + 56);
+                eng_gather_x(rl, bx(par, nL), layD, 0, D, tag, xA, gw, ENG_GW, dl, p.ctl, dead, 1000 + cb * 64 + 56);
                 eng_barrier(); if (*dead) { alive = false; break; }
                 ENG_GSTAMP(10);
                 {
-                    eng_gather_x(rl, blog(par), layV, 0, V, tag, logS, gw, ENG_GW, lane, p.ctl, dead, 1000 + cb * 64 + 57);
+                    eng_gather_x(rl, blog(par), layV, 0, V, tag, logS, gw, ENG_GW, dl, p.ctl, dead, 1000 + cb * 64 + 57);
                     sub.n = 0;
-                    if (atid == 0) *sub_count = *dead ? 1 : 0;
-                    sub.sync(lane);
+                    if (at == 0) *sub_count = *dead ? 1 : 0;
+                    sub.sync(dl);
                     ENG_GSTAMP(11);
                     if (*reinterpret_cast<volatile int*>(sub_count) == 0) {
                         const int last = cb == p.ncb - 1;
                         const int nfv = pre.nfv;
                         EngSampLds S{redbuf, pen_id, pen_val, amv, ami, wcnt, prL, keyL, cut};
-                        const int code = eng_sample_small(sp, pre, logS, S, sub, atid, lane, gw,
+                        const int code = eng_sample_small(sp, pre, logS, S, sub, at, dl, gw,
                                                           p.stamps ? p.stamps + (((size_t)b * p.ncb + cb) * nL + nL - 1) * 16 : nullptr);
                         ENG_GSTAMP(14);
                         const int R = p.ncb + 1;
```

Measured after the change: 787.1 tokens/s (median of 6 runs). 1.2% higher.
